# DIAGNijmegen/prostateMR_3D-CAD-csPCa

Measured on AMD Instinct MI355X. Metric: train-step volumes/sec (whole job), M1 (20,160,160,3), higher is better.
Workload: dtype bf16; 1 GPU; C3 M1 full hierarchical-probabilistic dense_skip+deep_supervision latents (3,2,1,0) (20,160,160,3); batch_per_gpu=2, global_batch=2, params=67254246, parallelism=dp1, hip_graph=True

## Files before the change

include/m1hip.h:

```cpp
#ifndef M1HIP_H
#define M1HIP_H

#include <stddef.h>
#include <stdint.h>

#ifdef __cplusplus
extern "C" {
#endif

enum m1_dtype { M1_F32 = 0, M1_BF16 = 1 };

enum m1_status {
    M1_OK = 0,
    M1_ERR_BAD_ARG = -1,
    M1_ERR_UNSUPPORTED = -2,
    M1_ERR_LAUNCH = -3,
    M1_ERR_WORKSPACE = -4
};

#define M1_MAX_SRC 6

typedef struct {
    const void* ptr;
    int C;
    int _pad;
} m1_src_t;

typedef struct {
    int N, D, H, W;
    int Cin, Cout;
    int kd, kh, kw;
    int sd, sh, sw;
    int dtype;
    int nsrc;
    m1_src_t src[M1_MAX_SRC];
} m1_conv_desc_t;

const char* m1_status_name(int status);
int m1_abi_version(void);

size_t m1_conv_ws_bytes(const m1_conv_desc_t* d, int transposed, int role);
int m1_conv_pack_jobs(const m1_conv_desc_t* d, int transposed, int role, void* ws, void** jobs_out);
int m1_pack_batch(const void* const* jobs_dev, const int* block_prefix_dev, int njobs, int total_blocks, void* stream);
int m1_conv3d_fwd(const m1_conv_desc_t* d, const float* w, const float* bias, void* y, float* stats, void* ws,
                  int ws_packed, void* stream);
int m1_conv3d_dgrad(const m1_conv_desc_t* d, const float* w, const void* dy, void* const* dx, const int* accumulate,
                    void* ws, int ws_packed, void* stream);
int m1_conv3d_pair_supported(const m1_conv_desc_t* d, int C1);
int m1_conv3d_dgrad_inbwd_rows(const m1_conv_desc_t* d);
int m1_conv3d_dgrad_inbwd(const m1_conv_desc_t* d, const float* w, const void* dy, void* da, const void* x, const float* stats,
                          const float* gamma, const float* beta, float slope, float* partial, int partial_rows, int* nparts,
                          void* ws, int ws_packed, void* stream);
int m1_conv3d_pair_fwd(const m1_conv_desc_t* d, const float* w1, const float* b1, const float* w4, const float* b4, int C1,
                       void* y1, void* y4, float* stats1, float* stats4, void* ws, int ws_packed, void* stream);
int m1_conv3d_pair_dgrad(const m1_conv_desc_t* d, const float* w1, const float* w4, int C1, const void* dy1, const void* dy4,
                         void* const* dx, const int* accumulate, void* ws, int ws_packed, void* stream);
int m1_conv3d_wgrad(const m1_conv_desc_t* d, const void* dy, float* dw, float* db, void* ws, int accumulate,
                    void* stream);
int m1_set_force_direct(int on);
int m1_config_set(const char* name, int value);
int m1_config_unset(const char* name);
int m1_config_get(const char* name, int* value);
int m1_debug_lds_canary(unsigned* bad, int blocks, int spins, void* stream);
int m1_debug_checksum(const void* p, long long nbytes, unsigned long long* slot, void* stream);
const char* m1_debug_kernels(int mode);
const char* m1_debug_plans(int mode);
int m1_debug_scribble(int blocks, int spins, void* stream);

int m1_convT3d_fwd(const m1_conv_desc_t* d, const float* w, const float* bias, void* y, void* ws, int ws_packed,
                   void* stream);
int m1_convT3d_dgrad(const m1_conv_desc_t* d, const float* w, const void* dy, void* const* dx, const int* accumulate,
                     void* ws, int ws_packed, void* stream);
int m1_convT3d_wgrad(const m1_conv_desc_t* d, const void* dy, float* dw, float* db, void* ws, int accumulate,
                     void* stream);

size_t m1_reduce_ws_floats(int N, long long V, int C, int nsums);
int m1_instnorm_stats(const void* x, int N, long long V, int C, int dtype, float eps, float* stats, float* ws,
                      void* stream);
int m1_instnorm_apply(const void* x, const float* stats, const float* gamma, const float* beta, float slope,
                      void* y, int N, long long V, int C, int dtype, void* stream);
int m1_instnorm_bwd(const void* x, const float* stats, const float* gamma, const float* beta, float slope,
                    const void* dy, void* dx, float* dgamma, float* dbeta, int N, long long V, int C, int dtype,
                    float* ws, int accumulate, void* stream);

int m1_instnorm_bwd_partials(const void* x, const float* stats, const float* gamma, const float* beta, float slope,
                             const void* dy, void* dx, float* dgamma, float* dbeta, int N, long long V, int C, int dtype,
                             const float* partial, int nparts, float* sums, int accumulate, void* stream);

int m1_se_gate_fwd(const float* beta3, const float* W6, const float* b6, const float* W7, const float* b7,
                   int F, int Fr, float* hidden, float* g, void* stream);
int m1_se_gate_bwd(const float* beta3, const float* W6, const float* W7, const float* hidden, const float* g,
                   const float* dg, int F, int Fr, float* dbeta3_add, float* dW6, float* db6, float* dW7,
                   float* db7, int accumulate, void* stream);
#define M1_SE_GATE_BATCH 16
typedef struct {
    const float* beta3; const float* W6; const float* b6; const float* W7; const float* b7;
    float* hidden; float* g;
    int F, Fr;
} m1_se_gate_fwd_job_t;
int m1_se_gate_fwd_batch(const m1_se_gate_fwd_job_t* jobs , int njobs, void* stream);
typedef struct {
    const float* beta3; const float* W6; const float* W7; const float* hidden; const float* g;
    float* dg;
    float* dbeta3_add; float* dW6; float* db6; float* dW7; float* db7;
    int F, Fr, accumulate, _pad;
} m1_se_gate_job_t;
int m1_se_gate_bwd_batch(const m1_se_gate_job_t* jobs , int njobs, void* stream);
int m1_se_combine_fwd(const void* y3, const void* y4, const float* stats3, const float* stats4,
                      const float* gamma3, const float* beta3, const float* gamma4, const float* beta4,
                      const float* g, void* out, int N, long long V, int F, int dtype, float drop_rate,
                      const uint64_t* rng, uint64_t layer_id, unsigned char* keep_mask, void* stream);
int m1_se_combine_bwd(const void* y3, const void* y4, const float* stats3, const float* stats4,
                      const float* gamma3, const float* beta3, const float* gamma4, const float* beta4,
                      const float* g, const void* dout, void* dy3, void* dy4, float* dgamma3, float* dbeta3,
                      float* dgamma4, float* dbeta4, float* dg, int N, long long V, int F, int dtype,
                      float drop_rate, const uint64_t* rng, uint64_t layer_id, const unsigned char* keep_mask,
                      float* ws, int accumulate, void* stream);

int m1_se_combine_dup_fwd(const void* y3, const void* y4, const float* stats3, const float* stats4,
                          const float* gamma3, const float* beta3, const float* gamma4, const float* beta4,
                          const float* g, void* out, int N, long long V, int F, int dtype, float drop_rate,
                          const uint64_t* rng, uint64_t layer_id, unsigned char* keep_mask, void* stream);
int m1_se_combine_dup_bwd(const void* y3, const void* y4, const float* stats3, const float* stats4,
                          const float* gamma3, const float* beta3, const float* gamma4, const float* beta4,
                          const float* g, const void* dout, void* dy3, void* dy4, float* dgamma3, float* dbeta3,
                          float* dgamma4, float* dbeta4, float* dg, int N, long long V, int F, int dtype,
                          float drop_rate, const uint64_t* rng, uint64_t layer_id, const unsigned char* keep_mask,
                          float* ws, int accumulate, void* stream);

int m1_gate_sigma_fwd(const void* theta, const void* phi, const float* wpsi, const float* bpsi, void* sigma,
                      int N, int Dt, int Ht, int Wt, int Dp, int Hp, int Wp, int C, int dtype, void* stream);
int m1_gate_sigma_bwd(const void* theta, const void* phi, const float* wpsi, const void* sigma,
                      const void* dsigma, void* dtheta, void* dphi, float* dwpsi, float* dbpsi, int N, int Dt,
                      int Ht, int Wt, int Dp, int Hp, int Wp, int C, int dtype, float* ws, int accumulate,
                      void* stream);
int m1_mul_sigma_fwd(const void* x, const void* sigma, void* y, int N, int D, int H, int W, int C, int s0,
                     int s1, int s2, int dtype, void* stream);
int m1_gate_sigma_mul_fwd(const void* theta, const void* phi, const float* wpsi, const float* bpsi, void* sigma, const void* x,
                          void* y, int N, int Dt, int Ht, int Wt, int Dp, int Hp, int Wp, int Ci, int D, int H, int W, int Cx,
                          int s0, int s1, int s2, int dtype, void* stream);
int m1_mul_sigma_bwd(const void* x, const void* sigma, const void* dy, void* dx, void* dsigma, int N, int D,
                     int H, int W, int C, int s0, int s1, int s2, int dtype, int accumulate_dx, void* stream);

int m1_latent_sample_fwd(const void* ml, const void* eps, void* z, int N, long long V, int L, int mode,
                         int dtype, void* stream);
int m1_latent_sample_bwd(const void* ml, const void* eps, const void* dz, void* dml, int N, long long V, int L,
                         int mode, int dtype, void* stream);
int m1_latent_sample_rng_fwd(const void* ml, const uint64_t* rng, uint64_t stream_id, void* z, int N, long long V, int L, int mode,
                             int dtype, void* stream);
int m1_latent_sample_rng_bwd(const void* ml, const uint64_t* rng, uint64_t stream_id, const void* dz, void* dml, int N, long long V,
                             int L, int mode, int dtype, void* stream);
int m1_kl_fwd(const void* ml_q, const void* ml_p, float* kl, int N, long long V, int L, int dtype, void* stream);
int m1_kl_bwd(const void* ml_q, const void* ml_p, const float* dkl, void* dml_q, void* dml_p, int N,
              long long V, int L, int dtype, void* stream);
int m1_kl_bwd_first(const void* ml_q, const void* ml_p, const float* dkl, void* dml_q, void* dml_p, int N, long long V,
                    int L, int Nall, int dtype, void* stream);

typedef struct {
    const void* logits;
    void* dlogits;
    int u0, u1, u2;
    int _pad;
} m1_head_t;
int m1_softmax_heads_fwd(const m1_head_t* heads, int nheads, float* probs, int N, int D, int H, int W, int nc,
                         int dtype, void* stream);
int m1_softmax_heads_bwd(const m1_head_t* heads, int nheads, const float* probs, const float* dprobs, int N,
                         int D, int H, int W, int nc, int dtype, void* stream);

int m1_mc_accum(const void* logits, int R, int B, long long V, int nc, int dtype, float* sum_p, int accumulate, float* samples_out,
                void* stream);
int m1_mc_finish(const float* sum_p, int n_draws, int B, long long V, int nc, float* mean, float* entropy, void* stream);

int m1_mc_accum_u(const void* logits, int R, int B, long long V, int nc, int dtype, float* sum_p, float* sum_h, float* sum_pp,
                  int accumulate, float* samples_out, void* stream);
int m1_mc_finish_u(const float* sum_p, const float* sum_h, const float* sum_pp, int n_draws, int B, long long V, int nc, float* mean,
                   float* entropy, float* expected_entropy, float* mutual_info, float* variance, void* stream);

int m1_mc_accum_v(const void* logits, int R, int B, int D, int H, int W, int nc, int dtype, unsigned long long flips, float* sum_p,
                  float* sum_h, float* sum_pp, int accumulate, float* samples_out, void* stream);
int m1_tta_views(const void* x, int B, int D, int H, int W, int C, int dtype, int R, unsigned long long flips, void* out, void* stream);

#define M1_TILE_MAX_AXIS 16
typedef struct { int vol[3]; int tile[3]; int n[3]; int origin[3][M1_TILE_MAX_AXIS]; } m1_tile_t;
int m1_tile_gather(const void* x, int B, int C, int dtype, const m1_tile_t* g, void* out, void* stream);
int m1_tile_blend(const float* tiles, int B, int C, const m1_tile_t* g, const float* profile, float* out, void* stream);

size_t m1_focal_ws_floats(int N, long long V, int nheads);
int m1_focal_fwd(const float* probs, const void* y_true, int y_dtype, const float* alpha, float gamma, int N, long long V,
                 int nheads, int nc, float* ws, float* loss, void* stream);
int m1_focal_bwd(const float* probs, const void* y_true, int y_dtype, const float* alpha, float gamma, int N, long long V,
                 int nheads, int nc, const float* dloss, float* dprobs, void* stream);

size_t m1_dist_map_ws_bytes(int N, int D, int H, int W, int nc);
int m1_dist_map(const void* y_true, int y_dtype, int N, int D, int H, int W, int nc, void* ws, float* out, void* stream);
size_t m1_dice_bd_ws_floats(long long NV, int nheads);
int m1_dice_bd_fwd(const float* probs, const void* y_true, int y_dtype, const float* phi, long long NV, int nheads, int nc,
                   float w0, float w1, float smooth, float* ws, float* loss, void* stream);
int m1_dice_bd_bwd(const float* probs, const void* y_true, int y_dtype, const float* phi, long long NV, int nheads, int nc,
                   float w0, float w1, float smooth, const float* ws, const float* dloss, float* dprobs, void* stream);

enum m1_aug_stage {
    M1_AUG_MASTER = 1, M1_AUG_ZOOM = 2, M1_AUG_FLIP = 4, M1_AUG_ROTATE = 8, M1_AUG_TRANSLATE = 16, M1_AUG_CSHIFT = 32,
    M1_AUG_GAMMA = 64, M1_AUG_POOR = 128, M1_AUG_NOISE = 256
};
typedef struct {
    uint32_t fired;
    uint32_t gamma_ch;
    uint32_t poor_ch;
    int32_t scale;
    int32_t rot_pad;
    float rot[6];
    int32_t tr[4];
    int32_t cs[4];
    int32_t cs_channel;
    float gamma;
    float noise_std;
    float angle_deg;
    int32_t _pad;
} m1_aug_params_t;
int m1_aug_draw(m1_aug_params_t* table, int N, const uint64_t* rng, uint64_t stream_id, double prob, double tx_prob,
                double translate_factor, double rotation_degree, int axial_hflip, double zoom_factor, double gauss_noise_stddev,
                double chan_shift_factor, int sim_poor_scan, double gamma_lo, double gamma_hi, int H, int W, int nimg, int lesion,
                void* stream);
size_t m1_aug_ws_bytes(int N, int D, int H, int W, int nimg);
int m1_aug_geom(const float* x, const float* y, const m1_aug_params_t* table, float* gx, float* gy, int N, int D, int H, int W,
                int C, int nimg, int nc, int stages, int dtype, void* ws, void* stream);
int m1_aug_gamma_stats(const float* gx, const m1_aug_params_t* table, int N, int D, int H, int W, int C, int nimg, int stages,
                       int dtype, void* ws, void* stream);
int m1_aug_intensity(const float* gx, const m1_aug_params_t* table, const uint64_t* rng, uint64_t stream_id, float* out, int N,
                     int D, int H, int W, int C, int nimg, int stages, int dtype, void* ws, void* stream);

int m1_contour_smooth_u8(const uint8_t* in, uint8_t* out, uint8_t* scratch, long long planes, int H, int W, const int* taps,
                         int iterations, void* stream);
enum m1_label_objective { M1_LABEL_LESION = 0, M1_LABEL_ZONAL = 1 };
enum m1_feed_mode { M1_FEED_TRAIN = 0, M1_FEED_VALID = 1, M1_FEED_TEST = 2 };
int m1_label_prepare(const uint8_t* ann, const float* image, float* x_out, float* detection, float* kl, int B, int D, int H, int W,
                     int C, int objective, int mode, int probabilistic, const int* taps, void* stream);

enum m1_raw_dtype { M1_RAW_F32 = 0, M1_RAW_I16 = 1, M1_RAW_I32 = 2 };
enum m1_pad_mode { M1_PAD_CONSTANT = 0, M1_PAD_EDGE = 1, M1_PAD_REFLECT = 2, M1_PAD_SYMMETRIC = 3 };
typedef struct { int src[3]; int dst[3]; int start[3]; int mode; float cval; } m1_crop_pad_t;
size_t m1_preprocess_ws_bytes(const m1_crop_pad_t* g, int B, int C, int nq);
int m1_crop_pad(const void* src, int src_dtype, const m1_crop_pad_t* g, int B, int C, void* out, int out_dtype, void* stream);
int m1_order_stats(const void* src, int src_dtype, const m1_crop_pad_t* g, int B, int C, const int* ranks, const double* weights,
                   int nq, float* pairs, float* values, void* ws, void* stream);
int m1_whiten(const void* src, int src_dtype, const m1_crop_pad_t* g, int B, int C, const float* bounds, void* out, int out_dtype,
              double* stats, void* ws, void* stream);

#define M1_RESAMPLE_MAX_LINE 1024
typedef struct { int src[3]; int dst[3]; int first[3]; int order; double step[3]; float defval; int _pad; } m1_resample_t;
size_t m1_resample_ws_bytes(const m1_resample_t* g, int B, int C);
int m1_resample(const void* src, int src_dtype, const m1_resample_t* g, int B, int C, void* out, int out_dtype, void* ws, void* stream);

#define M1_RESTORE_MAX_SEL 4
typedef struct { int src[3]; int dst[3]; int first[3]; int count[3]; int lo[3]; int order; double ratio[3]; float defval; int deflabel; } m1_restore_t;
int m1_restore(const void* src, int src_dtype, const m1_restore_t* g, int B, int C, int c0, int nsel, void* prob, void* label,
               void* stream);

#define M1_CC_TILE_Z 4
#define M1_CC_TILE_Y 8
#define M1_CC_TILE_X 32
enum m1_cc_dtype { M1_CC_F32 = 0, M1_CC_U8 = 1 };
enum m1_cc_state {
    M1_CC_ST_PEAK = 0, M1_CC_ST_ARGMAX = 1, M1_CC_ST_THRESHOLD = 2, M1_CC_ST_SEL = 3, M1_CC_ST_COUNT = 4, M1_CC_ST_DONE = 5,
    M1_CC_ST_NCAND = 6, M1_CC_ST_SPARE = 7
};
typedef struct {
    int32_t count;
    float vmax;
    int64_t argmax;
    int32_t lo[3];
    int32_t hi[3];
    int64_t sum[3];
} m1_cc_row_t;
size_t m1_cc_ws_bytes(int B, int D, int H, int W);
int m1_cc_label(const void* src, int src_dtype, float threshold, const float* threshold_dev, int connectivity, int B, int D, int H, int W,
                int* labels, int* counts, void* ws, void* stream);
int m1_cc_stats(const int* labels, const float* values, int B, int D, int H, int W, int max_components, m1_cc_row_t* rows, void* stream);
int m1_cc_overlap(const int* a, const int* b, int B, long long n, int max_a, int max_b, int* table, void* stream);
int m1_cc_peak(const float* w, int B, long long n, float factor, float min_confidence, int reset, int* state, void* ws, void* stream);
int m1_cc_select(const int* labels, int B, long long n, int* state, void* stream);
int m1_cc_take(const int* labels, int* state, const float* w_src, float* w, float* detection_map, int* candidates, float* confidences, int B, long long n,
               int max_candidates, int min_voxels, int reset, void* stream);
int m1_cc_relabel(const int* labels, const m1_cc_row_t* rows, int B, long long n, int max_components, int min_voxels, int* map,
                  float* detection_map, int* candidates, float* confidences, int* ncand, void* stream);

#define M1_SD_MAX_CLASSES 8
#define M1_SD_MAX_TOLERANCES 4
#define M1_SD_MAX_LINE 256
enum m1_sd_dtype { M1_SD_U8 = 0, M1_SD_I32 = 1 };
enum m1_sd_stage { M1_SD_STAGE_BORDER = 0, M1_SD_STAGE_DISTANCE = 1, M1_SD_STAGE_METRICS = 2 };
typedef struct {
    int64_t n[2];
    int64_t le[2][4];
    double sum[2];
    float hd, hd_ab, hd_ba;
    float assd, mean_ab, mean_ba;
    float hdq, hdq_ab, hdq_ba;
    float dice;
    float nsd[4];
    float _pad[2];
} m1_sd_row_t;
size_t m1_sd_ws_bytes(int stage, int B, int K, int D, int H, int W);
int m1_sd_border(const void* pred, const void* truth, int dtype, const int* labels, int K, int B, int D, int H, int W, uint8_t* borders,
                 long long* counts, void* ws, void* stream);
int m1_sd_distance(const uint8_t* mask, int N, int D, int H, int W, const double* spacing, float* dist, void* ws, void* stream);
int m1_sd_metrics(const uint8_t* borders, const float* dist, const long long* counts, int B, int K, int D, int H, int W, double percentile,
                  const float* tolerances, int T, m1_sd_row_t* rows, void* ws, void* stream);

int m1_dropout(const void* x, void* y, long long n, float rate, const uint64_t* rng, uint64_t layer_id, int dtype,
               void* stream);

int m1_cast(const void* x, int src_dtype, void* y, int dst_dtype, long long n, void* stream);

int m1_adam_amsgrad(float* p, const float* g, float* m, float* v, float* vhat, long long n, long long n_kernel,
                    long long n_bias, float l2_kernel, float l2_bias, float grad_scale, const float* lr_dev,
                    float beta1, float beta2, float eps, const int* step_dev, void* stream);
int m1_step_advance(int* step_dev, uint64_t* rng_dev, void* stream);

typedef struct {
    float norm;
    float coef;
    int32_t apply;
    int32_t skipped;
} m1_step_ctl_t;
size_t m1_grad_norm_ws(long long n);
int m1_grad_norm(const float* g, const float* p, long long n, long long n_kernel, long long n_bias, float l2_kernel,
                 float l2_bias, float grad_scale, float clipvalue, float global_clipnorm, int skip_nonfinite, void* ws,
                 size_t ws_bytes, m1_step_ctl_t* ctl, void* stream);
int m1_adam_amsgrad_ctl(float* p, const float* g, float* m, float* v, float* vhat, long long n, long long n_kernel,
                        long long n_bias, float l2_kernel, float l2_bias, float grad_scale, const float* lr_dev,
                        float beta1, float beta2, float eps, const int* step_dev, float clipvalue,
                        const m1_step_ctl_t* ctl, void* stream);
int m1_step_advance_ctl(int* step_dev, const m1_step_ctl_t* ctl, void* stream);

enum m1_val_dtype { M1_VAL_Y_F32 = 0, M1_VAL_Y_U8 = 1 };
typedef struct {
    double focal, entropy_sum, entropy_fg_sum, n_voxels, n_fg, _head[3];
    struct { double sum_p, sum_y, sum_py, n_pred, n_true, n_both, p_max, _pad; } cls[4];
} m1_val_record_t;
size_t m1_val_score_ws(int B, long long voxels, int K);
int m1_val_score(const float* p, const void* y, int y_dtype, const float* entropy, const float* alpha, float gamma, int B,
                 long long voxels, int K, m1_val_record_t* records, void* ws, size_t ws_bytes, void* stream);

size_t m1_cal_record_slots(int K, int bins);
int m1_cal_score(const void* p, int p_dtype, const unsigned char* label, const unsigned char* mask, const float* unc, float u_scale,
                 int B, long long voxels, int K, int bins, unsigned long long* records, void* stream);

#define M1_STREAM_BOOTSTRAP 0x424F4F54ull
#define M1_BOOTSTRAP_MAX_CASES 16384
#define M1_BOOTSTRAP_MAX_BOOT (1 << 20)
#define M1_BOOTSTRAP_MAX_RATES 8
#define M1_BOOTSTRAP_MAX_VALUES 16
#define M1_BOOTSTRAP_CHUNK 1024
typedef struct {
    const unsigned char* case_label; const unsigned char* case_group_end; const int* case_lesions;
    const int* ev_case; const unsigned char* ev_tp; const unsigned char* ev_group_end;
    const double* values; const int* draw_perm;
    int N, M, V, P;
} m1_bootstrap_table_t;
int m1_bootstrap_metrics(const m1_bootstrap_table_t* table, int n_boot, uint64_t seed, const int* weights, const double* fp_rates,
// ... 22 lines not shown
```

prostatemr_3d-cad-cspca_amd/csrc/dispatch.hip:

```cpp
#include "common.h"
#include "wgrad_fold.h"
#include "reduce.h"
#include <stdio.h>
#include <stdlib.h>

static inline bool desc_ok(const m1_conv_desc_t* d) {
    if (!(d && d->N > 0 && d->D > 0 && d->H > 0 && d->W > 0 && d->Cin > 0 && d->Cout > 0 && d->kd > 0 && d->kh > 0 &&
          d->kw > 0 && d->sd > 0 && d->sh > 0 && d->sw > 0 && d->nsrc >= 1 && d->nsrc <= M1_MAX_SRC)) return false;
    if (d->dtype != M1_F32 && d->dtype != M1_BF16) return false;
    int c = 0;
    for (int i = 0; i < d->nsrc; ++i) { if (!d->src[i].ptr || d->src[i].C <= 0) return false; c += d->src[i].C; }
    return c == d->Cin;
}
static inline double esz(int dt) { return dt == M1_BF16 ? 2.0 : 4.0; }
static inline void same_pad(int in, int k, int s, int* out, int* pb) {
    int o = (in + s - 1) / s;
    int tot = (o - 1) * s + k - in; if (tot < 0) tot = 0;
    *out = o; *pb = tot / 2;
}
static inline int convT_pb(int k, int s) { return (k - s > 0 ? k - s : 0) / 2; }

struct Geo { int OD, OH, OW, pd, ph, pw; };
static inline Geo conv_geo(const m1_conv_desc_t* d) {
    Geo g; same_pad(d->D, d->kd, d->sd, &g.OD, &g.pd); same_pad(d->H, d->kh, d->sh, &g.OH, &g.ph); same_pad(d->W, d->kw, d->sw, &g.OW, &g.pw);
// ... 240 lines not shown
    return align256(b);
}
struct WgradWs { size_t reduce_bytes, x8, r8, rx, total; long long rx_floats; };
static WgradWs wgrad_ws(const m1_conv_desc_t* d, bool T) {
    const Geo q = T ? convT_geo(d) : conv_geo(d);
    WgradWs w{};
    w.reduce_bytes = align256(m1_reduce_ws_floats(d->N, (long long)q.OD * q.OH * q.OW, d->Cout, 1) * sizeof(float)) + 256;
    w.x8 = w.r8 = w.rx = w.reduce_bytes;
    if (stem_wanted(d, T)) {
        w.r8 = w.x8 + align256((size_t)d->N * d->D * d->H * d->W * 16);
        w.rx = w.r8 + align256((size_t)d->kd * d->kh * d->kw * 8 * d->Cout * sizeof(float));
    }
    const size_t rx_bytes = wgrad_rx_bytes(d);
    w.rx_floats = (long long)(rx_bytes / sizeof(float));
    w.total = w.rx + rx_bytes * (size_t)d->nsrc;
    return w;
}

extern "C" size_t m1_conv_ws_bytes(const m1_conv_desc_t* d, int transposed, int role) {
    if (!desc_ok(d)) return 0;
    return role == 0 || role == 1 ? plan_gather(d, transposed != 0, role).total : wgrad_ws(d, transposed != 0).total;
}

extern "C" int m1_conv_pack_jobs(const m1_conv_desc_t* d, int transposed, int role, void* ws, void** jobs_out) {
    if (!desc_ok(d) || !ws || !jobs_out || (role != 0 && role != 1)) return 0;
    const GatherPlan p = plan_gather(d, transposed != 0, role);
    int n = 0;
    for (int k = 0; k < p.n; ++k) if (p.item[k].bytes) jobs_out[n++] = at(ws, p.item[k].off);
    return n;
}
extern "C" int m1_pack_batch(const void* const* jobs_dev, const int* block_prefix_dev, int njobs, int total_blocks, void* stream) {
    if (m1_debug_skip("pack")) return M1_OK;
    if (njobs < 0 || (njobs > 0 && !jobs_dev) || (block_prefix_dev && total_blocks < njobs)) return M1_ERR_BAD_ARG;
    M1ProfScope ps("pack_batch", 0.0, 0.0, (hipStream_t)stream);
    return m1_pack_batch_internal(jobs_dev, block_prefix_dev, njobs, total_blocks, (hipStream_t)stream);
}

static int fwd_common(const m1_conv_desc_t* d, bool T, const float* w, const float* bias, void* y, float* stats, void* ws, int ws_packed,
                      hipStream_t st) {
    if (stats && !ws) return M1_ERR_WORKSPACE;
    const GatherPlan p = plan_gather(d, T, 0);
    if (!ws && p.n > 1) return run_gather(fwd_spec(d, T, w, bias, y), nullptr, ws_packed, st);
    for (int k = 0; k < p.n; ++k) {
        GatherSpec g = fwd_item_spec(d, p, k, w, bias, y);
        const bool emit = stats && k == p.n - 1;
        if (emit) { g.stats_out = stats; g.stats_eps = 1e-3f; g.stats_ws = reinterpret_cast<float*>(at(ws, p.stats_off)); }
        int rc = run_gather(g, at(ws, p.item[k].off), ws_packed, st); if (rc) return rc;
        if (emit && p.n == 1 && !use_mfma(g))
            return m1_stats_internal(y, d->N, (long long)g.OD * g.OH * g.OW, d->Cout, d->dtype, 1e-3f, stats, g.stats_ws, st);
    }
    return M1_OK;
}
extern "C" int m1_conv3d_fwd(const m1_conv_desc_t* d, const float* w, const float* bias, void* y, float* stats, void* ws,
                             int ws_packed, void* stream) {
    if (m1_debug_skip("conv_fwd")) return M1_OK;
    if (!desc_ok(d) || !w || !y) return M1_ERR_BAD_ARG;
    M1ProfScope ps(prof_name("conv3d_fwd", d).s, 2.0 * conv_macs(d, false), conv_bytes(d, false), (hipStream_t)stream);
    return fwd_common(d, false, w, bias, y, stats, ws, ws_packed, (hipStream_t)stream);
}
static bool pair_ok(const m1_conv_desc_t* d, int C1) {
    if (!desc_ok(d) || g_force_direct) return false;
    const int seg = d->dtype == M1_BF16 ? 8 : 4;
    if (C1 <= 0 || C1 >= d->Cout || C1 % seg || (d->Cout - C1) % seg) return false;
    for (int i = 0; i < d->nsrc; ++i) if (d->src[i].C % seg) return false;
    return true;
}
static bool pair_fwd_spec(const m1_conv_desc_t* d, int C1, const float* w1, const float* b1, const float* w4, const float* b4, void* y1,
                          void* y4, float* stats1, float* stats4, void* ws, GatherSpec* out) {
    const GatherPlan p = plan_gather(d, false, 0);
    if (p.n != 1) return false;
    const int C4 = d->Cout - C1;
    GatherSpec g = fwd_item_spec(d, p, 0, w1, b1, nullptr);
    g.wST = (long long)d->Cin * C1; g.wSC = C1; g.wSO = 1;
    g.w2 = w4; g.w2ST = (long long)d->Cin * C4; g.w2SC = C4; g.w2SO = 1; g.oc_split = C1; g.bias2 = b4;
    g.nout = 2; g.outs[0] = y1; g.outC[0] = C1; g.outAcc[0] = 0; g.outs[1] = y4; g.outC[1] = C4; g.outAcc[1] = 0;
    if (stats1) { g.stats_out = stats1; g.stats_out2 = stats4; g.stats_eps = 1e-3f; g.stats_ws = reinterpret_cast<float*>(at(ws, p.stats_off)); }
    *out = g;
    return m1_mfma_supported(g) && gather_ws_bytes(g) == p.item[0].bytes;
}
static bool pair_dgrad_spec(const m1_conv_desc_t* d, int C1, const float* w1, const float* w4, const void* dy1, const void* dy4,
                            void* const* dx, const int* accumulate, GatherSpec* out) {
    const GatherPlan p = plan_gather(d, false, 1);
    if (p.n != 1) return false;
    const int C4 = d->Cout - C1;
    GatherSpec g = dgrad_item_spec(d, p, 0, w1, dy1, dx, accumulate);
    g.nsrc = 2; g.src[0] = dy1; g.srcC[0] = C1; g.src[1] = dy4; g.srcC[1] = C4;
    g.wST = (long long)d->Cin * C1; g.wSC = 1; g.wSO = C1;
    g.w2 = w4; g.w2ST = (long long)d->Cin * C4; g.w2SC = 1; g.w2SO = C4; g.c_split = C1;
    *out = g;
    return m1_mfma_supported(g) && gather_ws_bytes(g) <= p.item[0].bytes;
}
extern "C" int m1_conv3d_pair_fwd(const m1_conv_desc_t* d, const float* w1, const float* b1, const float* w4, const float* b4, int C1,
                                  void* y1, void* y4, float* stats1, float* stats4, void* ws, int ws_packed, void* stream) {
    if (m1_debug_skip("conv_fwd")) return M1_OK;
    if (!d || !w1 || !w4 || !y1 || !y4 || !ws || (stats1 == nullptr) != (stats4 == nullptr)) return M1_ERR_BAD_ARG;
    GatherSpec g;
    if (!pair_ok(d, C1) || !pair_fwd_spec(d, C1, w1, b1, w4, b4, y1, y4, stats1, stats4, ws, &g)) return M1_ERR_UNSUPPORTED;
    M1ProfScope ps(prof_name("conv3d_fwd", d).s, 2.0 * conv_macs(d, false), conv_bytes(d, false), (hipStream_t)stream);
    return m1_mfma_gather(g, ws, ws_packed, (hipStream_t)stream);
}
extern "C" int m1_conv3d_pair_dgrad(const m1_conv_desc_t* d, const float* w1, const float* w4, int C1, const void* dy1, const void* dy4,
                                    void* const* dx, const int* accumulate, void* ws, int ws_packed, void* stream) {
    if (m1_debug_skip("conv_dgrad")) return M1_OK;
    if (!d || !w1 || !w4 || !dy1 || !dy4 || !dx || !ws) return M1_ERR_BAD_ARG;
    if (!pair_ok(d, C1)) return M1_ERR_UNSUPPORTED;
    M1ProfScope ps(prof_name("conv3d_dgrad", d).s, 2.0 * conv_macs(d, false), conv_bytes(d, false), (hipStream_t)stream);
    if (d->nsrc == 1 && !dx[0]) return M1_OK;
    GatherSpec g;
    if (!pair_dgrad_spec(d, C1, w1, w4, dy1, dy4, dx, accumulate, &g)) return M1_ERR_UNSUPPORTED;
    bool any = false;
    for (int i = 0; i < d->nsrc; ++i) any |= dx[i] != nullptr;
    return any ? m1_mfma_gather(g, ws, ws_packed, (hipStream_t)stream) : M1_OK;
}

extern "C" int m1_conv3d_pair_supported(const m1_conv_desc_t* d, int C1) {
    GatherSpec g;
    return pair_ok(d, C1) && pair_fwd_spec(d, C1, nullptr, nullptr, nullptr, nullptr, nullptr, nullptr, nullptr, nullptr, nullptr, &g) &&
           pair_dgrad_spec(d, C1, nullptr, nullptr, nullptr, nullptr, nullptr, nullptr, &g);
}

extern "C" int m1_convT3d_fwd(const m1_conv_desc_t* d, const float* w, const float* bias, void* y, void* ws, int ws_packed,
                              void* stream) {
    if (m1_debug_skip("conv_fwd")) return M1_OK;
    if (!desc_ok(d) || !w || !y) return M1_ERR_BAD_ARG;
    M1ProfScope ps(prof_name("convT3d_fwd", d).s, 2.0 * conv_macs(d, true), conv_bytes(d, true), (hipStream_t)stream);
    return fwd_common(d, true, w, bias, y, nullptr, ws, ws_packed, (hipStream_t)stream);
}
static int dgrad_common(const m1_conv_desc_t* d, bool T, const float* w, const void* dy, void* const* dx, const int* accumulate,
                        void* ws, int ws_packed, hipStream_t st) {
    const GatherPlan p = plan_gather(d, T, 1);
    for (int k = 0; k < p.n; ++k) {
        const GatherItem& it = p.item[k];
        bool any = false;
        for (int i = it.first; i < it.first + it.count; ++i) any |= dx[i] != nullptr;
        if (!any) continue;
        int rc = run_gather(dgrad_item_spec(d, p, k, w, dy, dx, accumulate), at(ws, it.off), ws_packed, st); if (rc) return rc;
    }
    return M1_OK;
}
extern "C" int m1_conv3d_dgrad(const m1_conv_desc_t* d, const float* w, const void* dy, void* const* dx, const int* accumulate,
                               void* ws, int ws_packed, void* stream) {
    if (m1_debug_skip("conv_dgrad")) return M1_OK;
    if (!desc_ok(d) || !w || !dy || !dx) return M1_ERR_BAD_ARG;
    M1ProfScope ps(prof_name("conv3d_dgrad", d).s, 2.0 * conv_macs(d, false), conv_bytes(d, false), (hipStream_t)stream);
    return dgrad_common(d, false, w, dy, dx, accumulate, ws, ws_packed, (hipStream_t)stream);
}
extern "C" int m1_conv3d_dgrad_inbwd_rows(const m1_conv_desc_t* d) {
    if (!desc_ok(d)) return 0;
    const long long V = (long long)d->D * d->H * d->W;
    const long long tiles = m1_stats_rows_cap(V), chunks = m1_red_nchunks(V, d->Cin, d->N);
    const long long r = tiles > chunks ? tiles : chunks;
    return r > 0x3fffffff ? 0x3fffffff : (int)r;
}
extern "C" int m1_conv3d_dgrad_inbwd(const m1_conv_desc_t* d, const float* w, const void* dy, void* da, const void* x, const float* stats,
                                     const float* gamma, const float* beta, float slope, float* partial, int partial_rows, int* nparts,
                                     void* ws, int ws_packed, void* stream) {
    if (!desc_ok(d) || !w || !dy || !da || !x || !stats || !gamma || !beta || !partial || !nparts || d->nsrc != 1 || partial_rows < 0) return M1_ERR_BAD_ARG;
    M1ProfScope ps(prof_name("conv3d_dgrad", d).s, 2.0 * conv_macs(d, false), conv_bytes(d, false), (hipStream_t)stream);
    *nparts = 0;
    if (g_force_direct) { void* dxs[1] = {da}; int acc0[1] = {0}; return dgrad_common(d, false, w, dy, dxs, acc0, ws, ws_packed, (hipStream_t)stream); }
    GatherSpec g = dgrad_spec(d, false, w, dy, da, 0, 0);
    g.ib_x = x; g.ib_stats = stats; g.ib_gamma = gamma; g.ib_beta = beta; g.ib_slope = slope; g.ib_partial = partial; g.ib_nparts = nparts; g.ib_cap = partial_rows;
    return run_gather(g, ws, ws_packed, (hipStream_t)stream);
}
extern "C" int m1_convT3d_dgrad(const m1_conv_desc_t* d, const float* w, const void* dy, void* const* dx, const int* accumulate,
                                void* ws, int ws_packed, void* stream) {
    if (m1_debug_skip("conv_dgrad")) return M1_OK;
    if (!desc_ok(d) || !w || !dy || !dx) return M1_ERR_BAD_ARG;
    M1ProfScope ps(prof_name("convT3d_dgrad", d).s, 2.0 * conv_macs(d, true), conv_bytes(d, true), (hipStream_t)stream);
    return dgrad_common(d, true, w, dy, dx, accumulate, ws, ws_packed, (hipStream_t)stream);
}

static WgradSpec wgrad_spec(const m1_conv_desc_t* d, bool T, const Geo& q, int i, int off, const void* dy, float* dw, float* db, float* rx,
                            long long rx_floats) {
    WgradSpec g{};
    g.N = d->N; g.R = dw; g.kd = d->kd; g.kh = d->kh; g.kw = d->kw; g.sd = d->sd; g.sh = d->sh; g.sw = d->sw;
    g.pd = q.pd; g.ph = q.ph; g.pw = q.pw; g.dtype = d->dtype;
    g.rx = rx; g.rx_floats = rx_floats;
    if (!T) {
        g.A = d->src[i].ptr; g.CA = d->src[i].C; g.AD = d->D; g.AH = d->H; g.AW = d->W;
        g.B = dy; g.CB = d->Cout; g.BD = q.OD; g.BH = q.OH; g.BW = q.OW;
        g.RT = (long long)d->Cin * d->Cout; g.RSA = d->Cout; g.a_off = off; g.b_off = 0;
        if (db) { g.bsum = db; g.bsum_tap = (q.pd * d->kh + q.ph) * d->kw + q.pw; }
    } else {
        g.A = dy; g.CA = d->Cout; g.AD = q.OD; g.AH = q.OH; g.AW = q.OW;
        g.B = d->src[i].ptr; g.CB = d->src[i].C; g.BD = d->D; g.BH = d->H; g.BW = d->W;
        g.RT = (long long)d->Cout * d->Cin; g.RSA = d->Cin; g.a_off = 0; g.b_off = off;
    }
    return g;
}
static bool tf_wanted(const WgradSpec& g) {
    int maxc = M1_CFG("M1_TF_MAXC", 128);
    if (g.CA > 64 && g.CB > 32) return false;
    return g.CA <= maxc && g.CB <= maxc && m1_tf_wgrad_supported(g);
}
struct WgCall {
    bool T; int run; const void* Am[M1_MAX_SRC]; int aoffs[M1_MAX_SRC];
    long long nw; int nbias; long long rx_floats; hipStream_t st;
    const char** took;
};
static int equal_run(const m1_conv_desc_t* d, int i) {
    int n = 1;
    while (i + n < d->nsrc && d->src[i + n].C == d->src[i].C) ++n;
    return n;
}
struct WgRung {
    const char* name; bool whole_run, forced;
    bool (*gate)(const WgradSpec& g, const WgCall& c);
    int (*run)(const WgradSpec& g, const WgCall& c);
};
static const WgRung WG_LADDER[] = {
    {"t3", true, false, [](const WgradSpec& g, const WgCall&) { return g.rx && m1_t3_wgrad_supported(g); },
     [](const WgradSpec& g, const WgCall& c) { return m1_t3_wgrad(g, c.nw, c.nbias, c.st, c.run, c.Am, c.aoffs, c.rx_floats); }},
    {"pwf", false, false, [](const WgradSpec& g, const WgCall& c) { return g.rx && g.dtype == M1_F32 && !c.T && m1_pwf_wgrad_supported(g); },
     [](const WgradSpec& g, const WgCall& c) { return m1_pwf_wgrad(g, c.nw, c.nbias, c.st); }},
    {"t3s", false, false, [](const WgradSpec& g, const WgCall&) { return g.rx && g.dtype == M1_F32 && m1_t3s_wgrad_supported(g); },
     [](const WgradSpec& g, const WgCall& c) { return m1_t3s_wgrad(g, c.nw, c.nbias, c.st); }},
    {"tf-multi", true, false,
     [](const WgradSpec& g, const WgCall& c) { int multi = M1_CFG("M1_TF_MULTI", 1); return multi && !c.T && g.rx && tf_wanted(g) && c.run > 1; },
     [](const WgradSpec& g, const WgCall& c) { return m1_tf_wgrad_multi(g, c.nw, c.nbias, c.st, c.run, c.Am, c.aoffs, c.rx_floats); }},
    {"tf", false, false, [](const WgradSpec& g, const WgCall&) { return tf_wanted(g); },
     [](const WgradSpec& g, const WgCall& c) { return m1_tf_wgrad(g, c.nw, c.nbias, c.st); }},
    {"terminal", false, true, [](const WgradSpec&, const WgCall&) { return true; },
     [](const WgradSpec& g, const WgCall& c) {
         if (g_force_direct == 2 && m1_skinny_wgrad_supported(g)) { *c.took = "skinny"; return m1_skinny_wgrad(g, c.st); }
         if (!g_force_direct && m1_tap_wgrad_supported(g)) { *c.took = "tap"; return m1_tap_wgrad(g, c.nw, c.nbias, c.st); }
         if (!g_force_direct && m1_mfma_wgrad_supported(g)) { *c.took = "mfma"; return m1_mfma_wgrad_ex(g, c.nw, c.nbias, c.st); }
         *c.took = "direct"; return m1_direct_wgrad(g, c.st);
     }},
};
static int wgrad_common(const m1_conv_desc_t* d, bool T, const void* dy, float* dw, float* db, void* ws, hipStream_t st,
                        int accumulate) {
    Geo q = T ? convT_geo(d) : conv_geo(d);
    const size_t nw = (size_t)d->kd * d->kh * d->kw * d->Cin * d->Cout;
    if (!accumulate && m1_zero_async(dw, nw * sizeof(float), st) != M1_OK) return M1_ERR_LAUNCH;
    const bool fuse_db = db && !T && !g_force_direct;
    if (fuse_db && !accumulate && m1_zero_async(db, (size_t)d->Cout * sizeof(float), st) != M1_OK) return M1_ERR_LAUNCH;
    const int nbias = fuse_db ? d->Cout : 0;
    const WgradWs L = wgrad_ws(d, T);
    float* const rx = reinterpret_cast<float*>(at(ws, L.rx));
    const long long rx_floats = ws ? L.rx_floats : 0;
    if (stem_wanted(d, T) && ws) {
        const bool f32 = d->dtype == M1_F32;
        const int CP = f32 ? 4 : 8;
        uint4* x8 = reinterpret_cast<uint4*>(at(ws, L.x8));
        float* r8 = reinterpret_cast<float*>(at(ws, L.r8));
        m1_conv_desc_t dp = *d; dp.Cin = CP; dp.src[0].ptr = x8; dp.src[0].C = CP;
        const WgradSpec g = wgrad_spec(&dp, false, q, 0, 0, dy, r8, fuse_db ? db : nullptr, rx, rx_floats);
        if (f32 ? m1_t3s_wgrad_supported(g) : m1_tf_wgrad_supported(g)) {
            const int taps = d->kd * d->kh * d->kw, Cin = d->Cin;
            const long long nvox = (long long)d->N * d->D * d->H * d->W;
            const size_t nw8 = (size_t)taps * CP * d->Cout;
            if (m1_zero_async(r8, nw8 * sizeof(float), st) != M1_OK) return M1_ERR_LAUNCH;
            long long pb = (nvox + 255) / 256; if (pb > 8192) pb = 8192;
            if (f32) hipLaunchKernelGGL(stem_pad4f_kernel, dim3((unsigned)pb), dim3(256), 0, st, (const float*)d->src[0].ptr, reinterpret_cast<float4*>(x8), nvox, Cin);
            else hipLaunchKernelGGL(stem_pad8_kernel, dim3((unsigned)pb), dim3(256), 0, st, (const unsigned short*)d->src[0].ptr, x8, nvox, Cin);
            const int was = m1_fold_defer_set(0);
            int rc = f32 ? m1_t3s_wgrad(g, (long long)nw8, nbias, st) : m1_tf_wgrad(g, (long long)nw8, nbias, st);
            m1_fold_defer_set(was);
            if (rc == M1_OK) {
                m1_note_plan("stem:cp=%d", CP);
                hipLaunchKernelGGL(stem_fold_kernel, dim3((taps * Cin * d->Cout + 255) / 256), dim3(256), 0, st, r8, dw, taps, Cin, d->Cout, CP);
                return m1_check_launch();
            }
            if (rc != M1_ERR_UNSUPPORTED && rc != M1_ERR_WORKSPACE) return rc;
        }
    }
    const int wlog = M1_CFG("M1_WG_LOG", 0);
    for (int i = 0, off = 0; i < d->nsrc;) {
        WgCall c{};
        c.T = T; c.nw = (long long)nw; c.nbias = nbias; c.rx_floats = rx_floats; c.st = st;
        c.run = T ? 1 : equal_run(d, i);
        for (int m = 0, o = off; m < c.run; ++m) { c.Am[m] = d->src[i + m].ptr; c.aoffs[m] = o; o += d->src[i + m].C; }
        const WgradSpec g = wgrad_spec(d, T, q, i, off, dy, dw, fuse_db && i == 0 ? db : nullptr, rx ? rx + (long long)i * rx_floats : nullptr,
                                       rx_floats);
        int rc = M1_ERR_UNSUPPORTED, used = 1;
        for (const WgRung& r : WG_LADDER) {
            if ((g_force_direct && !r.forced) || !r.gate(g, c)) continue;
            const char* took = r.name; c.took = &took;
            rc = r.run(g, c); used = r.whole_run ? c.run : 1;
            if (wlog) fprintf(stderr, "wgrad %s N%d B %dx%dx%d CA %d x%d CB %d k%d%d%d s%d%d%d -> %s rc %d\n", T ? "convT" : "conv", g.N, g.BD,
                              g.BH, g.BW, g.CA, used, g.CB, g.kd, g.kh, g.kw, g.sd, g.sh, g.sw, took, rc);
            if (rc != M1_ERR_UNSUPPORTED && rc != M1_ERR_WORKSPACE) break;
            m1_note_plan("decline:%s rc=%d", r.name, rc);
        }
        if (rc) return rc;
        for (int m = 0; m < used; ++m) off += d->src[i++].C;
    }
    if (db && !fuse_db) {
        if (!ws) return M1_ERR_WORKSPACE;
        const long long Vd = (long long)q.OD * q.OH * q.OW;
        if (!g_force_direct && m1_colsum_defer(dy, d->N, Vd, d->Cout, d->dtype, db, (float*)ws, accumulate)) return M1_OK;
        return m1_colsum_internal(dy, d->N, Vd, d->Cout, d->dtype, db, (float*)ws, st, accumulate);
    }
    return M1_OK;
}
extern "C" int m1_conv3d_wgrad(const m1_conv_desc_t* d, const void* dy, float* dw, float* db, void* ws, int accumulate,
                               void* stream) {
    if (m1_debug_skip("conv_wgrad")) return M1_OK;
    if (!desc_ok(d) || !dy || !dw) return M1_ERR_BAD_ARG;
    M1ProfScope ps(prof_name("conv3d_wgrad", d).s, 2.0 * conv_macs(d, false), conv_bytes(d, false), (hipStream_t)stream);
    return wgrad_common(d, false, dy, dw, db, ws, (hipStream_t)stream, accumulate);
}
extern "C" int m1_convT3d_wgrad(const m1_conv_desc_t* d, const void* dy, float* dw, float* db, void* ws, int accumulate,
                                void* stream) {
    if (m1_debug_skip("conv_wgrad")) return M1_OK;
    if (!desc_ok(d) || !dy || !dw) return M1_ERR_BAD_ARG;
    M1ProfScope ps(prof_name("convT3d_wgrad", d).s, 2.0 * conv_macs(d, true), conv_bytes(d, true), (hipStream_t)stream);
    return wgrad_common(d, true, dy, dw, db, ws, (hipStream_t)stream, accumulate);
}
```

prostatemr_3d-cad-cspca_amd/csrc/gather.h:

```cpp
#pragma once
#include "common.h"

struct GatherSpec {
    const void* src[M1_MAX_SRC]; int srcC[M1_MAX_SRC]; int nsrc;
    int ID, IH, IW;
    void* out; int OC;
    int nout; void* outs[M1_MAX_SRC]; int outC[M1_MAX_SRC]; int outAcc[M1_MAX_SRC];
    int OD, OH, OW, N;
    const float* w; long long wST, wSC, wSO; int oc_off, cc_off;
    const float* bias;
    const float* w2; long long w2ST, w2SC, w2SO; int oc_split, c_split;
    const float* bias2; float* stats_out2;
    int kd, kh, kw, mode, sd, sh, sw, pd, ph, pw;
    int dtype, accumulate;
    float* stats_out;
    float* stats_ws;
    float stats_eps;
    const void* ib_x; const float* ib_stats; const float* ib_gamma; const float* ib_beta; float ib_slope;
    float* ib_partial; int* ib_nparts;
    int ib_cap;
};

int m1_stats_internal(const void* x, int N, long long V, int C, int dtype, float eps, float* stats, float* ws, hipStream_t st);
size_t m1_stats_ws_floats(int N, long long V, int C);

struct WgradSpec {
    const void* A; int CA; int AD, AH, AW;
    const void* B; int CB; int BD, BH, BW;
    int N;
    float* R; long long RT, RSA; int a_off, b_off;
    int kd, kh, kw, sd, sh, sw, pd, ph, pw;
    int dtype;
    float* rx; long long rx_floats;
    float* bsum;
    int bsum_tap;
};

int m1_direct_gather(const GatherSpec& g, hipStream_t st);
int m1_direct_wgrad(const WgradSpec& g, hipStream_t st);
bool m1_skinny_wgrad_supported(const WgradSpec& g);
int m1_skinny_wgrad(const WgradSpec& g, hipStream_t st);
bool m1_mfma_supported(const GatherSpec& g);
size_t m1_mfma_ws_bytes(const GatherSpec& g);
int m1_mfma_gather(const GatherSpec& g, void* ws, int ws_packed, hipStream_t st);
int m1_thin_conv_try(const GatherSpec& g, hipStream_t st, int* rc);
int m1_pack_batch_internal(const void* const* jobs_dev, const int* prefix_dev, int njobs, int total_blocks, hipStream_t st);
bool m1_mfma_wgrad_supported(const WgradSpec& g);
int m1_mfma_wgrad(const WgradSpec& g, hipStream_t st);
bool m1_tf_wgrad_supported(const WgradSpec& g);
int m1_tf_wgrad(const WgradSpec& g, long long nw, int nb, hipStream_t st);
int m1_tf_wgrad_multi(const WgradSpec& g, long long nw, int nb, hipStream_t st, int nmem, const void* const* Am, const int* a_offs, long long rx_mem);
int m1_mfma_wgrad_ex(const WgradSpec& g, long long nw, int nb, hipStream_t st);
bool m1_tap_wgrad_supported(const WgradSpec& g);
int m1_tap_wgrad(const WgradSpec& g, long long nw, int nb, hipStream_t st);
bool m1_t3_wgrad_supported(const WgradSpec& g);
int m1_t3_wgrad(const WgradSpec& g, long long nw, int nb, hipStream_t st, int nmem, const void* const* Am, const int* a_offs, long long rx_mem);
bool m1_t3s_wgrad_supported(const WgradSpec& g);
int m1_t3s_wgrad(const WgradSpec& g, long long nw, int nb, hipStream_t st);
bool m1_pwf_wgrad_supported(const WgradSpec& g);
int m1_pwf_wgrad(const WgradSpec& g, long long nw, int nb, hipStream_t st);
int m1_colsum_internal(const void* x, int N, long long V, int C, int dtype, float* out, float* ws, hipStream_t st, int accumulate);
long long m1_stats_rows_cap(long long V);
```

prostatemr_3d-cad-cspca_amd/csrc/wgrad_tf.hip:

```cpp
#include "common.h"
#include "wgrad_fold.h"
#include "cdna4.h"
#include <stdlib.h>

#define TF_MAX_NKS 4
#define TF_MAX_AIT 10

struct TfP {
    const bf16_t* A; const bf16_t* B; float* R; float* bsum;
    int CA, CB, AD, AH, AW, BD, BH, BW, N;
    long long RT, RSA; int a_off, b_off;
    int sd, sh, sw, pd, ph, pw;
    int KWs, TH;
    int AHt, AWt;
    int spra, sprb;
    int a_slots, b_slots;
    int a_bytes, b_bytes;
    int tiles_w, tiles_h; long long ntiles;
    int bTiles, nsplit;
    int stages;
    float* Rx; long long rx_stride;
    long long rx_bias;
    int nks;
    int nmem; const bf16_t* Am[M1_MAX_SRC]; long long rx_mem;
};

#define TF_MAX_STAGES 8

template <int KD, int KH, int KW, int KPARTS, int TF_NKS, bool M32 = false>
__global__ void __launch_bounds__(256, M32 ? 2 : 1) wgrad_tf_kernel(TfP p) {
#if defined(__HIP_DEVICE_COMPILE__)
    constexpr int NT = KD * KH * KW, NG = KD * KH;
    extern __shared__ __attribute__((aligned(16))) unsigned char smem[];
    const int tid = threadIdx.x, lane = tid & 63, wave = __builtin_amdgcn_readfirstlane(tid >> 6);
    constexpr int kparts = KPARTS, ntile = 4 / KPARTS;
    const int ntb = p.CB > 16 ? 2 : 1;
    const int tile_id = wave % ntile, part = wave / ntile;
    const int ta = tile_id / ntb, tb = tile_id % ntb;
    const int a0 = (blockIdx.x / p.bTiles) * 32, b0 = (blockIdx.x % p.bTiles) * 32;
    const int mem = p.nmem > 1 ? (int)blockIdx.z : 0;
    const bf16_t* Abase = p.A;
    if (p.nmem > 1) {
        Abase = p.Am[0];
#pragma unroll
        for (int m = 1; m < M1_MAX_SRC; ++m) if (mem == m) Abase = p.Am[m];
    }
    const int PA = p.spra * 16, PB = p.sprb * 16;
    const int stage_bytes = p.a_bytes + p.b_bytes;

    constexpr unsigned OOB = 0x80000000u;
    unsigned a_vo[TF_MAX_AIT]; int a_pk[TF_MAX_AIT];
    const int nait = p.a_slots >> 8;
#pragma unroll
    for (int it = 0; it < TF_MAX_AIT; ++it) {
        const int q = it * 256 + tid;
        const int row = q / p.spra, slp = q - row * p.spra;
        const int dd = row / (p.AHt * p.AWt); const int r2 = row - dd * (p.AHt * p.AWt);
        const int hh = r2 / p.AWt, ww = r2 - hh * p.AWt;
        const int sl = p.spra == 4 ? (slp ^ (((ww >> 3) & 1) << 1)) : slp;
        a_pk[it] = dd | (hh << 8) | (ww << 16);
        a_vo[it] = (row < KD * p.AHt * p.AWt) ? (unsigned)((((dd * p.AH + hh) * p.AW + ww) * p.CA + a0 + sl * 8) * 2) : OOB;
    }
    constexpr int NBIT = (TF_NKS * 32 * 4 + 255) / 256;
    const int nbit = (p.b_slots + 255) >> 8;
    unsigned b_vo[NBIT]; int b_th[NBIT];
#pragma unroll
    for (int it = 0; it < NBIT; ++it) {
        const int q = it * 256 + tid;
        const int row = q / p.sprb, slp = q - row * p.sprb;
        const int th = row / p.KWs, tw = row - th * p.KWs;
        const int sl = p.sprb == 4 ? (slp ^ (((tw >> 3) & 1) << 1)) : slp;
        b_th[it] = th;
        b_vo[it] = q < p.b_slots ? (unsigned)(((th * p.BW + tw) * p.CB + b0 + sl * 8) * 2) : OOB;
    }

    int q_kt = blockIdx.y, q_tw, q_th, q_bd, q_n;
    { int r = q_kt; q_tw = r % p.tiles_w; r /= p.tiles_w; q_th = r % p.tiles_h; r /= p.tiles_h; q_bd = r % p.BD; q_n = r / p.BD; }
    int s_tw, s_th, s_bd, s_n;
    { int r = p.nsplit; s_tw = r % p.tiles_w; r /= p.tiles_w; s_th = r % p.tiles_h; r /= p.tiles_h; s_bd = r % p.BD; s_n = r / p.BD; }
    auto issue = [&](int st) {
        const bool live = q_kt < (int)p.ntiles;
        const int twi = q_tw, thi = q_th, bd = q_bd, n = q_n;
        q_kt += p.nsplit;
        q_tw += s_tw; int c = q_tw >= p.tiles_w; q_tw -= c ? p.tiles_w : 0;
        q_th += s_th + c; c = q_th >= p.tiles_h; q_th -= c ? p.tiles_h : 0;
        q_bd += s_bd + c; c = q_bd >= p.BD; q_bd -= c ? p.BD : 0;
        q_n += s_n + c;
        const int ad0 = bd * p.sd - p.pd, ah0 = thi * p.TH * p.sh - p.ph, aw0 = twi * p.KWs * p.sw - p.pw;
        const long long lin0 = (((long long)n * p.AD + ad0) * p.AH + ah0) * p.AW + aw0;
        const int bh0 = thi * p.TH;
        const long long blin0 = (((long long)n * p.BD + bd) * p.BH + bh0) * p.BW + twi * p.KWs;
        unsigned char* As = smem + st * stage_bytes;
        unsigned char* Bs = As + p.a_bytes;
        const __amdgpu_buffer_rsrc_t ra = __builtin_amdgcn_make_buffer_rsrc((void*)(Abase + lin0 * p.CA), 0, live ? 0x7fffffff : 0, 0x00020000);
        const __amdgpu_buffer_rsrc_t rb = __builtin_amdgcn_make_buffer_rsrc((void*)(p.B + blin0 * p.CB), 0, live ? 0x7fffffff : 0, 0x00020000);
        const bool a_inner = ad0 >= 0 && ad0 + KD - 1 < p.AD && ah0 >= 0 && ah0 + p.AHt - 1 < p.AH && aw0 >= 0 && aw0 + p.AWt - 1 < p.AW;
        if (a_inner) {
#pragma unroll
            for (int it = 0; it < TF_MAX_AIT; ++it)
                if (it < nait) __builtin_amdgcn_raw_ptr_buffer_load_lds(ra, (lptr_t)(As + (it * 256 + wave * 64) * 16), 16, a_vo[it], 0, 0, 0);
        } else {
#pragma unroll
            for (int it = 0; it < TF_MAX_AIT; ++it) {
                if (it < nait) {
                    const int pk = a_pk[it];
                    const int dd = pk & 0xff, hh = (pk >> 8) & 0xff, ww = (pk >> 16) & 0xff;
                    const bool ok = (unsigned)(ad0 + dd) < (unsigned)p.AD && (unsigned)(ah0 + hh) < (unsigned)p.AH && (unsigned)(aw0 + ww) < (unsigned)p.AW;
                    __builtin_amdgcn_raw_ptr_buffer_load_lds(ra, (lptr_t)(As + (it * 256 + wave * 64) * 16), 16, ok ? a_vo[it] : OOB, 0, 0, 0);
                }
            }
        }
        const bool b_inner = bh0 + p.TH <= p.BH;
#pragma unroll
        for (int it = 0; it < NBIT; ++it)
            if (it < nbit)
                __builtin_amdgcn_raw_ptr_buffer_load_lds(rb, (lptr_t)(Bs + (it * 256 + wave * 64) * 16), 16,
                                                         (b_inner || bh0 + b_th[it] < p.BH) ? b_vo[it] : OOB, 0, 0, 0);
    };

    if constexpr (M32) {
    const unsigned lds0 = (unsigned)(unsigned long long)(lptr_t)smem;
    const int S = p.stages;
    const int npiece = nait + nbit;
    const long long kt0 = blockIdx.y, step = p.nsplit;
    static_assert(KPARTS == 1 && KW == 3, "the tap split assumes 32 x 32 tiles and t % KW == (w + j) % KW");
    constexpr int NK = 2 * TF_NKS, NTW = (NT + 3) / 4;
    const int g2 = lane >> 4, i = lane & 15, kg = g2 >> 1, ch = g2 & 1;
    unsigned a_ad[2][KW], b_ad[2];
#pragma unroll
    for (int h = 0; h < 2; ++h) {
        const int kk = 8 * kg + 4 * h + (i >> 2);
        const int th = kk / p.KWs, tw = kk - th * p.KWs;
#pragma unroll
        for (int r = 0; r < KW; ++r) {
            const int ww = tw * p.sw + (wave + r) % KW;
            a_ad[h][r] = lds0 + ((th * p.sh) * p.AWt + ww) * PA + (ch ^ ((ww >> 3) & 1)) * 32 + (i & 3) * 8;
        }
        b_ad[h] = lds0 + p.a_bytes + kk * PB + (ch ^ ((tw >> 3) & 1)) * 32 + (i & 3) * 8;
    }
    const unsigned ko1 = (unsigned)(((16 / p.KWs) * p.sh * p.AWt + (16 % p.KWs) * p.sw) * PA);
    const unsigned ko2 = (unsigned)(((32 / p.KWs) * p.sh * p.AWt + (32 % p.KWs) * p.sw) * PA);
    unsigned ro[NTW];
#pragma unroll
    for (int j = 0; j < NTW; ++j) {
        const int tg = (wave + 4 * j) / KW;
        ro[j] = (unsigned)(((tg / KH) * p.AHt + tg % KH) * p.AWt * PA);
    }
    const bool last_ok = wave + 4 * (NTW - 1) < NT;

    f32x16_t acc[NTW];
#pragma unroll
    for (int j = 0; j < NTW; ++j)
#pragma unroll
        for (int e = 0; e < 16; ++e) acc[j][e] = 0.f;
    const bool do_bsum = p.bsum != nullptr && a0 == 0 && wave == 3 && mem == 0;
    f32x16_t accb;
#pragma unroll
    for (int e = 0; e < 16; ++e) accb[e] = 0.f;
    const bf16x8_t ones = __builtin_bit_cast(bf16x8_t, make_uint4(0x3F803F80u, 0x3F803F80u, 0x3F803F80u, 0x3F803F80u));

    auto tile = [&](unsigned sb, auto n_c) {
        constexpr int N = decltype(n_c)::value, NI = NK * (N + 1);
        constexpr int D = N + 1 < 6 ? N + 1 : 6, RS = D + 1;
        u32x2_t bl[2], bh[2], al[RS], ah[RS];
        auto rd = [&](auto m_c) {
            constexpr int m = decltype(m_c)::value, u = m / (N + 1), j = m % (N + 1) - 1;
            if constexpr (j < 0) {
                const unsigned so = sb + (unsigned)(u * 16) * PB;
                bl[u & 1] = m1_tr_read_asm(b_ad[0] + so); bh[u & 1] = m1_tr_read_asm(b_ad[1] + so);
            } else {
                constexpr int sl = (u * N + j) % RS;
                const unsigned so = sb + ro[j] + (u >> 1) * ko2 + (u & 1) * ko1;
                al[sl] = m1_tr_read_asm(a_ad[0][j % KW] + so); ah[sl] = m1_tr_read_asm(a_ad[1][j % KW] + so);
            }
        };
        m1_static_for<0, D>(rd);
        bf16x8_t bfr;
        m1_static_for<0, NI>([&](auto m_c) {
            constexpr int m = decltype(m_c)::value, u = m / (N + 1), j = m % (N + 1) - 1;
            if constexpr (m + D < NI) rd(std::integral_constant<int, m + D>{});
            constexpr int after = NI - 1 - m < D ? NI - 1 - m : D;
            if constexpr (j < 0) {
                m1_lds_wait_n<2 * after>(bl[u & 1], bh[u & 1]);
                bfr = m1_frag8(bl[u & 1], bh[u & 1]);
                if (do_bsum) accb = __builtin_amdgcn_mfma_f32_32x32x16_bf16(ones, bfr, accb, 0, 0, 0);
            } else {
                constexpr int sl = (u * N + j) % RS;
                m1_lds_wait_n<2 * after>(al[sl], ah[sl]);
                acc[j] = __builtin_amdgcn_mfma_f32_32x32x16_bf16(m1_frag8(al[sl], ah[sl]), bfr, acc[j], 0, 0, 0);
            }
            __builtin_amdgcn_sched_barrier(0);
        });
    };

    auto run_tiles = [&](auto&& tile_fn) {
        for (int s = 0; s < S - 1; ++s) issue(s);
        int st = 0;
        for (long long kt = kt0; kt < p.ntiles; kt += step) {
            m1_wait_vm<48>(npiece * (S - 2));
            __builtin_amdgcn_s_barrier();
            int stn = st + S - 1; if (stn >= S) stn -= S;
            issue(stn);
            tile_fn((unsigned)(st * stage_bytes));
            if (++st == S) st = 0;
        }
        asm volatile("s_waitcnt vmcnt(0)" ::: "memory");
    };
    if (last_ok) run_tiles([&](unsigned sb) { tile(sb, std::integral_constant<int, NTW>{}); });
    else run_tiles([&](unsigned sb) { tile(sb, std::integral_constant<int, NTW - 1>{}); });

    float* Rx = p.Rx + (long long)mem * p.rx_mem + (long long)blockIdx.y * p.rx_stride;
    const int b = b0 + (lane & 31);
    if (do_bsum && lane < 32 && b < p.CB) Rx[p.rx_bias + b] = accb[0];
#pragma unroll
    for (int j = 0; j < NTW; ++j) {
        const int t = wave + 4 * j;
#pragma unroll
        for (int e = 0; e < 16; ++e) {
            const int a = a0 + (e & 3) + 8 * (e >> 2) + 4 * (lane >> 5);
            if (t < NT && a < p.CA && b < p.CB) Rx[((long long)t * p.CA + a) * p.CB + b] = acc[j][e];
        }
    }
    } else {
    const int g = lane >> 4, i = lane & 15;
    const unsigned lds0 = (unsigned)(unsigned long long)(lptr_t)smem;
    unsigned a_ad[TF_NKS][2][KW], b_ad[TF_NKS][2];
#pragma unroll
    for (int ks = 0; ks < TF_NKS; ++ks)
#pragma unroll
        for (int h = 0; h < 2; ++h) {
            const int kk = ks * 32 + 8 * g + 4 * h + (i >> 2);
            const int th = kk / p.KWs, tw = kk - th * p.KWs;
#pragma unroll
            for (int kw = 0; kw < KW; ++kw) {
                const int ww = tw * p.sw + kw;
                const int half = p.spra == 4 ? (ta ^ ((ww >> 3) & 1)) : ta;
                a_ad[ks][h][kw] = lds0 + ((th * p.sh) * p.AWt + ww) * PA + half * 32 + (i & 3) * 8;
            }
            const int halfb = p.sprb == 4 ? (tb ^ ((tw >> 3) & 1)) : tb;
            b_ad[ks][h] = lds0 + p.a_bytes + kk * PB + halfb * 32 + (i & 3) * 8;
        }
    const int grp_pitch = p.AWt * PA;

    f32x4_t acc[NT];
#pragma unroll
    for (int t = 0; t < NT; ++t) acc[t] = (f32x4_t){0.f, 0.f, 0.f, 0.f};
    const bool do_bsum = p.bsum != nullptr && a0 == 0 && ta == 0 && part == 0 && mem == 0;
    f32x4_t accb = (f32x4_t){0.f, 0.f, 0.f, 0.f};
    const bf16x8_t ones = __builtin_bit_cast(bf16x8_t, make_uint4(0x3F803F80u, 0x3F803F80u, 0x3F803F80u, 0x3F803F80u));

    const int S = p.stages;
    const int npiece = nait + nbit;
    const long long kt0 = blockIdx.y, step = p.nsplit;
    for (int s = 0; s < S - 1; ++s) issue(s);
    int st = 0;
    for (long long kt = kt0; kt < p.ntiles; kt += step) {
        m1_wait_vm<48>(npiece * (S - 2));
        __builtin_amdgcn_s_barrier();
        int stn = st + S - 1; if (stn >= S) stn -= S;
        issue(stn);
        const unsigned sb = (unsigned)(st * stage_bytes);
        constexpr int NU = TF_NKS * KD, CH = KH * KW;
        u32x2_t bl[2], bh[2], al[2][CH], ah[2][CH];
        auto rd_unit = [&](int u, int set) {
            const int ks = u / KD, kd = u % KD;
            if (kd == 0) { bl[ks & 1] = m1_tr_read_asm(b_ad[ks][0] + sb); bh[ks & 1] = m1_tr_read_asm(b_ad[ks][1] + sb); }
#pragma unroll
            for (int kh = 0; kh < KH; ++kh) {
                const unsigned ro = sb + (unsigned)((kd * p.AHt + kh) * grp_pitch);
#pragma unroll
                for (int kw = 0; kw < KW; ++kw) {
                    if (((kd * CH + kh * KW + kw) % kparts) == part) {
                        al[set][kh * KW + kw] = m1_tr_read_asm(a_ad[ks][0][kw] + ro);
                        ah[set][kh * KW + kw] = m1_tr_read_asm(a_ad[ks][1][kw] + ro);
                    }
                }
            }
        };
        rd_unit(0, 0);
#pragma unroll
        for (int u = 0; u < NU; ++u) {
            const int ks = u / KD, kd = u % KD, set = u & 1;
            if (kd == 0) m1_lds_wait(bl[ks & 1], bh[ks & 1]);
#pragma unroll
            for (int c = 0; c < CH; ++c) m1_lds_wait(al[set][c], ah[set][c]);
            if (u + 1 < NU) rd_unit(u + 1, set ^ 1);
            __builtin_amdgcn_sched_barrier(0);
            const bf16x8_t bfr = m1_frag8(bl[ks & 1], bh[ks & 1]);
            if (do_bsum && kd == 0) accb = __builtin_amdgcn_mfma_f32_16x16x32_bf16(ones, bfr, accb, 0, 0, 0);
#pragma unroll
            for (int c = 0; c < CH; ++c)
                if (((kd * CH + c) % kparts) == part)
                    acc[kd * CH + c] = __builtin_amdgcn_mfma_f32_16x16x32_bf16(m1_frag8(al[set][c], ah[set][c]), bfr, acc[kd * CH + c], 0, 0, 0);
            __builtin_amdgcn_sched_barrier(0);
        }
        if (++st == S) st = 0;
    }
    asm volatile("s_waitcnt vmcnt(0)" ::: "memory");

    float* Rx = p.Rx + (long long)mem * p.rx_mem + (long long)blockIdx.y * p.rx_stride;
    const int b = b0 + tb * 16 + i;
    if (do_bsum && g == 0 && b < p.CB) Rx[p.rx_bias + b] = accb[0];
#pragma unroll
    for (int t = 0; t < NT; ++t)
#pragma unroll
        for (int r = 0; r < 4; ++r) {
            const int a = a0 + ta * 16 + g * 4 + r;
            if ((t % kparts) == part && a < p.CA && b < p.CB) Rx[((long long)t * p.CA + a) * p.CB + b] = acc[t][r];
        }
    }
#endif
}


static inline bool tf_chan_ok(int c) { return c == 8 || c == 16 || (c >= 32 && c % 32 == 0); }

static bool tf_plan(const WgradSpec& g, TfP& p) {
    if (g.dtype != M1_BF16) return false;
    const bool k133 = g.kd == 1 && g.kh == 3 && g.kw == 3, k333 = g.kd == 3 && g.kh == 3 && g.kw == 3;
    if (!k133 && !k333) return false;
    if (!tf_chan_ok(g.CA) || !tf_chan_ok(g.CB)) return false;
    if (g.BW % 8) return false;
    if (!m1_wg_vox32(g)) return false;
    p = TfP{};
    p.A = (const bf16_t*)g.A; p.B = (const bf16_t*)g.B; p.R = g.R; p.bsum = g.bsum;
    p.CA = g.CA; p.CB = g.CB; p.AD = g.AD; p.AH = g.AH; p.AW = g.AW; p.BD = g.BD; p.BH = g.BH; p.BW = g.BW; p.N = g.N;
    p.RT = g.RT; p.RSA = g.RSA; p.a_off = g.a_off; p.b_off = g.b_off;
    p.sd = g.sd; p.sh = g.sh; p.sw = g.sw; p.pd = g.pd; p.ph = g.ph; p.pw = g.pw;
    int n4 = M1_CFG("M1_TF_NKS4", 2);
    const int nks = ((n4 && g.CA <= 16 && g.CB <= 16) || (n4 == 2 && g.kd == 1)) ? 4 : 2;
    p.nks = nks;
    if (!m1_wg_ktiles(g, nks * 32, m1_wg_kws(g.BW, 8), 0, p)) return false;
    p.AHt = (p.TH - 1) * g.sh + g.kh; p.AWt = (p.KWs - 1) * g.sw + g.kw;
    p.spra = (g.CA < 32 ? g.CA : 32) / 8; p.sprb = (g.CB < 32 ? g.CB : 32) / 8;
    const int a_rows = g.kd * p.AHt * p.AWt;
    p.a_slots = (a_rows * p.spra + 255) / 256 * 256; p.b_slots = nks * 32 * p.sprb;
    if (p.a_slots > TF_MAX_AIT * 256 || p.AHt > 255 || p.AWt > 255) return false;
    p.a_bytes = p.a_slots * 16; p.b_bytes = (p.b_slots + 255) / 256 * 256 * 16 + 64;
    const int sb = p.a_bytes + p.b_bytes, npiece = p.a_slots / 256 + (p.b_slots + 255) / 256;
    int S = (76 * 1024) / sb;
    if (S < 3) S = 3;
    if (S > TF_MAX_STAGES) S = TF_MAX_STAGES;
    while (S > 3 && npiece * (S - 2) > 48) --S;
    { int fs = M1_CFG("M1_TF_STAGES", 0); if (fs >= 3) S = fs; }
    p.stages = S;
    return npiece * (S - 2) <= 48 && (size_t)S * sb <= 160 * 1024;
}
bool m1_tf_wgrad_supported(const WgradSpec& g) { TfP p; return tf_plan(g, p); }

static const WgCopyRule TF_COPIES = {1, 0, 96ll << 20, WG_SHORT_ERROR};
static int tf_wgrad_launch(const WgradSpec& g, long long nw, int nb, hipStream_t st, int nmem, const void* const* Am, const int* a_offs, long long rx_mem);
int m1_tf_wgrad_multi(const WgradSpec& g, long long nw, int nb, hipStream_t st, int nmem, const void* const* Am, const int* a_offs, long long rx_mem) {
    return tf_wgrad_launch(g, nw, nb, st, nmem, Am, a_offs, rx_mem);
}
int m1_tf_wgrad(const WgradSpec& g, long long nw, int nb, hipStream_t st) { return tf_wgrad_launch(g, nw, nb, st, 1, nullptr, nullptr, 0); }
static int tf_wgrad_launch(const WgradSpec& g, long long nw, int nb, hipStream_t st, int nmem, const void* const* Am, const int* a_offs, long long rx_mem) {
    TfP p;
    if (!tf_plan(g, p)) return M1_ERR_UNSUPPORTED;
    const int TS = 32;
    const int aTiles = (g.CA + TS - 1) / TS; p.bTiles = (g.CB + TS - 1) / TS;
    const int ctiles = aTiles * p.bTiles;
    int tgt_env = M1_CFG("M1_TF_SPLIT", 0);
    const int tgt = tgt_env > 0 ? tgt_env : (p.ntiles >= 24576 ? 512 : 256);
    const long long want = (tgt + ctiles - 1) / ctiles;
    const WgCopies c = m1_wg_copies(g, g.kd * g.kh * g.kw, want, p.ntiles, TF_COPIES);
    if (c.rc) return c.rc;
    const long long nsplit = c.nsplit;
    p.nsplit = (int)nsplit;
    p.Rx = c.Rx; p.rx_stride = c.stride; p.rx_bias = c.rx_bias;
    const size_t smem = (size_t)p.stages * (p.a_bytes + p.b_bytes);
    dim3 grid(ctiles, (unsigned)nsplit, 1);
    p.nmem = 1; p.rx_mem = 0;
    if (nmem > 1) {
        if (nmem > M1_MAX_SRC) return M1_ERR_UNSUPPORTED;
        p.nmem = nmem; p.rx_mem = rx_mem; grid.z = (unsigned)nmem;
        for (int m = 0; m < nmem; ++m) p.Am[m] = (const bf16_t*)Am[m];
    }
    const int kparts = 4 / ((g.CA > 16 ? 2 : 1) * (g.CB > 16 ? 2 : 1));
    void (*kern)(TfP) = nullptr;
#define TF_PICK(KD_, KP_) if ((g.kd == KD_) && kparts == KP_ && p.nks == 2) kern = wgrad_tf_kernel<KD_, 3, 3, KP_, 2>;
    TF_PICK(1, 1) TF_PICK(1, 2) TF_PICK(1, 4) TF_PICK(3, 1) TF_PICK(3, 2) TF_PICK(3, 4)
#undef TF_PICK
    if (p.nks == 4 && kparts == 4) kern = g.kd == 1 ? wgrad_tf_kernel<1, 3, 3, 4, 4> : (g.kd == 3 ? wgrad_tf_kernel<3, 3, 3, 4, 4> : nullptr);
    if (p.nks == 4 && g.kd == 1 && kparts == 1) kern = wgrad_tf_kernel<1, 3, 3, 1, 4>;
    if (p.nks == 4 && g.kd == 1 && kparts == 2) kern = wgrad_tf_kernel<1, 3, 3, 2, 4>;
    if (kparts == 1 && kern && M1_CFG("M1_TF_MFMA32", 1)) {
        if (g.kd == 3) kern = wgrad_tf_kernel<3, 3, 3, 1, 2, true>;
        else kern = p.nks == 4 ? wgrad_tf_kernel<1, 3, 3, 1, 4, true> : wgrad_tf_kernel<1, 3, 3, 1, 2, true>;
    }
    if (!kern) return M1_ERR_UNSUPPORTED;
    if (m1_allow_dynamic_lds((const void*)kern, 160 * 1024) != M1_OK) return M1_ERR_LAUNCH;
    m1_note_kernel("wgrad_tf");
    m1_wg_note_plan("wgrad_tf", p.ntiles, want, nsplit, c, true, p.stages, grid.x, grid.y, grid.z);
    hipLaunchKernelGGL(kern, grid, dim3(256), smem, st, p);
    int rc = m1_check_launch(); if (rc) return rc;
    return m1_wg_fold_members(p.Rx, rx_mem, c.stride, (int)nsplit, g, c.rx_bias, nmem < 1 ? 1 : nmem, a_offs, st);
}
```

prostatemr_3d-cad-cspca_amd/hip/lib.py:

```python
from __future__ import annotations

import ctypes as C
import os
import subprocess
import threading

_HERE = os.path.dirname(os.path.abspath(__file__))
PKG_DIR = os.path.dirname(_HERE)
CSRC_DIR = os.path.join(PKG_DIR, "csrc")
SO_PATH = os.path.join(PKG_DIR, "libm1hip.so")
if os.environ.get("M1HIP_SO"):
    SO_PATH = os.path.join(PKG_DIR, os.path.basename(os.environ["M1HIP_SO"]))
HEADER = os.path.join(os.path.dirname(PKG_DIR), "include", "m1hip.h")

M1_F32, M1_BF16 = 0, 1
M1_MAX_SRC = 6


class m1_src_t(C.Structure):
    _fields_ = [("ptr", C.c_void_p), ("C", C.c_int), ("_pad", C.c_int)]


class m1_conv_desc_t(C.Structure):
    _fields_ = [("N", C.c_int), ("D", C.c_int), ("H", C.c_int), ("W", C.c_int),
                ("Cin", C.c_int), ("Cout", C.c_int),
                ("kd", C.c_int), ("kh", C.c_int), ("kw", C.c_int),
                ("sd", C.c_int), ("sh", C.c_int), ("sw", C.c_int),
                ("dtype", C.c_int), ("nsrc", C.c_int),
                ("src", m1_src_t * M1_MAX_SRC)]


class m1_head_t(C.Structure):
    _fields_ = [("logits", C.c_void_p), ("dlogits", C.c_void_p),
                ("u0", C.c_int), ("u1", C.c_int), ("u2", C.c_int), ("_pad", C.c_int)]


class SeGateFwdJob(C.Structure):
    _fields_ = [(n, C.c_void_p) for n in ("beta3", "W6", "b6", "W7", "b7", "hidden", "g")] + [("F", C.c_int), ("Fr", C.c_int)]


class SeGateJob(C.Structure):
    _fields_ = [(n, C.c_void_p) for n in ("beta3", "W6", "W7", "hidden", "g", "dg", "dbeta3_add", "dW6", "db6", "dW7", "db7")] \
        + [("F", C.c_int), ("Fr", C.c_int), ("accumulate", C.c_int), ("_pad", C.c_int)]


class m1_aug_params_t(C.Structure):
    _fields_ = [("fired", C.c_uint32), ("gamma_ch", C.c_uint32), ("poor_ch", C.c_uint32), ("scale", C.c_int32),
                ("rot_pad", C.c_int32), ("rot", C.c_float * 6), ("tr", C.c_int32 * 4), ("cs", C.c_int32 * 4),
                ("cs_channel", C.c_int32), ("gamma", C.c_float), ("noise_std", C.c_float), ("angle_deg", C.c_float),
                ("_pad", C.c_int32)]


M1_AUG_MASTER, M1_AUG_ZOOM, M1_AUG_FLIP, M1_AUG_ROTATE, M1_AUG_TRANSLATE = 1, 2, 4, 8, 16
M1_AUG_CSHIFT, M1_AUG_GAMMA, M1_AUG_POOR, M1_AUG_NOISE = 32, 64, 128, 256


class m1_crop_pad_t(C.Structure):
    _fields_ = [("src", C.c_int * 3), ("dst", C.c_int * 3), ("start", C.c_int * 3), ("mode", C.c_int), ("cval", C.c_float)]


M1_RAW_F32, M1_RAW_I16, M1_RAW_I32 = 0, 1, 2
M1_PAD_CONSTANT, M1_PAD_EDGE, M1_PAD_REFLECT, M1_PAD_SYMMETRIC = 0, 1, 2, 3


class m1_resample_t(C.Structure):
    _fields_ = [("src", C.c_int * 3), ("dst", C.c_int * 3), ("first", C.c_int * 3), ("order", C.c_int), ("step", C.c_double * 3),
                ("defval", C.c_float), ("_pad", C.c_int)]


M1_RESAMPLE_MAX_LINE = 1024


class m1_restore_t(C.Structure):
    _fields_ = [("src", C.c_int * 3), ("dst", C.c_int * 3), ("first", C.c_int * 3), ("count", C.c_int * 3), ("lo", C.c_int * 3),
                ("order", C.c_int), ("ratio", C.c_double * 3), ("defval", C.c_float), ("deflabel", C.c_int)]


M1_RESTORE_MAX_SEL = 4

M1_TILE_MAX_AXIS = 16


class m1_tile_t(C.Structure):
    _fields_ = [("vol", C.c_int * 3), ("tile", C.c_int * 3), ("n", C.c_int * 3), ("origin", (C.c_int * M1_TILE_MAX_AXIS) * 3)]


class m1_cc_row_t(C.Structure):
    _fields_ = [("count", C.c_int32), ("vmax", C.c_float), ("argmax", C.c_int64), ("lo", C.c_int32 * 3), ("hi", C.c_int32 * 3),
                ("sum", C.c_int64 * 3)]


M1_CC_F32, M1_CC_U8 = 0, 1
(M1_CC_ST_PEAK, M1_CC_ST_ARGMAX, M1_CC_ST_THRESHOLD, M1_CC_ST_SEL, M1_CC_ST_COUNT, M1_CC_ST_DONE, M1_CC_ST_NCAND,
 M1_CC_ST_SPARE) = range(8)
M1_CC_TILE = (4, 8, 32)

class m1_sd_row_t(C.Structure):
    _fields_ = [("n", C.c_int64 * 2), ("le", (C.c_int64 * 4) * 2), ("sum", C.c_double * 2), ("hd", C.c_float), ("hd_ab", C.c_float),
                ("hd_ba", C.c_float), ("assd", C.c_float), ("mean_ab", C.c_float), ("mean_ba", C.c_float), ("hdq", C.c_float),
                ("hdq_ab", C.c_float), ("hdq_ba", C.c_float), ("dice", C.c_float), ("nsd", C.c_float * 4), ("_pad", C.c_float * 2)]


M1_SD_U8, M1_SD_I32 = 0, 1
M1_SD_STAGE_BORDER, M1_SD_STAGE_DISTANCE, M1_SD_STAGE_METRICS = 0, 1, 2
M1_SD_MAX_CLASSES, M1_SD_MAX_TOLERANCES, M1_SD_MAX_LINE = 8, 4, 256

M1_VAL_Y_F32, M1_VAL_Y_U8 = 0, 1
M1_VAL_SLOTS, M1_VAL_MAX_K = 40, 4
VAL_HEAD_KEYS = ("focal", "entropy_sum", "entropy_fg_sum", "n_voxels", "n_fg")
VAL_CLASS_KEYS = ("sum_p", "sum_y", "sum_py", "n_pred", "n_true", "n_both", "p_max")

M1_CAL_HEAD, M1_CAL_MIN_K, M1_CAL_MAX_K, M1_CAL_MAX_BINS, M1_CAL_MAX_VOXELS = 8, 2, 4, 64, 1 << 27
CAL_HEAD_KEYS = ("n_valid", "n_invalid", "n_ignored", "nll")
CAL_HIST_KEYS = {"top": ("count", "conf_sum", "correct"), "cls": ("count", "p_sum", "pos"), "unc": ("count", "u_sum", "errors")}

M1_STREAM_BOOTSTRAP = 0x424F4F54
M1_BOOTSTRAP_MAX_CASES, M1_BOOTSTRAP_MAX_BOOT, M1_BOOTSTRAP_MAX_RATES, M1_BOOTSTRAP_MAX_VALUES = 16384, 1 << 20, 8, 16
M1_BOOTSTRAP_CHUNK = 1024


class m1_bootstrap_table_t(C.Structure):
    _fields_ = [(n, C.c_void_p) for n in ("case_label", "case_group_end", "case_lesions", "ev_case", "ev_tp", "ev_group_end",
                                          "values", "draw_perm")] + [(n, C.c_int) for n in ("N", "M", "V", "P")]


M1_LABEL_LESION, M1_LABEL_ZONAL = 0, 1
M1_FEED_TRAIN, M1_FEED_VALID, M1_FEED_TEST = 0, 1, 2


class m1_prof_rec_t(C.Structure):
    _fields_ = [("name", C.c_char * 48), ("total_ms", C.c_double), ("flops", C.c_double),
                ("bytes", C.c_double), ("launches", C.c_longlong)]


_vp, _i, _ll, _f, _u64, _sz, _d = C.c_void_p, C.c_int, C.c_longlong, C.c_float, C.c_uint64, C.c_size_t, C.c_double
_desc_p = C.POINTER(m1_conv_desc_t)

SIGNATURES = {
    "m1_status_name": (C.c_char_p, [_i]),
    "m1_abi_version": (_i, []),
    "m1_conv_ws_bytes": (_sz, [_desc_p, _i, _i]),
    "m1_conv_pack_jobs": (_i, [_desc_p, _i, _i, _vp, C.POINTER(_vp)]),
    "m1_pack_batch": (_i, [_vp, _vp, _i, _i, _vp]),
    "m1_set_force_direct": (_i, [_i]),
    "m1_conv3d_fwd": (_i, [_desc_p, _vp, _vp, _vp, _vp, _vp, _i, _vp]),
    "m1_conv3d_dgrad": (_i, [_desc_p, _vp, _vp, C.POINTER(_vp), C.POINTER(_i), _vp, _i, _vp]),
    "m1_conv3d_dgrad_inbwd_rows": (_i, [_desc_p]),
    "m1_conv3d_dgrad_inbwd": (_i, [_desc_p, _vp, _vp, _vp, _vp, _vp, _vp, _vp, _f, _vp, _i, C.POINTER(_i), _vp, _i, _vp]),
    "m1_config_set": (_i, [C.c_char_p, _i]),
    "m1_config_unset": (_i, [C.c_char_p]),
    "m1_config_get": (_i, [C.c_char_p, C.POINTER(_i)]),
    "m1_debug_lds_canary": (_i, [_vp, _i, _i, _vp]),
    "m1_debug_checksum": (_i, [_vp, _ll, _vp, _vp]),
    "m1_debug_scribble": (_i, [_i, _i, _vp]),
    "m1_debug_kernels": (C.c_char_p, [_i]),
    "m1_debug_plans": (C.c_char_p, [_i]),
    "m1_conv3d_wgrad": (_i, [_desc_p, _vp, _vp, _vp, _vp, _i, _vp]),
    "m1_conv3d_pair_supported": (_i, [_desc_p, _i]),
    "m1_conv3d_pair_fwd": (_i, [_desc_p, _vp, _vp, _vp, _vp, _i, _vp, _vp, _vp, _vp, _vp, _i, _vp]),
    "m1_conv3d_pair_dgrad": (_i, [_desc_p, _vp, _vp, _i, _vp, _vp, C.POINTER(_vp), C.POINTER(_i), _vp, _i, _vp]),
    "m1_convT3d_fwd": (_i, [_desc_p, _vp, _vp, _vp, _vp, _i, _vp]),
    "m1_convT3d_dgrad": (_i, [_desc_p, _vp, _vp, C.POINTER(_vp), C.POINTER(_i), _vp, _i, _vp]),
    "m1_convT3d_wgrad": (_i, [_desc_p, _vp, _vp, _vp, _vp, _i, _vp]),
    "m1_reduce_ws_floats": (_sz, [_i, _ll, _i, _i]),
    "m1_instnorm_stats": (_i, [_vp, _i, _ll, _i, _i, _f, _vp, _vp, _vp]),
    "m1_instnorm_apply": (_i, [_vp, _vp, _vp, _vp, _f, _vp, _i, _ll, _i, _i, _vp]),
    "m1_instnorm_bwd": (_i, [_vp, _vp, _vp, _vp, _f, _vp, _vp, _vp, _vp, _i, _ll, _i, _i, _vp, _i, _vp]),
    "m1_instnorm_bwd_partials": (_i, [_vp, _vp, _vp, _vp, _f, _vp, _vp, _vp, _vp, _i, _ll, _i, _i, _vp, _i, _vp, _i, _vp]),
    "m1_se_gate_fwd": (_i, [_vp, _vp, _vp, _vp, _vp, _i, _i, _vp, _vp, _vp]),
    "m1_se_gate_fwd_batch": (_i, [C.POINTER(SeGateFwdJob), _i, _vp]),
    "m1_se_gate_bwd_batch": (_i, [C.POINTER(SeGateJob), _i, _vp]),
    "m1_se_gate_bwd": (_i, [_vp, _vp, _vp, _vp, _vp, _vp, _i, _i, _vp, _vp, _vp, _vp, _vp, _i, _vp]),
    "m1_se_combine_fwd": (_i, [_vp] * 10 + [_i, _ll, _i, _i, _f, _vp, _u64, _vp, _vp]),
    "m1_se_combine_bwd": (_i, [_vp] * 17 + [_i, _ll, _i, _i, _f, _vp, _u64, _vp, _vp, _i, _vp]),
    "m1_se_combine_dup_fwd": (_i, [_vp] * 10 + [_i, _ll, _i, _i, _f, _vp, _u64, _vp, _vp]),
    "m1_se_combine_dup_bwd": (_i, [_vp] * 17 + [_i, _ll, _i, _i, _f, _vp, _u64, _vp, _vp, _i, _vp]),
    "m1_gate_sigma_fwd": (_i, [_vp] * 5 + [_i] * 9 + [_vp]),
    "m1_gate_sigma_bwd": (_i, [_vp] * 9 + [_i] * 9 + [_vp, _i, _vp]),
    "m1_mul_sigma_fwd": (_i, [_vp] * 3 + [_i] * 9 + [_vp]),
    "m1_gate_sigma_mul_fwd": (_i, [_vp] * 7 + [_i] * 16 + [_vp]),
    "m1_mul_sigma_bwd": (_i, [_vp] * 5 + [_i] * 10 + [_vp]),
    "m1_latent_sample_fwd": (_i, [_vp, _vp, _vp, _i, _ll, _i, _i, _i, _vp]),
    "m1_latent_sample_bwd": (_i, [_vp, _vp, _vp, _vp, _i, _ll, _i, _i, _i, _vp]),
    "m1_latent_sample_rng_fwd": (_i, [_vp, _vp, _u64, _vp, _i, _ll, _i, _i, _i, _vp]),
    "m1_latent_sample_rng_bwd": (_i, [_vp, _vp, _u64, _vp, _vp, _i, _ll, _i, _i, _i, _vp]),
    "m1_kl_fwd": (_i, [_vp, _vp, _vp, _i, _ll, _i, _i, _vp]),
    "m1_kl_bwd": (_i, [_vp, _vp, _vp, _vp, _vp, _i, _ll, _i, _i, _vp]),
    "m1_kl_bwd_first": (_i, [_vp, _vp, _vp, _vp, _vp, _i, _ll, _i, _i, _i, _vp]),
    "m1_softmax_heads_fwd": (_i, [C.POINTER(m1_head_t), _i, _vp, _i, _i, _i, _i, _i, _i, _vp]),
    "m1_softmax_heads_bwd": (_i, [C.POINTER(m1_head_t), _i, _vp, _vp, _i, _i, _i, _i, _i, _i, _vp]),
    "m1_mc_accum": (_i, [_vp, _i, _i, _ll, _i, _i, _vp, _i, _vp, _vp]),
    "m1_mc_finish": (_i, [_vp, _i, _i, _ll, _i, _vp, _vp, _vp]),
    "m1_mc_accum_u": (_i, [_vp, _i, _i, _ll, _i, _i, _vp, _vp, _vp, _i, _vp, _vp]),
    "m1_mc_finish_u": (_i, [_vp, _vp, _vp, _i, _i, _ll, _i, _vp, _vp, _vp, _vp, _vp, _vp]),
    "m1_mc_accum_v": (_i, [_vp, _i, _i, _i, _i, _i, _i, _i, _u64, _vp, _vp, _vp, _i, _vp, _vp]),
    "m1_tta_views": (_i, [_vp, _i, _i, _i, _i, _i, _i, _i, _u64, _vp, _vp]),
    "m1_tile_gather": (_i, [_vp, _i, _i, _i, C.POINTER(m1_tile_t), _vp, _vp]),
    "m1_tile_blend": (_i, [_vp, _i, _i, C.POINTER(m1_tile_t), _vp, _vp, _vp]),
    "m1_focal_ws_floats": (_sz, [_i, _ll, _i]),
    "m1_focal_fwd": (_i, [_vp, _vp, _i, C.POINTER(_f), _f, _i, _ll, _i, _i, _vp, _vp, _vp]),
    "m1_focal_bwd": (_i, [_vp, _vp, _i, C.POINTER(_f), _f, _i, _ll, _i, _i, _vp, _vp, _vp]),
    "m1_dist_map_ws_bytes": (_sz, [_i, _i, _i, _i, _i]),
    "m1_dist_map": (_i, [_vp, _i, _i, _i, _i, _i, _i, _vp, _vp, _vp]),
    "m1_dice_bd_ws_floats": (_sz, [_ll, _i]),
    "m1_dice_bd_fwd": (_i, [_vp, _vp, _i, _vp, _ll, _i, _i, _f, _f, _f, _vp, _vp, _vp]),
    "m1_dice_bd_bwd": (_i, [_vp, _vp, _i, _vp, _ll, _i, _i, _f, _f, _f, _vp, _vp, _vp, _vp]),
    "m1_aug_draw": (_i, [_vp, _i, _vp, _u64, _d, _d, _d, _d, _i, _d, _d, _d, _i, _d, _d, _i, _i, _i, _i, _vp]),
    "m1_aug_ws_bytes": (_sz, [_i, _i, _i, _i, _i]),
    "m1_aug_geom": (_i, [_vp] * 5 + [_i] * 9 + [_vp, _vp]),
    "m1_aug_gamma_stats": (_i, [_vp, _vp] + [_i] * 8 + [_vp, _vp]),
    "m1_aug_intensity": (_i, [_vp, _vp, _vp, _u64, _vp] + [_i] * 8 + [_vp, _vp]),
    "m1_contour_smooth_u8": (_i, [_vp, _vp, _vp, _ll, _i, _i, C.POINTER(_i), _i, _vp]),
    "m1_label_prepare": (_i, [_vp] * 5 + [_i] * 8 + [C.POINTER(_i), _vp]),
    "m1_preprocess_ws_bytes": (_sz, [C.POINTER(m1_crop_pad_t), _i, _i, _i]),
    "m1_crop_pad": (_i, [_vp, _i, C.POINTER(m1_crop_pad_t), _i, _i, _vp, _i, _vp]),
    "m1_order_stats": (_i, [_vp, _i, C.POINTER(m1_crop_pad_t), _i, _i, C.POINTER(_i), C.POINTER(_d), _i, _vp, _vp, _vp, _vp]),
    "m1_whiten": (_i, [_vp, _i, C.POINTER(m1_crop_pad_t), _i, _i, _vp, _vp, _i, _vp, _vp, _vp]),
    "m1_resample_ws_bytes": (_sz, [C.POINTER(m1_resample_t), _i, _i]),
    "m1_resample": (_i, [_vp, _i, C.POINTER(m1_resample_t), _i, _i, _vp, _i, _vp, _vp]),
    "m1_restore": (_i, [_vp, _i, C.POINTER(m1_restore_t), _i, _i, _i, _i, _vp, _vp, _vp]),
    "m1_cc_ws_bytes": (_sz, [_i, _i, _i, _i]),
    "m1_cc_label": (_i, [_vp, _i, _f, _vp, _i, _i, _i, _i, _i, _vp, _vp, _vp, _vp]),
    "m1_cc_stats": (_i, [_vp, _vp, _i, _i, _i, _i, _i, _vp, _vp]),
    "m1_cc_overlap": (_i, [_vp, _vp, _i, _ll, _i, _i, _vp, _vp]),
    "m1_cc_peak": (_i, [_vp, _i, _ll, _f, _f, _i, _vp, _vp, _vp]),
    "m1_cc_select": (_i, [_vp, _i, _ll, _vp, _vp]),
    "m1_cc_take": (_i, [_vp, _vp, _vp, _vp, _vp, _vp, _vp, _i, _ll, _i, _i, _i, _vp]),
    "m1_cc_relabel": (_i, [_vp, _vp, _i, _ll, _i, _i, _vp, _vp, _vp, _vp, _vp, _vp]),
    "m1_sd_ws_bytes": (_sz, [_i, _i, _i, _i, _i, _i]),
    "m1_sd_border": (_i, [_vp, _vp, _i, C.POINTER(_i), _i, _i, _i, _i, _i, _vp, _vp, _vp, _vp]),
    "m1_sd_distance": (_i, [_vp, _i, _i, _i, _i, C.POINTER(_d), _vp, _vp, _vp]),
    "m1_sd_metrics": (_i, [_vp, _vp, _vp, _i, _i, _i, _i, _i, _d, C.POINTER(_f), _i, _vp, _vp, _vp]),
    "m1_dropout": (_i, [_vp, _vp, _ll, _f, _vp, _u64, _i, _vp]),
    "m1_cast": (_i, [_vp, _i, _vp, _i, _ll, _vp]),
    "m1_adam_amsgrad": (_i, [_vp] * 5 + [_ll, _ll, _ll, _f, _f, _f, _vp, _f, _f, _f, _vp, _vp]),
    "m1_step_advance": (_i, [_vp, _vp, _vp]),
    "m1_grad_norm_ws": (_sz, [_ll]),
    "m1_grad_norm": (_i, [_vp, _vp, _ll, _ll, _ll, _f, _f, _f, _f, _f, _i, _vp, _sz, _vp, _vp]),
    "m1_adam_amsgrad_ctl": (_i, [_vp] * 5 + [_ll, _ll, _ll, _f, _f, _f, _vp, _f, _f, _f, _vp, _f, _vp, _vp]),
    "m1_step_advance_ctl": (_i, [_vp, _vp, _vp]),
    "m1_val_score_ws": (_sz, [_i, _ll, _i]),
    "m1_val_score": (_i, [_vp, _vp, _i, _vp, C.POINTER(_f), _f, _i, _ll, _i, _vp, _vp, _sz, _vp]),
    "m1_cal_record_slots": (_sz, [_i, _i]),
    "m1_cal_score": (_i, [_vp, _i, _vp, _vp, _vp, _f, _i, _ll, _i, _i, _vp, _vp]),
    "m1_bootstrap_metrics": (_i, [C.POINTER(m1_bootstrap_table_t), _i, _u64, _vp, C.POINTER(_d), _i, _vp, _vp]),
    "m1_wgrad_defer": (_i, [_i]),
    "m1_wgrad_fold_pending": (_i, [_vp]),
    "m1_wgrad_fold_drop": (_i, []),
    "m1_prof_enable": (_i, [_i]),
    "m1_prof_reset": (_i, []),
    "m1_prof_read": (_i, [C.POINTER(m1_prof_rec_t), _i]),
}

_lib = None
_lock = threading.Lock()


def build(verbose: bool = False) -> str:
    cmd = ["make", "-C", CSRC_DIR, "-j8"]
    res = subprocess.run(cmd, capture_output=True, text=True)
    if verbose or res.returncode != 0:
        print(res.stdout[-4000:])
        print(res.stderr[-4000:])
    if res.returncode != 0:
        raise RuntimeError("hipcc build of libm1hip.so failed (see output above)")
    return SO_PATH


def load() -> C.CDLL:
    global _lib
    with _lock:
        if _lib is not None:
            return _lib
        if not os.path.exists(SO_PATH):
            raise RuntimeError(
                f"libm1hip.so not found at {SO_PATH}: the HIP extension is the only compute path of this "
                "package (no CPU/eager fallback). Run `python -c 'import __graft_entry__ as g; g.build()'`.")
        import torch
        lib = C.CDLL(SO_PATH, mode=C.RTLD_GLOBAL)
        for name, (res, args) in SIGNATURES.items():
            fn = getattr(lib, name)
            fn.restype = res
            fn.argtypes = args
        _lib = lib
        return _lib


def status_name(rc: int) -> str:
    return load().m1_status_name(rc).decode()


def check(rc: int, what: str) -> None:
    if rc != 0:
        raise RuntimeError(f"{what} failed: {status_name(rc)} ({rc})")
```

prostatemr_3d-cad-cspca_amd/hip/ops.py:

```python
from __future__ import annotations

import ctypes as C
import os as _os
from typing import Optional, Sequence, Tuple

import torch

from .debug import trace_reset, trace_snapshot
from . import lib as L
from .streams import (_BRANCH, _FOLD, _WGP, _p, _req, _run_deferred_wgrads, _stream, branch, exchange_streams,
                      finish_queued_for_exchange, fold_async_default, fold_drop, fold_pending, join_side_streams,
                      on_origin_stream, submit_wgrad)
from .gradslot import _GradSlot, _slot_of, _slot_target, _slot_written, batch_tail, fanout
from .panels import _PANEL_EPOCH, _conv_ws, _pair_panel_ws, _panel_ws, invalidate_panels, repack_all

IN_EPS = 1e-3


def _dt(t: torch.Tensor) -> int:
    if t.dtype == torch.float32:
        return L.M1_F32
    if t.dtype == torch.bfloat16:
        return L.M1_BF16
    raise RuntimeError(f"unsupported activation dtype {t.dtype} (float32 / bfloat16 only)")


def _ws(N: int, V: int, Cn: int, nsums: int, device) -> torch.Tensor:
    n = L.load().m1_reduce_ws_floats(int(N), int(V), int(Cn), int(nsums))
    return torch.empty(int(n), dtype=torch.float32, device=device)


def _desc(srcs: Sequence[torch.Tensor], cout: int, k, s) -> L.m1_conv_desc_t:
    d = L.m1_conv_desc_t()
    x0 = srcs[0]
    d.N, d.D, d.H, d.W = int(x0.shape[0]), int(x0.shape[1]), int(x0.shape[2]), int(x0.shape[3])
    d.Cin = int(sum(int(t.shape[4]) for t in srcs))
    d.Cout = int(cout)
    d.kd, d.kh, d.kw = (int(v) for v in k)
    d.sd, d.sh, d.sw = (int(v) for v in s)
    d.dtype = _dt(x0)
    d.nsrc = len(srcs)
    if len(srcs) > L.M1_MAX_SRC:
        raise RuntimeError("too many concat members")
    for i, t in enumerate(srcs):
        if t.shape[:4] != x0.shape[:4] or t.dtype != x0.dtype:
            raise RuntimeError("concat members must agree in N,D,H,W and dtype")
        d.src[i].ptr = t.data_ptr()
        d.src[i].C = int(t.shape[4])
    return d


def _nvc(x: torch.Tensor, k: int = 1) -> Tuple[int, int, int]:
    N, Cn = int(x.shape[0]), int(x.shape[-1]) // k
    return N, x.numel() // (N * k * Cn), Cn


def _sink(param: torch.Tensor):
    g = getattr(param, "_m1_gsink", None)
    if g is not None:
        param._m1_live = True
        return g, 1, None
    t = torch.empty_like(param, dtype=torch.float32)
    return t, 0, t


def _sinks(*params):
    bound = {getattr(p, "_m1_gsink", None) is not None for p in params if p is not None}
    if len(bound) == 1:
        out = [(None, 0, None) if p is None else _sink(p) for p in params]
        return [o[0] for o in out], int(True in bound), [o[2] for o in out]
    tmp = [None if p is None else torch.empty(p.shape if p.dim() > 1 else (p.numel(),), dtype=torch.float32, device=p.device)
           for p in params]
    return tmp, 0, list(tmp)


def same_out(size: int, s: int) -> int:
    return -(-size // s)


_INBWD = {"on": _os.environ.get("M1_INBWD_FUSE", "1") != "0", "fused": 0, "plain": 0}


def _dgrad_targets(ctx, srcs, first: int):
    dsrc = []
    ptrs = (C.c_void_p * len(srcs))()
    accs = (C.c_int * len(srcs))()
    for i, t in enumerate(srcs):
        g = None
        if ctx.needs_input_grad[first + i]:
            g, accs[i] = _slot_target(ctx.gslots[i], t)
        dsrc.append(g)
        ptrs[i] = _p(g)
    return dsrc, ptrs, accs


def _dgrad_written(ctx, dsrc) -> None:
    for slot, g in zip(ctx.gslots, dsrc):
        if g is not None:
            _slot_written(slot)


class _Conv3d(torch.autograd.Function):
    @staticmethod
    def forward(ctx, w, b, k, s, transposed, want_stats, *srcs):
        _req(w, b, *srcs)
        lib = L.load()
        x0 = srcs[0]
        cout = int(w.shape[3] if transposed else w.shape[4])
        cin = int(w.shape[4] if transposed else w.shape[3])
        d = _desc(srcs, cout, k, s)
        if d.Cin != cin or tuple(w.shape[:3]) != tuple(k):
            raise RuntimeError(f"kernel {tuple(w.shape)} does not match inputs (Cin={d.Cin}, k={k})")
        if transposed:
            osz = (d.N, d.D * d.sd, d.H * d.sh, d.W * d.sw, cout)
        else:
            osz = (d.N, same_out(d.D, d.sd), same_out(d.H, d.sh), same_out(d.W, d.sw), cout)
        y = torch.empty(osz, dtype=x0.dtype, device=x0.device)
        ws, packed = _panel_ws(w, d, transposed, 0)
        stats = None
        if transposed:
            L.check(lib.m1_convT3d_fwd(C.byref(d), _p(w), _p(b), _p(y), _p(ws), packed, _stream()), "m1_convT3d_fwd")
        else:
            if want_stats:
                stats = torch.empty((d.N, cout, 2), dtype=torch.float32, device=x0.device)
            L.check(lib.m1_conv3d_fwd(C.byref(d), _p(w), _p(b), _p(y), _p(stats), _p(ws), packed, _stream()), "m1_conv3d_fwd")
        ctx.save_for_backward(w, *srcs)
        ctx.w_param, ctx.b_param = w, b
        ctx.gslots = [_slot_of(t) for t in srcs]
        ctx.k, ctx.s, ctx.transposed, ctx.has_bias, ctx.cout = tuple(k), tuple(s), transposed, b is not None, cout
        ctx.in_src = None
        for t in srcs:
            tk = getattr(t, "_m1_in_src", None)
            if tk is not None:
                tk.readers += 1
        tok = getattr(srcs[0], "_m1_in_src", None)
        if _INBWD["on"] and len(srcs) == 1 and not transposed and ctx.gslots[0] is None and tok is not None and tok.src is not None:
            ctx.in_src = tok
        if want_stats:
            ctx.mark_non_differentiable(stats)
            ctx.set_materialize_grads(False)
            return y, stats
        return y

    @staticmethod
    def backward(ctx, dy, *_unused):
        lib = L.load()
        w, *srcs = ctx.saved_tensors
        if dy is None:
            return (None,) * (6 + len(srcs))
        dy = dy.contiguous()
        _req(dy)
        d = _desc(srcs, ctx.cout, ctx.k, ctx.s)
        st = _stream()
        name = "convT3d" if ctx.transposed else "conv3d"
        dw = db = None
        if ctx.needs_input_grad[0] or (ctx.has_bias and ctx.needs_input_grad[1]):
            dw, db = _wgrad_into_sinks(lib, d, dy, ctx.w_param, ctx.b_param if ctx.has_bias else None, ctx.transposed, st, srcs)
        dsrc, ptrs, accs = _dgrad_targets(ctx, srcs, 6)
        any_d = any(g is not None for g in dsrc)
        if any_d and ctx.in_src is not None and accs[0] == 0:
            tok = ctx.in_src
            xs, stats, gamma, beta, slope = tok.src
            da = dsrc[0]
            N, _, Cn = _nvc(xs)
            nmax = int(lib.m1_conv3d_dgrad_inbwd_rows(C.byref(d)))
            part = torch.empty(N * nmax * Cn * 2 + N * Cn * 2 + 64, dtype=torch.float32, device=da.device)
            nparts = C.c_int(0)
            ws, packed = _panel_ws(ctx.w_param, d, False, 1, (True,))
            L.check(lib.m1_conv3d_dgrad_inbwd(C.byref(d), _p(w), _p(dy), _p(da), _p(xs), _p(stats), _p(gamma), _p(beta), float(slope),
                                              _p(part), nmax, C.byref(nparts), _p(ws), packed, st), "m1_conv3d_dgrad_inbwd")
            if nparts.value > 0:
                tok.partials = (part, int(nparts.value), da.data_ptr(), da._version, tuple(da.shape))
                _INBWD["fused"] += 1
            else:
                _INBWD["plain"] += 1
        elif any_d:
            fn = lib.m1_convT3d_dgrad if ctx.transposed else lib.m1_conv3d_dgrad
            ws, packed = _panel_ws(ctx.w_param, d, ctx.transposed, 1, tuple(bool(g is not None) for g in dsrc))
            L.check(fn(C.byref(d), _p(w), _p(dy), ptrs, accs, _p(ws), packed, st), f"m1_{name}_dgrad")
            _dgrad_written(ctx, dsrc)
        return (dw, db, None, None, None, None, *dsrc)


def _wgrad_into_sinks(lib, d, dy, w_param, b_param, transposed: bool, st, srcs=()):
    (wbuf, bbuf), acc_w, (dw, db) = _sinks(w_param, b_param)
    fn = lib.m1_convT3d_wgrad if transposed else lib.m1_conv3d_wgrad
    ws = _conv_ws(d, transposed, 2, w_param.device)
    submit_wgrad(fn, d, dy, wbuf, bbuf, ws, acc_w, transposed, srcs, st, flat=dw is None and db is None)
    return dw, db


class _ConvPair(torch.autograd.Function):

    @staticmethod
    def forward(ctx, w1, b1, w4, b4, k, s, *srcs):
        _req(w1, b1, w4, b4, *srcs)
        lib = L.load()
        x0 = srcs[0]
        c1, c4 = int(w1.shape[4]), int(w4.shape[4])
        d = _desc(srcs, c1 + c4, k, s)
        osz = (d.N, same_out(d.D, d.sd), same_out(d.H, d.sh), same_out(d.W, d.sw))
        y1 = torch.empty((*osz, c1), dtype=x0.dtype, device=x0.device)
        y4 = torch.empty((*osz, c4), dtype=x0.dtype, device=x0.device)
        s1 = torch.empty((d.N, c1, 2), dtype=torch.float32, device=x0.device)
        s4 = torch.empty((d.N, c4, 2), dtype=torch.float32, device=x0.device)
        ws, packed = _pair_panel_ws(w1, w4, d, 0)
        L.check(lib.m1_conv3d_pair_fwd(C.byref(d), _p(w1), _p(b1), _p(w4), _p(b4), c1, _p(y1), _p(y4), _p(s1), _p(s4), _p(ws), packed,
                                       _stream()), "m1_conv3d_pair_fwd")
        ctx.save_for_backward(w1, w4, *srcs)
        ctx.w1_param, ctx.b1_param, ctx.w4_param = w1, b1, w4
        ctx.gslots = [_slot_of(t) for t in srcs]
        ctx.k, ctx.s, ctx.c1, ctx.c4 = tuple(k), tuple(s), c1, c4
        ctx.mark_non_differentiable(s1, s4)
        ctx.set_materialize_grads(False)
        return y1, s1, y4, s4

    @staticmethod
    def backward(ctx, dy1, _s1, dy4, _s4):
        lib = L.load()
        w1, w4, *srcs = ctx.saved_tensors
        n_in = 6 + len(srcs)
        if dy1 is None and dy4 is None:
            return (None,) * n_in
        osz = (srcs[0].shape[0], *[same_out(int(v), st_) for v, st_ in zip(srcs[0].shape[1:4], ctx.s)])
        if dy1 is None:
            dy1 = torch.zeros((*osz, ctx.c1), dtype=srcs[0].dtype, device=srcs[0].device)
        if dy4 is None:
            dy4 = torch.zeros((*osz, ctx.c4), dtype=srcs[0].dtype, device=srcs[0].device)
        dy1, dy4 = dy1.contiguous(), dy4.contiguous()
        st = _stream()
        dw1 = db1 = None
        iw, isrc = getattr(ctx, "idx_w1", 0), getattr(ctx, "idx_src", 6)
        if ctx.needs_input_grad[iw] or ctx.needs_input_grad[iw + 1]:
            dw1, db1 = _wgrad_into_sinks(lib, _desc(srcs, ctx.c1, ctx.k, ctx.s), dy1, ctx.w1_param, ctx.b1_param, False, st, srcs)
        d = _desc(srcs, ctx.c1 + ctx.c4, ctx.k, ctx.s)
        dsrc, ptrs, accs = _dgrad_targets(ctx, srcs, isrc)
        if any(g is not None for g in dsrc):
            ws, packed = _pair_panel_ws(ctx.w1_param, ctx.w4_param, d, 1, tuple(bool(g is not None) for g in dsrc))
            L.check(lib.m1_conv3d_pair_dgrad(C.byref(d), _p(w1), _p(w4), ctx.c1, _p(dy1), _p(dy4), ptrs, accs, _p(ws), packed, st),
                    "m1_conv3d_pair_dgrad")
            _dgrad_written(ctx, dsrc)
        return (dw1, db1, None, None, None, None, *dsrc)


class _WgradTap(torch.autograd.Function):

    @staticmethod
    def forward(ctx, y, w, b, k, s, *srcs):
        ctx.save_for_backward(*srcs)
        ctx.w_param, ctx.b_param, ctx.k, ctx.s = w, b, tuple(k), tuple(s)
        return y.view_as(y)

    @staticmethod
    def backward(ctx, dy):
        srcs = ctx.saved_tensors
        if dy is None:
            return (None,) * (5 + len(srcs))
        dyc = dy.contiguous()
        dw, db = _wgrad_into_sinks(L.load(), _desc(srcs, int(ctx.w_param.shape[4]), ctx.k, ctx.s), dyc, ctx.w_param, ctx.b_param, False,
                                   _stream(), srcs)
        return (dy, dw, db, None, None, *([None] * len(srcs)))


class _PairGraft(torch.autograd.Function):

    @staticmethod
    def forward(ctx, y1, y4, w1, b1, w4, k, s, *srcs):
        ctx.save_for_backward(w1, w4, *srcs)
        ctx.w1_param, ctx.b1_param, ctx.w4_param = w1, b1, w4
        ctx.gslots = [_slot_of(t) for t in srcs]
        ctx.k, ctx.s, ctx.c1, ctx.c4 = tuple(k), tuple(s), int(w1.shape[4]), int(w4.shape[4])
        ctx.idx_w1, ctx.idx_src = 2, 7
        ctx.set_materialize_grads(False)
        return y1.view_as(y1), y4.view_as(y4)

    @staticmethod
    def backward(ctx, dy1, dy4):
        g = _ConvPair.backward(ctx, dy1, None, dy4, None)
        return (None, None, g[0], g[1], None, None, None, *g[6:])


_FORCE_DIRECT = [False]


def conv_pair_supported(srcs, w1, w4, s) -> bool:
    if _os.environ.get("M1_CONV_PAIR", "1") == "0" or _FORCE_DIRECT[0] or not srcs[0].is_cuda:
        return False
    seg = 8 if srcs[0].dtype == torch.bfloat16 else 4
    c1, c4 = int(w1.shape[4]), int(w4.shape[4])
    if not (c4 >= 128 and c1 % seg == 0 and all(int(t.shape[4]) % seg == 0 for t in srcs)):
        return False
    d = _desc(srcs, c1 + c4, tuple(int(v) for v in w1.shape[:3]), s)
    return bool(L.load().m1_conv3d_pair_supported(C.byref(d), c1))


def conv_pair_same(srcs, w1, b1, w4, b4, k, s):
    dev = srcs[0].device
    if _os.environ.get("M1_CONV_PAIR_FWD", "1") == "1":
        y1, s1, y4raw, s4 = _ConvPair.apply(w1, b1, w4, b4, tuple(k), tuple(s), *srcs)
    else:
        with torch.no_grad():
            det = [t.detach() for t in srcs]
            with branch(dev, 0) as br0:
                y4n, s4 = _Conv3d.apply(w4, b4, tuple(k), tuple(s), False, True, *det)
            y1n, s1 = _Conv3d.apply(w1, b1, tuple(k), tuple(s), False, True, *det)
            br0.join()
        y1, y4raw = _PairGraft.apply(y1n, y4n, w1, b1, w4, tuple(k), tuple(s), *srcs)
    with branch(dev, 0) as br:
        y4 = _WgradTap.apply(y4raw, w4, b4, tuple(k), tuple(s), *[t.detach() for t in srcs])
    return y1, s1, y4, s4, br


def conv3d_same(srcs, w, b, k, s, stats: bool = False):
    if isinstance(srcs, torch.Tensor):
        srcs = [srcs]
    return _Conv3d.apply(w, b, tuple(k), tuple(s), False, bool(stats), *srcs)


def conv3d_transpose_same(srcs, w, b, k, s):
    if isinstance(srcs, torch.Tensor):
        srcs = [srcs]
    return _Conv3d.apply(w, b, tuple(k), tuple(s), True, False, *srcs)


def instnorm_stats(x: torch.Tensor) -> torch.Tensor:
    _req(x)
    N, V, Cn = _nvc(x)
    stats = torch.empty((N, Cn, 2), dtype=torch.float32, device=x.device)
    ws = _ws(N, V, Cn, 2, x.device)
    L.check(L.load().m1_instnorm_stats(_p(x), N, V, Cn, _dt(x), IN_EPS, _p(stats), _p(ws), _stream()), "m1_instnorm_stats")
    return stats


class _InTok:
    __slots__ = ("src", "partials", "readers")

    def __init__(self):
        self.src, self.partials, self.readers = None, None, 0


class _InstNormAct(torch.autograd.Function):
    @staticmethod
    def forward(ctx, x, gamma, beta, slope, stats, tok=None):
        _req(x, gamma, beta)
        N, V, Cn = _nvc(x)
        if stats is None:
            stats = instnorm_stats(x)
        y = torch.empty_like(x)
        L.check(L.load().m1_instnorm_apply(_p(x), _p(stats), _p(gamma), _p(beta), float(slope), _p(y), N, V, Cn, _dt(x),
                                           _stream()), "m1_instnorm_apply")
        ctx.save_for_backward(x, stats, gamma, beta)
        ctx.g_param, ctx.b_param = gamma, beta
        ctx.slope = float(slope)
        ctx.tok = tok
        return y

    @staticmethod
    def backward(ctx, dy):
        x, stats, gamma, beta = ctx.saved_tensors
        dy = dy.contiguous()
        N, V, Cn = _nvc(x)
        dx = torch.empty_like(x)
        (gbuf, bbuf), acc, (dg, db) = _sinks(ctx.g_param, ctx.b_param)
        tok = ctx.tok
        pp = tok.partials if tok is not None else None
        if tok is not None:
            tok.partials = None
        if (pp is not None and tok.readers == 1 and pp[2] == dy.data_ptr() and pp[3] == dy._version and pp[4] == tuple(dy.shape)):
            part, nparts = pp[0], pp[1]
            sums = part[part.numel() - N * Cn * 2 - 64:]
            L.check(L.load().m1_instnorm_bwd_partials(_p(x), _p(stats), _p(gamma), _p(beta), ctx.slope, _p(dy), _p(dx), _p(gbuf), _p(bbuf),
                                                      N, V, Cn, _dt(x), _p(part), nparts, _p(sums), acc, _stream()),
                    "m1_instnorm_bwd_partials")
            return dx, dg, db, None, None, None
        ws = _ws(N, V, Cn, 2, x.device)
        L.check(L.load().m1_instnorm_bwd(_p(x), _p(stats), _p(gamma), _p(beta), ctx.slope, _p(dy), _p(dx), _p(gbuf), _p(bbuf),
                                         N, V, Cn, _dt(x), _p(ws), acc, _stream()), "m1_instnorm_bwd")
        return dx, dg, db, None, None, None


def instnorm_act(x, gamma, beta, slope: float = 1.0, stats=None):
    if _INBWD["on"] and stats is not None and torch.is_grad_enabled():
        tok = _InTok()
        y = _InstNormAct.apply(x, gamma, beta, slope, stats, tok)
        tok.src = (x, stats, gamma, beta, float(slope))
        y._m1_in_src = tok
        return y
    return _InstNormAct.apply(x, gamma, beta, slope, stats)


_SE_DEFER: list = []


def flush_deferred() -> None:
    join_side_streams()
    if not _SE_DEFER:
        return
    jobs = (L.SeGateJob * len(_SE_DEFER))(*[j for j, _ in _SE_DEFER])
    try:
        L.check(L.load().m1_se_gate_bwd_batch(jobs, len(_SE_DEFER), _stream()), "m1_se_gate_bwd_batch")
    finally:
        _SE_DEFER.clear()


def drop_deferred() -> None:
    fold_drop()
    join_side_streams()
    _SE_DEFER.clear()


class _SECombine(torch.autograd.Function):
    @staticmethod
    def forward(ctx, y3, y4, g3, b3, g4, b4, W6, b6, W7, b7, drop_rate, rng, layer_id, s3, s4, gate, dup=False):
        _req(y3, y4, g3, b3, g4, b4, W6, b6, W7, b7)
        lib = L.load()
        N, V, Fn = _nvc(y3)
        Fr = int(W6.shape[-1])
        st = _stream()
        ident = g4 is None and b4 is None
        if (g4 is None) != (b4 is None) or tuple(y4.shape) != tuple(y3.shape):
            raise RuntimeError("se_combine: gamma4 / beta4 both or neither; y4 must have y3's shape")
        s3 = instnorm_stats(y3) if s3 is None else s3
        s4 = None if ident else (instnorm_stats(y4) if s4 is None else s4)
        if gate is not None:
            hidden, g = gate
            if hidden.numel() != Fr or g.numel() != Fn:
                raise RuntimeError("se_combine: precomputed gate does not match this block")
        else:
            hidden = torch.empty(Fr, dtype=torch.float32, device=y3.device)
            g = torch.empty(Fn, dtype=torch.float32, device=y3.device)
            L.check(lib.m1_se_gate_fwd(_p(b3), _p(W6), _p(b6), _p(W7), _p(b7), Fn, Fr, _p(hidden), _p(g), st), "m1_se_gate_fwd")
        dup = bool(dup)
        if dup and (ident or Fn % (8 if y3.dtype == torch.bfloat16 else 4)):
            raise RuntimeError("se_combine: the duplicating form needs a norm4 residual and whole 16-byte channel vectors")
        out = torch.empty((2 * N, *y3.shape[1:]), dtype=y3.dtype, device=y3.device) if dup else torch.empty_like(y3)
        mask = None
        if drop_rate > 0.0 and y3.dtype == torch.bfloat16 and Fn % 8 == 0 and any(ctx.needs_input_grad):
            mask = torch.empty(out.numel() // 8, dtype=torch.uint8, device=y3.device)
        fwd = lib.m1_se_combine_dup_fwd if dup else lib.m1_se_combine_fwd
        L.check(fwd(_p(y3), _p(y4), _p(s3), _p(s4), _p(g3), _p(b3), _p(g4), _p(b4), _p(g), _p(out), N, V, Fn,
                    _dt(y3), float(drop_rate), _p(rng), int(layer_id), _p(mask), st), "m1_se_combine_fwd")
        ctx.ident, ctx.dup = ident, dup
        if ident:
            ctx.save_for_backward(y3, y4, s3, g3, b3, W6, W7, hidden, g)
        else:
            ctx.save_for_backward(y3, y4, s3, s4, g3, b3, g4, b4, W6, W7, hidden, g)
        ctx.params = (g3, b3, g4, b4, W6, b6, W7, b7)
        ctx.mask = mask
        ctx.rng, ctx.drop_rate, ctx.layer_id = rng, float(drop_rate), int(layer_id)
        return out

    @staticmethod
    def backward(ctx, dout):
        lib = L.load()
        if ctx.ident:
            y3, y4, s3, g3, b3, W6, W7, hidden, g = ctx.saved_tensors
            s4 = g4 = b4 = None
        else:
            y3, y4, s3, s4, g3, b3, g4, b4, W6, W7, hidden, g = ctx.saved_tensors
        dout = dout.contiguous()
        N, V, Fn = _nvc(y3)
        Fr = int(W6.shape[-1])
        st = _stream()
        dev = y3.device
        dy3, dy4 = torch.empty_like(y3), torch.empty_like(y4)
        (bg3, bb3, bg4, bb4, bW6, bb6, bW7, bb7), acc, rets = _sinks(*ctx.params)
        dg = torch.empty(Fn + Fr, dtype=torch.float32, device=dev)
        ws = _ws(N, V, Fn, 5, dev)
        bwd = lib.m1_se_combine_dup_bwd if ctx.dup else lib.m1_se_combine_bwd
        L.check(bwd(_p(y3), _p(y4), _p(s3), _p(s4), _p(g3), _p(b3), _p(g4), _p(b4), _p(g), _p(dout),
                    _p(dy3), _p(dy4), _p(bg3), _p(bb3), _p(bg4), _p(bb4), _p(dg), N, V, Fn, _dt(y3),
                    ctx.drop_rate, _p(ctx.rng), ctx.layer_id, _p(ctx.mask), _p(ws), acc, st), "m1_se_combine_bwd")
        if acc == 1:
            job = L.SeGateJob(_p(b3), _p(W6), _p(W7), _p(hidden), _p(g), _p(dg), _p(bb3), _p(bW6), _p(bb6), _p(bW7), _p(bb7),
                              Fn, Fr, 1, 0)
            _SE_DEFER.append((job, (b3, W6, W7, hidden, g, dg)))
        else:
            L.check(lib.m1_se_gate_bwd(_p(b3), _p(W6), _p(W7), _p(hidden), _p(g), _p(dg), Fn, Fr, _p(bb3), _p(bW6), _p(bb6),
                                       _p(bW7), _p(bb7), acc, st), "m1_se_gate_bwd")
        return (dy3, dy4, *rets, None, None, None, None, None, None, None)


def se_combine(y3, y4, g3, b3, g4, b4, W6, b6, W7, b7, drop_rate=0.0, rng=None, layer_id=0, stats3=None, stats4=None,
               gate=None, dup=False):
    return _SECombine.apply(y3, y4, g3, b3, g4, b4, W6, b6, W7, b7, drop_rate, rng, layer_id, stats3, stats4, gate, bool(dup))


def se_gate_batch(params):
    if not params:
        return []
    _req(*[t for ps in params for t in ps])
    dev = params[0][0].device
    sizes = [(int(W6.shape[-1]), int(W6.shape[-2])) for _, W6, _, _, _ in params]
    buf = torch.empty(sum(a + b for a, b in sizes), dtype=torch.float32, device=dev)
    jobs = (L.SeGateFwdJob * len(params))()
    out, off = [], 0
    for j, ((b3, W6, b6, W7, b7), (Fr, Fn)) in enumerate(zip(params, sizes)):
        hidden, g = buf[off:off + Fr], buf[off + Fr:off + Fr + Fn]
        off += Fr + Fn
        jobs[j] = L.SeGateFwdJob(_p(b3), _p(W6), _p(b6), _p(W7), _p(b7), hidden.data_ptr(), g.data_ptr(), Fn, Fr)
        out.append((hidden, g))
    L.check(L.load().m1_se_gate_fwd_batch(jobs, len(params), _stream()), "m1_se_gate_fwd_batch")
    return out


def _gate_sigma_bwd(ctx, theta, phi, wpsi, sigma, dsigma):
    N, Dt, Ht, Wt, Cn = (int(v) for v in theta.shape)
    Dp, Hp, Wp = (int(v) for v in phi.shape[1:4])
    dtheta, dphi = torch.empty_like(theta), torch.empty_like(phi)
    (wbuf, bbuf), acc, (dw, db) = _sinks(ctx.w_param, ctx.b_param)
    ws = _ws(N, Dt * Ht * Wt, Cn, 2, theta.device)
    L.check(L.load().m1_gate_sigma_bwd(_p(theta), _p(phi), _p(wpsi), _p(sigma), _p(dsigma), _p(dtheta), _p(dphi), _p(wbuf),
                                       _p(bbuf), N, Dt, Ht, Wt, Dp, Hp, Wp, Cn, _dt(theta), _p(ws), acc, _stream()),
            "m1_gate_sigma_bwd")
    return dtheta, dphi, dw, db


def _mul_sigma_bwd(ctx, x, sigma, dy):
    N, D, H, W, Cn = (int(v) for v in x.shape)
    dsig = torch.empty_like(sigma)
    dx, acc = _slot_target(ctx.gslot, x)
    L.check(L.load().m1_mul_sigma_bwd(_p(x), _p(sigma), _p(dy), _p(dx), _p(dsig), N, D, H, W, Cn, *ctx.ss, _dt(x), acc,
                                      _stream()), "m1_mul_sigma_bwd")
    _slot_written(ctx.gslot)
    return dx, dsig


class _GateSigma(torch.autograd.Function):
    @staticmethod
    def forward(ctx, theta, phi, wpsi, bpsi):
        _req(theta, phi, wpsi, bpsi)
        N, Dt, Ht, Wt, Cn = (int(v) for v in theta.shape)
        Dp, Hp, Wp = (int(v) for v in phi.shape[1:4])
        sigma = torch.empty((N, Dt, Ht, Wt), dtype=theta.dtype, device=theta.device)
        L.check(L.load().m1_gate_sigma_fwd(_p(theta), _p(phi), _p(wpsi), _p(bpsi), _p(sigma), N, Dt, Ht, Wt, Dp, Hp, Wp, Cn,
                                           _dt(theta), _stream()), "m1_gate_sigma_fwd")
        ctx.save_for_backward(theta, phi, wpsi, sigma)
        ctx.w_param, ctx.b_param = wpsi, bpsi
        return sigma

    @staticmethod
    def backward(ctx, dsigma):
        return _gate_sigma_bwd(ctx, *ctx.saved_tensors, dsigma.contiguous())


def gate_sigma(theta, phi, wpsi, bpsi):
    return _GateSigma.apply(theta, phi, wpsi, bpsi)


class _MulSigma(torch.autograd.Function):
    @staticmethod
    def forward(ctx, x, sigma, ss):
        _req(x, sigma)
        N, D, H, W, Cn = (int(v) for v in x.shape)
        y = torch.empty_like(x)
        L.check(L.load().m1_mul_sigma_fwd(_p(x), _p(sigma), _p(y), N, D, H, W, Cn, int(ss[0]), int(ss[1]), int(ss[2]), _dt(x),
                                          _stream()), "m1_mul_sigma_fwd")
        ctx.save_for_backward(x, sigma)
        ctx.ss = tuple(int(v) for v in ss)
        ctx.gslot = _slot_of(x)
        return y

    @staticmethod
    def backward(ctx, dy):
        return (*_mul_sigma_bwd(ctx, *ctx.saved_tensors, dy.contiguous()), None)


def mul_sigma(x, sigma, ss=(1, 1, 1)):
    return _MulSigma.apply(x, sigma, tuple(ss))


class _GateSigmaMul(torch.autograd.Function):

    @staticmethod
    def forward(ctx, theta, phi, wpsi, bpsi, x, ss):
        _req(theta, phi, x)
        N, Dt, Ht, Wt, Ci = (int(v) for v in theta.shape)
        Dp, Hp, Wp = (int(v) for v in phi.shape[1:4])
        _, D, H, W, Cx = (int(v) for v in x.shape)
        sigma = torch.empty((N, Dt, Ht, Wt), dtype=theta.dtype, device=theta.device)
        y = torch.empty_like(x)
        L.check(L.load().m1_gate_sigma_mul_fwd(_p(theta), _p(phi), _p(wpsi), _p(bpsi), _p(sigma), _p(x), _p(y), N, Dt, Ht, Wt, Dp, Hp, Wp,
                                               Ci, D, H, W, Cx, int(ss[0]), int(ss[1]), int(ss[2]), _dt(x), _stream()),
                "m1_gate_sigma_mul_fwd")
        ctx.save_for_backward(theta, phi, wpsi, sigma, x)
        ctx.w_param, ctx.b_param = wpsi, bpsi
        ctx.ss = tuple(int(v) for v in ss)
        ctx.gslot = _slot_of(x)
        ctx.set_materialize_grads(False)
        return y, sigma

    @staticmethod
    def backward(ctx, dy, dsigma_out):
        theta, phi, wpsi, sigma, x = ctx.saved_tensors
        if dy is None:
            dy = torch.zeros_like(x)
        dx, dsig = _mul_sigma_bwd(ctx, x, sigma, dy.contiguous())
        if dsigma_out is not None:
            dsig = dsig + dsigma_out.to(dsig.dtype)
        return (*_gate_sigma_bwd(ctx, theta, phi, wpsi, sigma, dsig), dx, None)


_GATE_FUSED = {"on": _os.environ.get("M1_GATE_FWD_FUSED", "1") != "0"}


def gate_sigma_mul(theta, phi, wpsi, bpsi, x, ss=(1, 1, 1)):
    vec = 8 if theta.dtype == torch.bfloat16 else 4
    ok = (_GATE_FUSED["on"] and theta.shape[-1] % vec == 0 and x.shape[-1] % vec == 0 and
          all(int(x.shape[1 + i]) == int(theta.shape[1 + i]) * int(ss[i]) for i in range(3)))
    if ok:
        return _GateSigmaMul.apply(theta, phi, wpsi, bpsi, x, tuple(ss))
    sigma = gate_sigma(theta, phi, wpsi, bpsi)
    return mul_sigma(x, sigma, ss), sigma
# ... 1164 lines not shown
```

prostatemr_3d-cad-cspca_amd/hip/streams.py:

```python
import ctypes as C
import os as _os
from typing import Optional

import torch

from . import lib as L
from .debug import _POISON

_BRANCH = {"on": _os.environ.get("M1_STREAMS", "1") != "0", "streams": {}, "used": set(), "depth": 0}


def _p(t: Optional[torch.Tensor]):
    return None if t is None else t.data_ptr()


def _stream():
    s = torch.cuda.current_stream().cuda_stream
    if _POISON >= 2:
        L.load().m1_debug_scribble(0, 8, s)
    return s


def _side_stream():
    if not _BRANCH["on"]:
        return False
    origin = _BRANCH.get("origin")
    if origin is None:
        return False
    cur = torch.cuda.current_stream()
    return cur if cur != origin else False


def _req(*ts):
    side = None
    for t in ts:
        if t is None:
            continue
        if not t.is_cuda:
            raise RuntimeError("M1 HIP ops need tensors on a GPU (cuda/HIP) device: the HIP extension is the only "
                               "compute path of this package; there is no CPU fallback")
        if not t.is_contiguous():
            raise RuntimeError("M1 HIP ops need contiguous NDHWC tensors")
        if side is None:
            side = _side_stream()
        if side:
            t.record_stream(side)


class branch:

    def __init__(self, device, k: int = 0):
        self.on = _BRANCH["on"] and device.type == "cuda" and _BRANCH["depth"] == 0
        if self.on:
            _BRANCH["origin"] = torch.cuda.current_stream(device)
            key = (device, k)
            if key not in _BRANCH["streams"]:
                _BRANCH["streams"][key] = torch.cuda.Stream(device=device)
            self.side = _BRANCH["streams"][key]
            self.cur = torch.cuda.current_stream(device)
            self.ctx = torch.cuda.stream(self.side)

    def __enter__(self):
        if self.on:
            self.side.wait_stream(self.cur)
            _BRANCH["used"].add(self.side)
            self.ctx.__enter__()
            _BRANCH["depth"] += 1
        return self

    def __exit__(self, *exc):
        if self.on:
            _BRANCH["depth"] -= 1
            self.ctx.__exit__(*exc)
        return False

    def join(self, *tensors):
        if self.on:
            self.cur.wait_stream(self.side)
            for t in tensors:
                if t is not None:
                    t.record_stream(self.cur)


_FOLD = {"on": _os.environ.get("M1_WG_FOLD_BATCH", "1") != "0", "keep": [],
         "async": int(_os.environ.get("M1_FOLD_ASYNC", "-1")), "stream": None,
         "async_mb": int(_os.environ.get("M1_FOLD_ASYNC_MB", "0")), "bytes": 0}


_WGP = {"maxvox": int(_os.environ.get("M1_WG_DEFER_VOX", str(1 << 40)) or 0), "jobs": [], "extra": []}


def submit_wgrad(fn, d, dy, wbuf, bbuf, ws, acc_w, transposed: bool, srcs, st, flat: bool) -> None:
    if not (flat and _FOLD["on"]):
        L.check(fn(C.byref(d), _p(dy), _p(wbuf), _p(bbuf), _p(ws), acc_w, st), "m1_conv3d_wgrad")
        return
    lib = L.load()
    cur_ = torch.cuda.current_stream(ws.device)
    if (_WGP["maxvox"] > 0 and _BRANCH["on"] and _BRANCH.get("origin") is not None and
            int(d.N) * int(d.D) * int(d.H) * int(d.W) <= _WGP["maxvox"]):
        _WGP["jobs"].append((fn, d, dy, wbuf, bbuf, ws, acc_w, tuple(srcs)))
        _WGP["extra"].extend((t, cur_) for t in (dy, *srcs))
    else:
        lib.m1_wgrad_defer(1)
        try:
            L.check(fn(C.byref(d), _p(dy), _p(wbuf), _p(bbuf), _p(ws), acc_w, st), "m1_conv3d_wgrad")
        finally:
            lib.m1_wgrad_defer(0)
    _FOLD["keep"].append((ws, cur_))
    if transposed and bbuf is not None:
        _FOLD["keep"].append((dy, cur_))
    _FOLD["bytes"] += ws.numel() * ws.element_size()
    if _BRANCH["on"] and ((_FOLD["async"] > 0 and len(_FOLD["keep"]) >= _FOLD["async"]) or
                          (_FOLD["async_mb"] > 0 and _FOLD["bytes"] >= _FOLD["async_mb"] << 20)):
        _fold_async()


def _run_deferred_wgrads(stream_handle, stream) -> None:
    jobs, _WGP["jobs"] = _WGP["jobs"], []
    if not jobs:
        return
    lib = L.load()
    lib.m1_wgrad_defer(1)
    try:
        for fn, d, dy, wbuf, bbuf, ws, acc_w, _srcs in jobs:
            L.check(fn(C.byref(d), _p(dy), _p(wbuf), _p(bbuf), _p(ws), acc_w, stream_handle), "m1_conv3d_wgrad (deferred)")
    finally:
        lib.m1_wgrad_defer(0)
    for t, made_on in _WGP["extra"]:
        if made_on != stream:
            t.record_stream(stream)
    _WGP["extra"] = []


def fold_async_default(n: int) -> None:
    if "M1_FOLD_ASYNC" not in _os.environ:
        _FOLD["async"] = int(n)


def _fold_here() -> None:
    cur = torch.cuda.current_stream()
    try:
        _run_deferred_wgrads(_stream(), cur)
        L.check(L.load().m1_wgrad_fold_pending(_stream()), "m1_wgrad_fold_pending")
        for ws, made_on in _FOLD["keep"]:
            if made_on != cur:
                ws.record_stream(cur)
    finally:
        _FOLD["keep"].clear(); _FOLD["bytes"] = 0


def _fold_async() -> None:
    origin = _BRANCH.get("origin")
    cur = torch.cuda.current_stream()
    if origin is None or cur != origin or not _FOLD["keep"]:
        return
    fs = _FOLD["stream"]
    if fs is None:
        fs = _FOLD["stream"] = torch.cuda.Stream(device=cur.device)
    fs.wait_stream(cur)
    for s in _BRANCH["used"]:
        if s != cur and s != fs:
            fs.wait_stream(s)
    _BRANCH["used"].add(fs)
    with torch.cuda.stream(fs):
        _fold_here()


def fold_pending() -> None:
    if _FOLD["keep"]:
        _fold_here()


def fold_drop() -> None:
    _WGP["jobs"], _WGP["extra"] = [], []
    if _FOLD["keep"]:
        L.load().m1_wgrad_fold_drop()
        _FOLD["keep"].clear(); _FOLD["bytes"] = 0


def join_side_streams() -> None:
    if _BRANCH["used"]:
        cur = torch.cuda.current_stream()
        for s in _BRANCH["used"]:
            if s != cur:
                cur.wait_stream(s)
        _BRANCH["used"].clear()
    fold_pending()


def finish_queued_for_exchange() -> None:
    if _FOLD["keep"]:
        cur = torch.cuda.current_stream()
        origin = _BRANCH.get("origin")
        if origin is not None and origin != cur:
            cur.wait_stream(origin)
        for s in _BRANCH["used"]:
            if s != cur:
                cur.wait_stream(s)
        fold_pending()


def on_origin_stream() -> bool:
    origin = _BRANCH.get("origin")
    return origin is None or not torch.cuda.is_available() or torch.cuda.current_stream() == origin


def exchange_streams():
    origin = _BRANCH.get("origin")
    out = [origin] if origin is not None else []
    return out + [s for s in _BRANCH["used"] if s is not origin]
```

prostatemr_3d-cad-cspca_amd/unets/network_blocks.py:

```python
from __future__ import annotations

from typing import Dict, List, Optional, Sequence, Union

import torch
import torch.nn as nn

from .. import initializers as init
from ..hip import ops

Tensors = Union[torch.Tensor, Sequence[torch.Tensor]]
_GEN = torch.Generator().manual_seed(0)


def set_init_seed(seed: int) -> None:
    _GEN.manual_seed(int(seed))


def _as_list(x: Tensors) -> List[torch.Tensor]:
    return [x] if isinstance(x, torch.Tensor) else list(x)


class Conv3D(nn.Module):
    transposed = False

    def __init__(self, in_channels: int, filters: int, kernel_size, strides=(1, 1, 1), padding: str = "same",
                 kernel_initializer=None, bias_initializer=None, kernel_regularizer=None, bias_regularizer=None):
        super().__init__()
        assert padding == "same" or tuple(kernel_size) == (1, 1, 1), "only padding='same' occurs on the M1 path"
        self.in_channels, self.filters = int(in_channels), int(filters)
        self.kernel_size, self.strides = tuple(int(k) for k in kernel_size), tuple(int(s) for s in strides)
        self.kernel_regularizer, self.bias_regularizer = kernel_regularizer, bias_regularizer
        kinit = kernel_initializer if kernel_initializer is not None else init.GlorotUniform()
        binit = bias_initializer if bias_initializer is not None else init.Zeros()
        self.kernel = nn.Parameter(kinit(self._kernel_shape(), _GEN).contiguous())
        self.bias = nn.Parameter(binit((self.filters,), _GEN).contiguous())

    def _kernel_shape(self):
        return (*self.kernel_size, self.in_channels, self.filters)

    def forward(self, x: Tensors, stats: bool = False):
        return ops.conv3d_same(_as_list(x), self.kernel, self.bias, self.kernel_size, self.strides, stats=stats)


class Conv3DTranspose(Conv3D):
    transposed = True

    def _kernel_shape(self):
        return (*self.kernel_size, self.filters, self.in_channels)

    def forward(self, x: Tensors) -> torch.Tensor:
        return ops.conv3d_transpose_same(_as_list(x), self.kernel, self.bias, self.kernel_size, self.strides)


class InstanceNormalization(nn.Module):

    def __init__(self, channels: int):
        super().__init__()
        self.gamma = nn.Parameter(torch.ones(channels))
        self.beta = nn.Parameter(torch.zeros(channels))

    def forward(self, x: torch.Tensor, slope: float = 1.0, stats=None) -> torch.Tensor:
        return ops.instnorm_act(x, self.gamma, self.beta, slope, stats)


class _DropoutBase(nn.Module):
    _next_id = [1]

    def __init__(self, rate: float):
        super().__init__()
        self.rate = float(rate)
        self.layer_id = _DropoutBase._next_id[0]
        _DropoutBase._next_id[0] += 1
        self.rng: Optional[torch.Tensor] = None

    def active(self) -> bool:
        raise NotImplementedError

    def effective_rate(self) -> float:
        return self.rate if (self.rate > 0.0 and self.active()) else 0.0

    def forward(self, x: torch.Tensor) -> torch.Tensor:
        r = self.effective_rate()
        if r == 0.0:
            return x
        if self.rng is None:
            raise RuntimeError("dropout layer has no RNG state attached (construct it through M1/M1Core)")
        return ops.dropout(x, r, self.rng, self.layer_id)


class MonteCarloDropout(_DropoutBase):

    def active(self) -> bool:
        return True


class Dropout(_DropoutBase):

    def active(self) -> bool:
        return self.training


class SEResNetBottleNeck(nn.Module):

    def __init__(self, filters, kernel_size, strides, conv_params, reduction, in_channels=None):
        super().__init__()
        if in_channels is None:
            raise TypeError("SEResNetBottleNeck needs in_channels (torch builds weights eagerly)")
        self.filters, self.kernel_size, self.strides = int(filters), tuple(kernel_size), tuple(strides)
        self.identity_residual = int(in_channels) == int(filters)
        if self.identity_residual and self.strides != (1, 1, 1):
            raise ValueError("Incompatible shapes: SEResNetBottleNeck with C_in == filters (%d) multiplies its output with its own input "
                             "(network_blocks.py:63,77), which needs strides (1,1,1), got %r" % (self.filters, self.strides))
        self.conv_params, self.reduction = conv_params, int(reduction)
        cp = {k: v for k, v in conv_params.items() if k != "padding"}
        q = self.filters // 4
        self.conv1 = Conv3D(in_channels, q, self.kernel_size, self.strides, **cp)
        self.norm1 = InstanceNormalization(q)
        self.conv2 = Conv3D(q, q, (3, 3, 3), (1, 1, 1), **cp)
        self.norm2 = InstanceNormalization(q)
        self.conv3 = Conv3D(q, self.filters, (1, 1, 1), (1, 1, 1), **cp)
        self.norm3 = InstanceNormalization(self.filters)
        if not self.identity_residual:
            self.conv4 = Conv3D(in_channels, self.filters, self.kernel_size, self.strides, **cp)
            self.norm4 = InstanceNormalization(self.filters)
        self.conv6 = Conv3D(self.filters, self.filters // self.reduction, (1, 1, 1), (1, 1, 1), padding="valid")
        self.conv7 = Conv3D(self.filters // self.reduction, self.filters, (1, 1, 1), (1, 1, 1), padding="valid")
        self._gate = None

    def gate_params(self):
        return (self.norm3.beta, self.conv6.kernel, self.conv6.bias, self.conv7.kernel, self.conv7.bias)

    @staticmethod
    def precompute_gates(blocks):
        for blk, pair in zip(blocks, ops.se_gate_batch([b.gate_params() for b in blocks])):
            blk._gate = pair

    def forward(self, input_tensor: Tensors, dropout: Optional[_DropoutBase] = None, dup: bool = False) -> torch.Tensor:
        members = _as_list(input_tensor)
        if self.identity_residual:
            if dup:
                members = [torch.cat([t, t], dim=0) for t in members]
            return self._forward_identity(members, dropout)
        if ops.conv_pair_supported(members, self.conv1.kernel, self.conv4.kernel, self.strides):
            y1, s1, y4, s4, br = ops.conv_pair_same(members, self.conv1.kernel, self.conv1.bias, self.conv4.kernel, self.conv4.bias,
                                                    self.kernel_size, self.strides)
        else:
            pairs = [ops.fanout(t, 2) for t in members]
            srcs, srcs4 = [a for a, _ in pairs], [b for _, b in pairs]
            with ops.branch(srcs[0].device, 0) as br:
                y4, s4 = self.conv4(srcs4, stats=True)
            y1, s1 = self.conv1(srcs, stats=True)
        a = self.norm1(y1, 0.1, s1)
        y2, s2 = self.conv2(a, stats=True)
        a = self.norm2(y2, 0.1, s2)
        y3, s3 = self.conv3(a, stats=True)
        br.join(y4, s4)
        rate = dropout.effective_rate() if dropout is not None else 0.0
        gate, self._gate = self._gate, None
        return ops.se_combine(y3, y4, self.norm3.gamma, self.norm3.beta, self.norm4.gamma, self.norm4.beta,
                              self.conv6.kernel, self.conv6.bias, self.conv7.kernel, self.conv7.bias, rate,
                              dropout.rng if (dropout is not None and rate > 0.0) else None,
                              dropout.layer_id if dropout is not None else 0, s3, s4, gate, dup=dup)


    def _forward_identity(self, members, dropout):
        x = members[0] if len(members) == 1 else torch.cat(members, dim=-1).contiguous()
        x1, xr = ops.fanout(x, 2)
        y1, s1 = self.conv1([x1], stats=True)
        a = self.norm1(y1, 0.1, s1)
        y2, s2 = self.conv2(a, stats=True)
        a = self.norm2(y2, 0.1, s2)
        y3, s3 = self.conv3(a, stats=True)
        rate = dropout.effective_rate() if dropout is not None else 0.0
        gate, self._gate = self._gate, None
        return ops.se_combine(y3, xr, self.norm3.gamma, self.norm3.beta, None, None,
                              self.conv6.kernel, self.conv6.bias, self.conv7.kernel, self.conv7.bias, rate,
                              dropout.rng if (dropout is not None and rate > 0.0) else None,
                              dropout.layer_id if dropout is not None else 0, s3, None, gate)


class GridAttentionBlock3D(nn.Module):

    def __init__(self, inter_channels, sub_samp, conv_params, in_channels=None, gating_channels=None):
        super().__init__()
        if in_channels is None or gating_channels is None:
            raise TypeError("GridAttentionBlock3D needs in_channels and gating_channels")
        self.inter_channels, self.sub_samp, self.conv_params = int(inter_channels), tuple(sub_samp), conv_params
        cp = {k: v for k, v in conv_params.items() if k != "padding"}
        ic = self.inter_channels
        self.theta = Conv3D(in_channels, ic, self.sub_samp, self.sub_samp, **cp)
        self.phi = Conv3D(gating_channels, ic, (1, 1, 1), (1, 1, 1), **cp)
        self.psi = Conv3D(ic, 1, (1, 1, 1), (1, 1, 1), **cp)
        self.W = Conv3D(in_channels, ic, (1, 1, 1), (1, 1, 1), **cp)
        self.normW = InstanceNormalization(ic)

    def forward(self, conv_tensor: torch.Tensor, gating_tensor: torch.Tensor):
        g = gating_tensor
        x_t, x = ops.fanout(conv_tensor, 2)
        theta_x = self.theta(x_t)
        phi_g = self.phi(g)
        y, sigma = ops.gate_sigma_mul(theta_x, phi_g, self.psi.kernel, self.psi.bias, x, self.sub_samp)
        Wy_raw, sW = self.W(y, stats=True)
        W_y = self.normW(Wy_raw, 1.0, sW)
        return W_y, sigma


class StitchingProbDecoder(nn.Module):

    def __init__(self, num_classes=2, filters=(32, 64, 128, 256, 512), strides=None, kernel_sizes=None,
                 kernel_initializer=None, bias_initializer=None, kernel_regularizer=None, bias_regularizer=None):
        super().__init__()
        self.num_classes, self.filters = int(num_classes), tuple(filters)
        self.logits = Conv3D(self.filters[0], self.num_classes, (1, 1, 1), (1, 1, 1),
                             kernel_initializer=kernel_initializer, bias_initializer=bias_initializer,
                             kernel_regularizer=kernel_regularizer, bias_regularizer=bias_regularizer)

    def forward(self, decoder_features: torch.Tensor) -> torch.Tensor:
        return self.logits(decoder_features)
```

Before: 91.07 volumes/s.

## Fuse twin conv1/conv4 weight-gradient jobs into one paired wgrad kernel

Adds a paired weight-gradient kernel that reads the shared input activation once and accumulates gradients for two convolutions (conv1 and the small conv4 branch) that consume the same sources, writing both dW/dB outputs. On the Python side, deferred wgrad jobs are tagged as twins, matched at fold time and launched as one paired call, and unmatched jobs are carried over to a later fold. The goal is to avoid loading the input tile twice and to save a kernel launch per residual block. The cost is a more complex deferral and matching path, a per-launch workspace allocation, and a new kernel variant that only applies to bf16 1x3x3 shapes where the second conv has at most 32 output channels.

```diff
diff --git a/include/m1hip.h b/include/m1hip.h
--- a/include/m1hip.h
+++ b/include/m1hip.h
@@ -57,6 +57,9 @@
                          void* const* dx, const int* accumulate, void* ws, int ws_packed, void* stream);
 int m1_conv3d_wgrad(const m1_conv_desc_t* d, const void* dy, float* dw, float* db, void* ws, int accumulate,
                     void* stream);
+int m1_conv3d_pair_wgrad_supported(const m1_conv_desc_t* d, int C1);
+int m1_conv3d_pair_wgrad(const m1_conv_desc_t* d, int C1, const void* dy1, const void* dy4, float* dw1, float* db1, float* dw4,
+                         float* db4, void* ws, int accumulate, void* stream);
 int m1_set_force_direct(int on);
 int m1_config_set(const char* name, int value);
 int m1_config_unset(const char* name);
diff --git a/prostatemr_3d-cad-cspca_amd/csrc/dispatch.hip b/prostatemr_3d-cad-cspca_amd/csrc/dispatch.hip
--- a/prostatemr_3d-cad-cspca_amd/csrc/dispatch.hip
+++ b/prostatemr_3d-cad-cspca_amd/csrc/dispatch.hip
@@ -566,6 +566,47 @@
     M1ProfScope ps(prof_name("conv3d_wgrad", d).s, 2.0 * conv_macs(d, false), conv_bytes(d, false), (hipStream_t)stream);
     return wgrad_common(d, false, dy, dw, db, ws, (hipStream_t)stream, accumulate);
 }
+static int pair_wgrad_runs(const m1_conv_desc_t* d, int C1, const void* dy1, const void* dy4, float* dw1, float* db1, float* dw4, float* db4,
+                           void* ws, hipStream_t st, bool dry) {
+    if (!desc_ok(d) || g_force_direct || !M1_CFG("M1_WG_PAIR", 1)) return M1_ERR_UNSUPPORTED;
+    if (d->dtype != M1_BF16 || C1 <= 0 || C1 >= d->Cout) return M1_ERR_UNSUPPORTED;
+    const Geo q = conv_geo(d);
+    const WgradWs L = wgrad_ws(d, false);
+    float* const rx = ws ? reinterpret_cast<float*>(at(ws, L.rx)) : reinterpret_cast<float*>(256);
+    m1_conv_desc_t d1 = *d, d4 = *d;
+    d1.Cout = C1; d4.Cout = d->Cout - C1;
+    for (int i = 0, off = 0; i < d->nsrc;) {
+        const int run = equal_run(d, i);
+        const void* Am[M1_MAX_SRC]; int aoffs[M1_MAX_SRC];
+        for (int m = 0, o = off; m < run; ++m) { Am[m] = d->src[i + m].ptr; aoffs[m] = o; o += d->src[i + m].C; }
+        float* const rxi = rx + (long long)i * L.rx_floats;
+        const WgradSpec g4 = wgrad_spec(&d4, false, q, i, off, dy4, dw4, i == 0 ? db4 : nullptr, rxi, L.rx_floats);
+        const WgradSpec g1 = wgrad_spec(&d1, false, q, i, off, dy1, dw1, i == 0 ? db1 : nullptr, rxi, L.rx_floats);
+        if (!tf_wanted(g4) || !tf_wanted(g1)) return M1_ERR_UNSUPPORTED;
+        const int rc = m1_tf_pair_wgrad(g4, g1, st, run, Am, aoffs, L.rx_floats, dry);
+        if (rc) return dry ? M1_ERR_UNSUPPORTED : rc;
+        for (int m = 0; m < run; ++m) off += d->src[i++].C;
+    }
+    return M1_OK;
+}
+extern "C" int m1_conv3d_pair_wgrad_supported(const m1_conv_desc_t* d, int C1) {
+    return pair_wgrad_runs(d, C1, nullptr, nullptr, nullptr, nullptr, nullptr, nullptr, nullptr, nullptr, true) == M1_OK;
+}
+extern "C" int m1_conv3d_pair_wgrad(const m1_conv_desc_t* d, int C1, const void* dy1, const void* dy4, float* dw1, float* db1, float* dw4,
+                                    float* db4, void* ws, int accumulate, void* stream) {
+    if (m1_debug_skip("conv_wgrad")) return M1_OK;
+    if (!desc_ok(d) || !dy1 || !dy4 || !dw1 || !dw4 || !ws) return M1_ERR_BAD_ARG;
+    hipStream_t st = (hipStream_t)stream;
+    int rc = pair_wgrad_runs(d, C1, dy1, dy4, dw1, db1, dw4, db4, ws, st, true); if (rc) return rc;
+    M1ProfScope ps(prof_name("conv3d_wgrad", d).s, 2.0 * conv_macs(d, false), conv_bytes(d, false), st);
+    if (!accumulate) {
+        const size_t taps = (size_t)d->kd * d->kh * d->kw, C4 = (size_t)(d->Cout - C1);
+        if (m1_zero_async(dw1, taps * d->Cin * C1 * sizeof(float), st) != M1_OK || m1_zero_async(dw4, taps * d->Cin * C4 * sizeof(float), st) != M1_OK ||
+            (db1 && m1_zero_async(db1, (size_t)C1 * sizeof(float), st) != M1_OK) || (db4 && m1_zero_async(db4, C4 * sizeof(float), st) != M1_OK))
+            return M1_ERR_LAUNCH;
+    }
+    return pair_wgrad_runs(d, C1, dy1, dy4, dw1, db1, dw4, db4, ws, st, false);
+}
 extern "C" int m1_convT3d_wgrad(const m1_conv_desc_t* d, const void* dy, float* dw, float* db, void* ws, int accumulate,
                                 void* stream) {
     if (m1_debug_skip("conv_wgrad")) return M1_OK;
diff --git a/prostatemr_3d-cad-cspca_amd/csrc/gather.h b/prostatemr_3d-cad-cspca_amd/csrc/gather.h
--- a/prostatemr_3d-cad-cspca_amd/csrc/gather.h
+++ b/prostatemr_3d-cad-cspca_amd/csrc/gather.h
@@ -50,6 +50,9 @@
 bool m1_tf_wgrad_supported(const WgradSpec& g);
 int m1_tf_wgrad(const WgradSpec& g, long long nw, int nb, hipStream_t st);
 int m1_tf_wgrad_multi(const WgradSpec& g, long long nw, int nb, hipStream_t st, int nmem, const void* const* Am, const int* a_offs, long long rx_mem);
+bool m1_tf_pair_wgrad_supported(const WgradSpec& g4, int C1);
+int m1_tf_pair_wgrad(const WgradSpec& g4, const WgradSpec& g1, hipStream_t st, int nmem, const void* const* Am, const int* a_offs,
+                     long long rx_mem, bool dry);
 int m1_mfma_wgrad_ex(const WgradSpec& g, long long nw, int nb, hipStream_t st);
 bool m1_tap_wgrad_supported(const WgradSpec& g);
 int m1_tap_wgrad(const WgradSpec& g, long long nw, int nb, hipStream_t st);
diff --git a/prostatemr_3d-cad-cspca_amd/csrc/wgrad_tf.hip b/prostatemr_3d-cad-cspca_amd/csrc/wgrad_tf.hip
--- a/prostatemr_3d-cad-cspca_amd/csrc/wgrad_tf.hip
+++ b/prostatemr_3d-cad-cspca_amd/csrc/wgrad_tf.hip
@@ -312,9 +312,247 @@
 #endif
 }
 
+struct TfPairP {
+    TfP t;
+    const bf16_t* B1; int C1;
+    long long off1;
+    int bias4, bias1;
+    int remap;
+};
+
+template <int TF_NKS, int NB>
+__global__ void __launch_bounds__(256, NB == 2 ? 2 : 1) wgrad_tf_pair_kernel(TfPairP pp) {
+#if defined(__HIP_DEVICE_COMPILE__)
+    const TfP& p = pp.t;
+    constexpr int KD = 1, KH = 3, KW = 3, NT = KD * KH * KW;
+    extern __shared__ __attribute__((aligned(16))) unsigned char smem[];
+    const int tid = threadIdx.x, lane = tid & 63, wave = __builtin_amdgcn_readfirstlane(tid >> 6);
+    int bx = blockIdx.x, by = blockIdx.y, bz = blockIdx.z;
+    if (pp.remap) {
+        const int gx = gridDim.x, units = gx * gridDim.z;
+        const int lin = bx + gx * (by + (int)gridDim.y * bz), j = lin >> 3, u = j % units;
+        by = (j / units) * 8 + (lin & 7); bx = u % gx; bz = u / gx;
+    }
+    const int a0 = bx * 32;
+    const int mem = p.nmem > 1 ? bz : 0;
+    const bf16_t* Abase = p.A;
+    if (p.nmem > 1) {
+        Abase = p.Am[0];
+#pragma unroll
+        for (int m = 1; m < M1_MAX_SRC; ++m) if (mem == m) Abase = p.Am[m];
+    }
+    constexpr int PA = 64, PB = 64;
+    constexpr int BT = TF_NKS * 32 * 4 / 256;
+    constexpr int BTILE = BT * 256 * 16;
+    constexpr int NBIT = NB * BT;
+    const int stage_bytes = p.a_bytes + p.b_bytes;
+
+    constexpr unsigned OOB = 0x80000000u;
+    unsigned a_vo[TF_MAX_AIT]; int a_pk[TF_MAX_AIT];
+    const int nait = p.a_slots >> 8;
+#pragma unroll
+    for (int it = 0; it < TF_MAX_AIT; ++it) {
+        const int q = it * 256 + tid;
+        const int row = q >> 2, slp = q & 3;
+        const int hh = row / p.AWt, ww = row - hh * p.AWt;
+        const int sl = slp ^ (((ww >> 3) & 1) << 1);
+        a_pk[it] = (hh << 8) | (ww << 16);
+        a_vo[it] = (row < p.AHt * p.AWt) ? (unsigned)(((hh * p.AW + ww) * p.CA + a0 + sl * 8) * 2) : OOB;
+    }
+    unsigned b_vo[NBIT]; int b_th[BT];
+#pragma unroll
+    for (int it = 0; it < NBIT; ++it) {
+        const int j = it / BT, q = (it % BT) * 256 + tid;
+        const int row = q >> 2, slp = q & 3;
+        const int th = row / p.KWs, tw = row - th * p.KWs;
+        const int sl = slp ^ (((tw >> 3) & 1) << 1);
+        b_th[it % BT] = th;
+        if (j < NB - 1) b_vo[it] = (unsigned)(((th * p.BW + tw) * p.CB + j * 32 + sl * 8) * 2);
+        else b_vo[it] = sl * 8 < pp.C1 ? (unsigned)(((th * p.BW + tw) * pp.C1 + sl * 8) * 2) : OOB;
+    }
+
+    int q_kt = by, q_tw, q_th, q_bd, q_n;
+    { int r = q_kt; q_tw = r % p.tiles_w; r /= p.tiles_w; q_th = r % p.tiles_h; r /= p.tiles_h; q_bd = r % p.BD; q_n = r / p.BD; }
+    int s_tw, s_th, s_bd, s_n;
+    { int r = p.nsplit; s_tw = r % p.tiles_w; r /= p.tiles_w; s_th = r % p.tiles_h; r /= p.tiles_h; s_bd = r % p.BD; s_n = r / p.BD; }
+    auto issue = [&](int st) {
+        const bool live = q_kt < (int)p.ntiles;
+        const int twi = q_tw, thi = q_th, bd = q_bd, n = q_n;
+        q_kt += p.nsplit;
+        q_tw += s_tw; int c = q_tw >= p.tiles_w; q_tw -= c ? p.tiles_w : 0;
+        q_th += s_th + c; c = q_th >= p.tiles_h; q_th -= c ? p.tiles_h : 0;
+        q_bd += s_bd + c; c = q_bd >= p.BD; q_bd -= c ? p.BD : 0;
+        q_n += s_n + c;
+        const int ad0 = bd * p.sd - p.pd, ah0 = thi * p.TH * p.sh - p.ph, aw0 = twi * p.KWs * p.sw - p.pw;
+        const long long lin0 = (((long long)n * p.AD + ad0) * p.AH + ah0) * p.AW + aw0;
+        const int bh0 = thi * p.TH;
+        const long long blin0 = (((long long)n * p.BD + bd) * p.BH + bh0) * p.BW + twi * p.KWs;
+        unsigned char* As = smem + st * stage_bytes;
+        unsigned char* Bs = As + p.a_bytes;
+        const int nrec = live ? 0x7fffffff : 0;
+        const __amdgpu_buffer_rsrc_t ra = __builtin_amdgcn_make_buffer_rsrc((void*)(Abase + lin0 * p.CA), 0, nrec, 0x00020000);
+        const __amdgpu_buffer_rsrc_t rb4 = __builtin_amdgcn_make_buffer_rsrc((void*)(p.B + blin0 * p.CB), 0, nrec, 0x00020000);
+        const __amdgpu_buffer_rsrc_t rb1 = __builtin_amdgcn_make_buffer_rsrc((void*)(pp.B1 + blin0 * pp.C1), 0, nrec, 0x00020000);
+        const bool a_inner = (unsigned)ad0 < (unsigned)p.AD && ah0 >= 0 && ah0 + p.AHt - 1 < p.AH && aw0 >= 0 && aw0 + p.AWt - 1 < p.AW;
+        if (a_inner) {
+#pragma unroll
+            for (int it = 0; it < TF_MAX_AIT; ++it)
+                if (it < nait) __builtin_amdgcn_raw_ptr_buffer_load_lds(ra, (lptr_t)(As + (it * 256 + wave * 64) * 16), 16, a_vo[it], 0, 0, 0);
+        } else {
+#pragma unroll
+            for (int it = 0; it < TF_MAX_AIT; ++it) {
+                if (it < nait) {
+                    const int pk = a_pk[it];
+                    const int hh = (pk >> 8) & 0xff, ww = (pk >> 16) & 0xff;
+                    const bool ok = (unsigned)ad0 < (unsigned)p.AD && (unsigned)(ah0 + hh) < (unsigned)p.AH && (unsigned)(aw0 + ww) < (unsigned)p.AW;
+                    __builtin_amdgcn_raw_ptr_buffer_load_lds(ra, (lptr_t)(As + (it * 256 + wave * 64) * 16), 16, ok ? a_vo[it] : OOB, 0, 0, 0);
+                }
+            }
+        }
+        const bool b_inner = bh0 + p.TH <= p.BH;
+#pragma unroll
+        for (int it = 0; it < NBIT; ++it)
+            __builtin_amdgcn_raw_ptr_buffer_load_lds(it / BT < NB - 1 ? rb4 : rb1, (lptr_t)(Bs + (it * 256 + wave * 64) * 16), 16,
+                                                     (b_inner || bh0 + b_th[it % BT] < p.BH) ? b_vo[it] : OOB, 0, 0, 0);
+    };
+
+    const unsigned lds0 = (unsigned)(unsigned long long)(lptr_t)smem;
+    const int S = p.stages;
+    const int npiece = nait + NBIT;
+    const long long kt0 = by, step = p.nsplit;
+    constexpr int NK = 2 * TF_NKS, NTW = (NT + 3) / 4;
+    const int g2 = lane >> 4, i = lane & 15, kg = g2 >> 1, ch = g2 & 1;
+    unsigned a_ad[2][KW], b_ad[2];
+#pragma unroll
+    for (int h = 0; h < 2; ++h) {
+        const int kk = 8 * kg + 4 * h + (i >> 2);
+        const int th = kk / p.KWs, tw = kk - th * p.KWs;
+#pragma unroll
+        for (int r = 0; r < KW; ++r) {
+            const int ww = tw * p.sw + (wave + r) % KW;
+            a_ad[h][r] = lds0 + ((th * p.sh) * p.AWt + ww) * PA + (ch ^ ((ww >> 3) & 1)) * 32 + (i & 3) * 8;
+        }
+        b_ad[h] = lds0 + p.a_bytes + kk * PB + (ch ^ ((tw >> 3) & 1)) * 32 + (i & 3) * 8;
+    }
+    const unsigned ko1 = (unsigned)(((16 / p.KWs) * p.sh * p.AWt + (16 % p.KWs) * p.sw) * PA);
+    const unsigned ko2 = (unsigned)(((32 / p.KWs) * p.sh * p.AWt + (32 % p.KWs) * p.sw) * PA);
+    unsigned ro[NTW];
+#pragma unroll
+    for (int j = 0; j < NTW; ++j) ro[j] = (unsigned)((((wave + 4 * j) / KW) % KH) * p.AWt * PA);
+    const bool last_ok = wave + 4 * (NTW - 1) < NT;
+    const bool do_bsum = (pp.bias4 || pp.bias1) && a0 == 0 && wave == 3 && mem == 0;
+    const bf16x8_t ones = __builtin_bit_cast(bf16x8_t, make_uint4(0x3F803F80u, 0x3F803F80u, 0x3F803F80u, 0x3F803F80u));
+
+    auto tile = [&](unsigned sb, auto n_c, auto wb_c, f32x16_t (&acc)[NTW][NB], f32x16_t (&accb)[NB]) {
+        constexpr int N = decltype(n_c)::value, P = N + NB, NI = NK * P;
+        constexpr bool WB = decltype(wb_c)::value;
+        constexpr int D = 4, RS = D + 1;
+        static_assert(D <= P, "a dY fragment set must outlive its k-step");
+        u32x2_t bl[2][NB], bh[2][NB], al[RS], ah[RS];
+        auto rd = [&](auto m_c) {
+            constexpr int m = decltype(m_c)::value, u = m / P, j = m % P - NB;
+            if constexpr (j < 0) {
+                const unsigned so = sb + (unsigned)(u * 16) * PB + (unsigned)((j + NB) * BTILE);
+                bl[u & 1][j + NB] = m1_tr_read_asm(b_ad[0] + so); bh[u & 1][j + NB] = m1_tr_read_asm(b_ad[1] + so);
+            } else {
+                constexpr int sl = (u * N + j) % RS;
+                const unsigned so = sb + ro[j] + (u >> 1) * ko2 + (u & 1) * ko1;
+                al[sl] = m1_tr_read_asm(a_ad[0][j % KW] + so); ah[sl] = m1_tr_read_asm(a_ad[1][j % KW] + so);
+            }
+        };
+        m1_static_for<0, D>(rd);
+        bf16x8_t bfr[NB];
+        m1_static_for<0, NI>([&](auto m_c) {
+            constexpr int m = decltype(m_c)::value, u = m / P, j = m % P - NB;
+            if constexpr (m + D < NI) rd(std::integral_constant<int, m + D>{});
+            constexpr int after = NI - 1 - m < D ? NI - 1 - m : D;
+            if constexpr (j < 0) {
+                constexpr int nb = j + NB;
+                m1_lds_wait_n<2 * after>(bl[u & 1][nb], bh[u & 1][nb]);
+                bfr[nb] = m1_frag8(bl[u & 1][nb], bh[u & 1][nb]);
+                if constexpr (WB) { if (do_bsum) accb[nb] = __builtin_amdgcn_mfma_f32_32x32x16_bf16(ones, bfr[nb], accb[nb], 0, 0, 0); }
+            } else {
+                constexpr int sl = (u * N + j) % RS;
+                m1_lds_wait_n<2 * after>(al[sl], ah[sl]);
+                const bf16x8_t afr = m1_frag8(al[sl], ah[sl]);
+#pragma unroll
+                for (int nb = 0; nb < NB; ++nb) acc[j][nb] = __builtin_amdgcn_mfma_f32_32x32x16_bf16(afr, bfr[nb], acc[j][nb], 0, 0, 0);
+            }
+            __builtin_amdgcn_sched_barrier(0);
+        });
+    };
+    auto run_tiles = [&](auto&& tile_fn) {
+        for (int s = 0; s < S - 1; ++s) issue(s);
+        int st = 0;
+        for (long long kt = kt0; kt < p.ntiles; kt += step) {
+            m1_wait_vm<48>(npiece * (S - 2));
+            __builtin_amdgcn_s_barrier();
+            int stn = st + S - 1; if (stn >= S) stn -= S;
+            issue(stn);
+            tile_fn((unsigned)(st * stage_bytes));
+            if (++st == S) st = 0;
+        }
+        asm volatile("s_waitcnt vmcnt(0)" ::: "memory");
+    };
+    float* Rx = p.Rx + (long long)mem * p.rx_mem + (long long)by * p.rx_stride;
+    const int b = lane & 31;
+    auto store = [&](auto n_c, f32x16_t (&acc)[NTW][NB]) {
+#pragma unroll
+        for (int j = 0; j < decltype(n_c)::value; ++j) {
+            const int t = wave + 4 * j;
+#pragma unroll
+            for (int nb = 0; nb < NB; ++nb)
+#pragma unroll
+                for (int e = 0; e < 16; ++e) {
+                    const int a = a0 + (e & 3) + 8 * (e >> 2) + 4 * (lane >> 5);
+                    if (nb < NB - 1) Rx[((long long)t * p.CA + a) * p.CB + nb * 32 + b] = acc[j][nb][e];
+                    else if (b < pp.C1) Rx[pp.off1 + ((long long)t * p.CA + a) * pp.C1 + b] = acc[j][nb][e];
+                }
+        }
+    };
+    f32x16_t acc[NTW][NB];
+#pragma unroll
+    for (int j = 0; j < NTW; ++j)
+#pragma unroll
+        for (int nb = 0; nb < NB; ++nb)
+#pragma unroll
+            for (int e = 0; e < 16; ++e) acc[j][nb][e] = 0.f;
+    f32x16_t accb[NB];
+    if (last_ok) {
+        run_tiles([&](unsigned sb) { tile(sb, std::integral_constant<int, NTW>{}, std::false_type{}, acc, accb); });
+        store(std::integral_constant<int, NTW>{}, acc);
+    } else {
+#pragma unroll
+        for (int nb = 0; nb < NB; ++nb)
+#pragma unroll
+            for (int e = 0; e < 16; ++e) accb[nb][e] = 0.f;
+        run_tiles([&](unsigned sb) { tile(sb, std::integral_constant<int, NTW - 1>{}, std::true_type{}, acc, accb); });
+        store(std::integral_constant<int, NTW - 1>{}, acc);
+        if (do_bsum && lane < 32) {
+#pragma unroll
+            for (int nb = 0; nb < NB; ++nb) {
+                if (nb < NB - 1) { if (pp.bias4) Rx[p.rx_bias + nb * 32 + b] = accb[nb][0]; }
+                else if (pp.bias1 && b < pp.C1) Rx[pp.off1 + (long long)NT * p.CA * pp.C1 + b] = accb[nb][0];
+            }
+        }
+    }
+#endif
+}
+
 
 static inline bool tf_chan_ok(int c) { return c == 8 || c == 16 || (c >= 32 && c % 32 == 0); }
 
+static bool tf_tiles(const WgradSpec& g, int nks, TfP& p) {
+    p.nks = nks;
+    if (!m1_wg_ktiles(g, nks * 32, m1_wg_kws(g.BW, 8), 0, p)) return false;
+    p.AHt = (p.TH - 1) * g.sh + g.kh; p.AWt = (p.KWs - 1) * g.sw + g.kw;
+    p.spra = (g.CA < 32 ? g.CA : 32) / 8; p.sprb = (g.CB < 32 ? g.CB : 32) / 8;
+    const int a_rows = g.kd * p.AHt * p.AWt;
+    p.a_slots = (a_rows * p.spra + 255) / 256 * 256; p.b_slots = nks * 32 * p.sprb;
+    if (p.a_slots > TF_MAX_AIT * 256 || p.AHt > 255 || p.AWt > 255) return false;
+    p.a_bytes = p.a_slots * 16; p.b_bytes = (p.b_slots + 255) / 256 * 256 * 16 + 64;
+    return true;
+}
 static bool tf_plan(const WgradSpec& g, TfP& p) {
     if (g.dtype != M1_BF16) return false;
     const bool k133 = g.kd == 1 && g.kh == 3 && g.kw == 3, k333 = g.kd == 3 && g.kh == 3 && g.kw == 3;
@@ -329,14 +567,7 @@
     p.sd = g.sd; p.sh = g.sh; p.sw = g.sw; p.pd = g.pd; p.ph = g.ph; p.pw = g.pw;
     int n4 = M1_CFG("M1_TF_NKS4", 2);
     const int nks = ((n4 && g.CA <= 16 && g.CB <= 16) || (n4 == 2 && g.kd == 1)) ? 4 : 2;
-    p.nks = nks;
-    if (!m1_wg_ktiles(g, nks * 32, m1_wg_kws(g.BW, 8), 0, p)) return false;
-    p.AHt = (p.TH - 1) * g.sh + g.kh; p.AWt = (p.KWs - 1) * g.sw + g.kw;
-    p.spra = (g.CA < 32 ? g.CA : 32) / 8; p.sprb = (g.CB < 32 ? g.CB : 32) / 8;
-    const int a_rows = g.kd * p.AHt * p.AWt;
-    p.a_slots = (a_rows * p.spra + 255) / 256 * 256; p.b_slots = nks * 32 * p.sprb;
-    if (p.a_slots > TF_MAX_AIT * 256 || p.AHt > 255 || p.AWt > 255) return false;
-    p.a_bytes = p.a_slots * 16; p.b_bytes = (p.b_slots + 255) / 256 * 256 * 16 + 64;
+    if (!tf_tiles(g, nks, p)) return false;
     const int sb = p.a_bytes + p.b_bytes, npiece = p.a_slots / 256 + (p.b_slots + 255) / 256;
     int S = (76 * 1024) / sb;
     if (S < 3) S = 3;
@@ -396,3 +627,64 @@
     int rc = m1_check_launch(); if (rc) return rc;
     return m1_wg_fold_members(p.Rx, rx_mem, c.stride, (int)nsplit, g, c.rx_bias, nmem < 1 ? 1 : nmem, a_offs, st);
 }
+
+static bool tf_pair_plan(const WgradSpec& g4, int C1, TfPairP& pp) {
+    TfP& p = pp.t;
+    if (g4.kd != 1 || g4.CA % 32 || (g4.CB != 32 && g4.CB != 64) || (C1 != 8 && C1 != 16 && C1 != 32)) return false;
+    if (g4.sd != 1 || g4.sh != g4.sw || (g4.sh != 1 && g4.sh != 2)) return false;
+    if (!tf_plan(g4, p)) return false;
+    const int NB = g4.CB / 32 + 1, fenv = M1_CFG("M1_WG_PAIR_NKS", 0), force = (fenv == 2 || fenv == 4) ? fenv : 0;
+    const int first = force ? force : 4;
+    for (int k = 0; k < 2; ++k) {
+        const int nks = k == 0 ? first : 6 - first;
+        if (!tf_tiles(g4, nks, p)) { if (force) return false; continue; }
+        p.b_slots = NB * nks * 128; p.b_bytes = p.b_slots * 16 + 64;
+        const int sb = p.a_bytes + p.b_bytes, npiece = (p.a_slots + p.b_slots) / 256;
+        int S = (76 * 1024) / sb;
+        if (S < 3) S = (160 * 1024) / sb;
+        if (S > TF_MAX_STAGES) S = TF_MAX_STAGES;
+        while (S > 3 && npiece * (S - 2) > 48) --S;
+        if (S >= 3 && npiece * (S - 2) <= 48) { p.stages = S; return true; }
+        if (force) return false;
+    }
+    return false;
+}
+bool m1_tf_pair_wgrad_supported(const WgradSpec& g4, int C1) { TfPairP pp; return tf_pair_plan(g4, C1, pp); }
+
+int m1_tf_pair_wgrad(const WgradSpec& g4, const WgradSpec& g1, hipStream_t st, int nmem, const void* const* Am, const int* a_offs,
+                     long long rx_mem, bool dry) {
+    TfPairP pp;
+    if (nmem < 1 || nmem > M1_MAX_SRC || !tf_pair_plan(g4, g1.CB, pp)) return M1_ERR_UNSUPPORTED;
+    TfP& p = pp.t;
+    const int NB = g4.CB / 32 + 1, taps = g4.kd * g4.kh * g4.kw, aTiles = g4.CA / 32;
+    int tgt_env = M1_CFG("M1_TF_SPLIT", 0);
+    const int tgt = tgt_env > 0 ? tgt_env : (p.ntiles >= 24576 ? 512 : 256);
+    const int ctiles = aTiles * (NB - 1);
+    const long long want = (tgt + ctiles - 1) / ctiles;
+    WgradSpec gc = g4; gc.CB = g4.CB + g1.CB;
+    const WgCopies c = m1_wg_copies(gc, taps, want, p.ntiles, TF_COPIES);
+    if (c.rc) return c.rc;
+    if (dry) return M1_OK;
+    p.bTiles = 1; p.nsplit = (int)c.nsplit;
+    p.Rx = c.Rx; p.rx_stride = c.stride; p.rx_bias = (long long)taps * g4.CA * g4.CB;
+    p.nmem = nmem; p.rx_mem = nmem > 1 ? rx_mem : 0;
+    for (int m = 0; m < nmem && nmem > 1; ++m) p.Am[m] = (const bf16_t*)Am[m];
+    pp.B1 = (const bf16_t*)g1.B; pp.C1 = g1.CB;
+    pp.off1 = m1_wg_copy_floats(taps, g4.CA, g4.CB, g4.CB);
+    pp.bias4 = g4.bsum != nullptr; pp.bias1 = g1.bsum != nullptr;
+    pp.remap = c.nsplit % 8 == 0 && M1_CFG("M1_WG_PAIR_XCD", 1);
+    void (*kern)(TfPairP) = nullptr;
+    if (NB == 2) kern = p.nks == 4 ? wgrad_tf_pair_kernel<4, 2> : wgrad_tf_pair_kernel<2, 2>;
+    if (NB == 3) kern = p.nks == 4 ? wgrad_tf_pair_kernel<4, 3> : wgrad_tf_pair_kernel<2, 3>;
+    if (!kern) return M1_ERR_UNSUPPORTED;
+    if (m1_allow_dynamic_lds((const void*)kern, 160 * 1024) != M1_OK) return M1_ERR_LAUNCH;
+    const size_t smem = (size_t)p.stages * (p.a_bytes + p.b_bytes);
+    dim3 grid(aTiles, (unsigned)c.nsplit, (unsigned)nmem);
+    m1_note_kernel("wgrad_tf_pair");
+    m1_wg_note_plan("wgrad_tf_pair", p.ntiles, want, c.nsplit, c, true, p.stages, grid.x, grid.y, grid.z);
+    m1_note_plan("wgpair:nks=%d nb=%d c1=%d lds=%d xcd=%d", p.nks, NB, g1.CB, (int)smem, pp.remap);
+    hipLaunchKernelGGL(kern, grid, dim3(256), smem, st, pp);
+    int rc = m1_check_launch(); if (rc) return rc;
+    rc = m1_wg_fold_members(p.Rx, p.rx_mem, c.stride, (int)c.nsplit, g4, p.rx_bias, nmem, a_offs, st); if (rc) return rc;
+    return m1_wg_fold_members(p.Rx + pp.off1, p.rx_mem, c.stride, (int)c.nsplit, g1, (long long)taps * g1.CA * g1.CB, nmem, a_offs, st);
+}
diff --git a/prostatemr_3d-cad-cspca_amd/hip/lib.py b/prostatemr_3d-cad-cspca_amd/hip/lib.py
--- a/prostatemr_3d-cad-cspca_amd/hip/lib.py
+++ b/prostatemr_3d-cad-cspca_amd/hip/lib.py
@@ -159,6 +159,8 @@
     "m1_conv3d_pair_supported": (_i, [_desc_p, _i]),
     "m1_conv3d_pair_fwd": (_i, [_desc_p, _vp, _vp, _vp, _vp, _i, _vp, _vp, _vp, _vp, _vp, _i, _vp]),
     "m1_conv3d_pair_dgrad": (_i, [_desc_p, _vp, _vp, _i, _vp, _vp, C.POINTER(_vp), C.POINTER(_i), _vp, _i, _vp]),
+    "m1_conv3d_pair_wgrad_supported": (_i, [_desc_p, _i]),
+    "m1_conv3d_pair_wgrad": (_i, [_desc_p, _i, _vp, _vp, _vp, _vp, _vp, _vp, _vp, _i, _vp]),
     "m1_convT3d_fwd": (_i, [_desc_p, _vp, _vp, _vp, _vp, _i, _vp]),
     "m1_convT3d_dgrad": (_i, [_desc_p, _vp, _vp, C.POINTER(_vp), C.POINTER(_i), _vp, _i, _vp]),
     "m1_convT3d_wgrad": (_i, [_desc_p, _vp, _vp, _vp, _vp, _i, _vp]),
diff --git a/prostatemr_3d-cad-cspca_amd/hip/ops.py b/prostatemr_3d-cad-cspca_amd/hip/ops.py
--- a/prostatemr_3d-cad-cspca_amd/hip/ops.py
+++ b/prostatemr_3d-cad-cspca_amd/hip/ops.py
@@ -10,7 +10,7 @@
 from . import lib as L
 from .streams import (_BRANCH, _FOLD, _WGP, _p, _req, _run_deferred_wgrads, _stream, branch, exchange_streams,
                       finish_queued_for_exchange, fold_async_default, fold_drop, fold_pending, join_side_streams,
-                      on_origin_stream, submit_wgrad)
+                      on_origin_stream, submit_wgrad, current_twin, wgrad_twin, match_wgrad_twins)
 from .gradslot import _GradSlot, _slot_of, _slot_target, _slot_written, batch_tail, fanout
 from .panels import _PANEL_EPOCH, _conv_ws, _pair_panel_ws, _panel_ws, invalidate_panels, repack_all
 
@@ -128,6 +128,7 @@
         ctx.w_param, ctx.b_param = w, b
         ctx.gslots = [_slot_of(t) for t in srcs]
         ctx.k, ctx.s, ctx.transposed, ctx.has_bias, ctx.cout = tuple(k), tuple(s), transposed, b is not None, cout
+        ctx.twin = None if transposed else current_twin()
         ctx.in_src = None
         for t in srcs:
             tk = getattr(t, "_m1_in_src", None)
@@ -155,7 +156,8 @@
         name = "convT3d" if ctx.transposed else "conv3d"
         dw = db = None
         if ctx.needs_input_grad[0] or (ctx.has_bias and ctx.needs_input_grad[1]):
-            dw, db = _wgrad_into_sinks(lib, d, dy, ctx.w_param, ctx.b_param if ctx.has_bias else None, ctx.transposed, st, srcs)
+            dw, db = _wgrad_into_sinks(lib, d, dy, ctx.w_param, ctx.b_param if ctx.has_bias else None, ctx.transposed, st, srcs,
+                                       twin=ctx.twin)
         dsrc, ptrs, accs = _dgrad_targets(ctx, srcs, 6)
         any_d = any(g is not None for g in dsrc)
         if any_d and ctx.in_src is not None and accs[0] == 0:
@@ -182,11 +184,11 @@
         return (dw, db, None, None, None, None, *dsrc)
 
 
-def _wgrad_into_sinks(lib, d, dy, w_param, b_param, transposed: bool, st, srcs=()):
+def _wgrad_into_sinks(lib, d, dy, w_param, b_param, transposed: bool, st, srcs=(), twin=None):
     (wbuf, bbuf), acc_w, (dw, db) = _sinks(w_param, b_param)
     fn = lib.m1_convT3d_wgrad if transposed else lib.m1_conv3d_wgrad
     ws = _conv_ws(d, transposed, 2, w_param.device)
-    submit_wgrad(fn, d, dy, wbuf, bbuf, ws, acc_w, transposed, srcs, st, flat=dw is None and db is None)
+    submit_wgrad(fn, d, dy, wbuf, bbuf, ws, acc_w, transposed, srcs, st, flat=dw is None and db is None, twin=twin)
     return dw, db
 
 
@@ -309,6 +311,29 @@
     with branch(dev, 0) as br:
         y4 = _WgradTap.apply(y4raw, w4, b4, tuple(k), tuple(s), *[t.detach() for t in srcs])
     return y1, s1, y4, s4, br
+
+
+def conv_pair_wgrad_supported(srcs, c1: int, c4: int, k, s) -> bool:
+    return bool(L.load().m1_conv3d_pair_wgrad_supported(C.byref(_desc(srcs, int(c1) + int(c4), k, s)), int(c1)))
+
+
+def conv_pair_wgrad(srcs, dy1, dy4, k, s, dw1, db1, dw4, db4, accumulate: bool = False) -> int:
+    _req(dy1, dy4, dw1, db1, dw4, db4, *srcs)
+    lib = L.load()
+    c1, c4 = int(dy1.shape[4]), int(dy4.shape[4])
+    d = _desc(srcs, c1 + c4, k, s)
+    ws = _conv_ws(d, False, 2, dy4.device)
+    lib.m1_wgrad_defer(1)
+    try:
+        rc = lib.m1_conv3d_pair_wgrad(C.byref(d), c1, _p(dy1), _p(dy4), _p(dw1), _p(db1), _p(dw4), _p(db4), _p(ws), int(bool(accumulate)),
+                                      _stream())
+    finally:
+        lib.m1_wgrad_defer(0)
+    if rc not in (0, -2):
+        L.check(rc, "m1_conv3d_pair_wgrad")
+    if rc == 0:
+        _FOLD["keep"].append((ws, torch.cuda.current_stream(ws.device)))
+    return rc
 
 
 def conv3d_same(srcs, w, b, k, s, stats: bool = False):
diff --git a/prostatemr_3d-cad-cspca_amd/hip/streams.py b/prostatemr_3d-cad-cspca_amd/hip/streams.py
--- a/prostatemr_3d-cad-cspca_amd/hip/streams.py
+++ b/prostatemr_3d-cad-cspca_amd/hip/streams.py
@@ -87,10 +87,89 @@
          "async_mb": int(_os.environ.get("M1_FOLD_ASYNC_MB", "0")), "bytes": 0}
 
 
-_WGP = {"maxvox": int(_os.environ.get("M1_WG_DEFER_VOX", str(1 << 40)) or 0), "jobs": [], "extra": []}
-
-
-def submit_wgrad(fn, d, dy, wbuf, bbuf, ws, acc_w, transposed: bool, srcs, st, flat: bool) -> None:
+_WGP = {"maxvox": int(_os.environ.get("M1_WG_DEFER_VOX", str(1 << 40)) or 0), "jobs": []}
+
+
+_TWIN = [None]
+_PAIR_MAX_C4 = int(_os.environ.get("M1_WG_PAIR_MAXC4", "32"))
+
+
+class wgrad_twin:
+
+    def __init__(self, key, role: int, c_other: int):
+        self.tag = (key, int(role), int(c_other))
+
+    def __enter__(self):
+        self.prev, _TWIN[0] = _TWIN[0], self.tag
+        return self
+
+    def __exit__(self, *exc):
+        _TWIN[0] = self.prev
+        return False
+
+
+def current_twin():
+    return _TWIN[0]
+
+
+class WgJob:
+    __slots__ = ("fn", "d", "dy", "wbuf", "bbuf", "ws", "acc_w", "srcs", "made_on", "twin", "role", "carried")
+
+    def __init__(self, fn, d, dy, wbuf, bbuf, ws, acc_w, srcs, made_on, twin=None, role=0):
+        self.fn, self.d, self.dy, self.wbuf, self.bbuf, self.ws, self.acc_w, self.srcs = fn, d, dy, wbuf, bbuf, ws, acc_w, srcs
+        self.made_on, self.twin, self.role, self.carried = made_on, twin, role, False
+
+
+def match_wgrad_twins(jobs, final: bool, compatible=lambda j1, j4: True):
+    out, waiting = [], {}
+    for j in jobs:
+        key = getattr(j, "twin", None)
+        if key is None or key not in waiting:
+            if key is not None:
+                waiting[key] = len(out)
+            out.append((j,))
+            continue
+        i = waiting.pop(key)
+        other = out[i][0]
+        j1, j4 = (other, j) if other.role == 1 else (j, other)
+        if {other.role, j.role} == {1, 4} and compatible(j1, j4):
+            out[i] = None
+            out.append((j1, j4))
+        else:
+            out.append((j,))
+    held = []
+    if not final:
+        for i in waiting.values():
+            held.append(out[i][0])
+            out[i] = None
+    return [x for x in out if x is not None], held
+
+
+def _pair_desc(d, cout: int):
+    d2 = type(d).from_buffer_copy(d)
+    d2.Cout = int(cout)
+    return d2
+
+
+def _twins_compatible(j1, j4) -> bool:
+    a, b = j1.d, j4.d
+    same = all(int(getattr(a, f)) == int(getattr(b, f)) for f in ("N", "D", "H", "W", "Cin", "kd", "kh", "kw", "sd", "sh", "sw", "dtype", "nsrc"))
+    return (same and j1.acc_w == j4.acc_w and
+            all(a.src[i].ptr == b.src[i].ptr and int(a.src[i].C) == int(b.src[i].C) for i in range(int(a.nsrc))))
+
+
+def _twin_of(tag, d, transposed: bool):
+    if tag is None or transposed:
+        return None, 0
+    key, role, c_other = tag
+    c1 = int(d.Cout) if role == 1 else c_other
+    if int(d.Cout) + c_other - c1 > _PAIR_MAX_C4:
+        return None, 0
+    ok = L.load().m1_conv3d_pair_wgrad_supported(C.byref(_pair_desc(d, int(d.Cout) + c_other)), c1)
+    return (key, role) if ok else (None, 0)
+
+
+def submit_wgrad(fn, d, dy, wbuf, bbuf, ws, acc_w, transposed: bool, srcs, st, flat: bool, twin=None) -> None:
     if not (flat and _FOLD["on"]):
         L.check(fn(C.byref(d), _p(dy), _p(wbuf), _p(bbuf), _p(ws), acc_w, st), "m1_conv3d_wgrad")
         return
@@ -98,8 +177,8 @@
     cur_ = torch.cuda.current_stream(ws.device)
     if (_WGP["maxvox"] > 0 and _BRANCH["on"] and _BRANCH.get("origin") is not None and
             int(d.N) * int(d.D) * int(d.H) * int(d.W) <= _WGP["maxvox"]):
-        _WGP["jobs"].append((fn, d, dy, wbuf, bbuf, ws, acc_w, tuple(srcs)))
-        _WGP["extra"].extend((t, cur_) for t in (dy, *srcs))
+        key, role = _twin_of(twin, d, transposed)
+        _WGP["jobs"].append(WgJob(fn, d, dy, wbuf, bbuf, ws, acc_w, tuple(srcs), cur_, key, role))
     else:
         lib.m1_wgrad_defer(1)
         try:
@@ -115,21 +194,38 @@
         _fold_async()
 
 
-def _run_deferred_wgrads(stream_handle, stream) -> None:
+def _run_deferred_wgrads(stream_handle, stream, final: bool = True) -> None:
     jobs, _WGP["jobs"] = _WGP["jobs"], []
     if not jobs:
         return
+    launches, held = match_wgrad_twins(jobs, final, _twins_compatible)
     lib = L.load()
     lib.m1_wgrad_defer(1)
     try:
-        for fn, d, dy, wbuf, bbuf, ws, acc_w, _srcs in jobs:
-            L.check(fn(C.byref(d), _p(dy), _p(wbuf), _p(bbuf), _p(ws), acc_w, stream_handle), "m1_conv3d_wgrad (deferred)")
+        for la in launches:
+            if len(la) == 2:
+                j1, j4 = la
+                c1 = int(j1.d.Cout)
+                d = _pair_desc(j4.d, c1 + int(j4.d.Cout))
+                ws = torch.empty(max(int(lib.m1_conv_ws_bytes(C.byref(d), 0, 2)), 256), dtype=torch.uint8, device=j4.ws.device)
+                L.check(lib.m1_conv3d_pair_wgrad(C.byref(d), c1, _p(j1.dy), _p(j4.dy), _p(j1.wbuf), _p(j1.bbuf), _p(j4.wbuf), _p(j4.bbuf),
+                                                 _p(ws), j4.acc_w, stream_handle), "m1_conv3d_pair_wgrad (deferred)")
+                _FOLD["keep"].append((ws, stream))
+            else:
+                j = la[0]
+                L.check(j.fn(C.byref(j.d), _p(j.dy), _p(j.wbuf), _p(j.bbuf), _p(j.ws), j.acc_w, stream_handle), "m1_conv3d_wgrad (deferred)")
+                if j.carried:
+                    _FOLD["keep"].append((j.ws, j.made_on))
     finally:
         lib.m1_wgrad_defer(0)
-    for t, made_on in _WGP["extra"]:
-        if made_on != stream:
-            t.record_stream(stream)
-    _WGP["extra"] = []
+    for la in launches:
+        for j in la:
+            for t in (j.dy, *j.srcs):
+                if j.made_on != stream:
+                    t.record_stream(stream)
+    for j in held:
+        j.carried = True
+    _WGP["jobs"] = held + _WGP["jobs"]
 
 
 def fold_async_default(n: int) -> None:
@@ -137,10 +233,10 @@
         _FOLD["async"] = int(n)
 
 
-def _fold_here() -> None:
+def _fold_here(final: bool = True) -> None:
     cur = torch.cuda.current_stream()
     try:
-        _run_deferred_wgrads(_stream(), cur)
+        _run_deferred_wgrads(_stream(), cur, final)
         L.check(L.load().m1_wgrad_fold_pending(_stream()), "m1_wgrad_fold_pending")
         for ws, made_on in _FOLD["keep"]:
             if made_on != cur:
@@ -163,16 +259,16 @@
             fs.wait_stream(s)
     _BRANCH["used"].add(fs)
     with torch.cuda.stream(fs):
+        _fold_here(final=False)
+
+
+def fold_pending() -> None:
+    if _FOLD["keep"] or _WGP["jobs"]:
         _fold_here()
 
 
-def fold_pending() -> None:
-    if _FOLD["keep"]:
-        _fold_here()
-
-
 def fold_drop() -> None:
-    _WGP["jobs"], _WGP["extra"] = [], []
+    _WGP["jobs"] = []
     if _FOLD["keep"]:
         L.load().m1_wgrad_fold_drop()
         _FOLD["keep"].clear(); _FOLD["bytes"] = 0
@@ -189,7 +285,7 @@
 
 
 def finish_queued_for_exchange() -> None:
-    if _FOLD["keep"]:
+    if _FOLD["keep"] or _WGP["jobs"]:
         cur = torch.cuda.current_stream()
         origin = _BRANCH.get("origin")
         if origin is not None and origin != cur:
diff --git a/prostatemr_3d-cad-cspca_amd/unets/network_blocks.py b/prostatemr_3d-cad-cspca_amd/unets/network_blocks.py
--- a/prostatemr_3d-cad-cspca_amd/unets/network_blocks.py
+++ b/prostatemr_3d-cad-cspca_amd/unets/network_blocks.py
@@ -147,9 +147,12 @@
         else:
             pairs = [ops.fanout(t, 2) for t in members]
             srcs, srcs4 = [a for a, _ in pairs], [b for _, b in pairs]
+            key, q = object(), self.filters // 4
             with ops.branch(srcs[0].device, 0) as br:
-                y4, s4 = self.conv4(srcs4, stats=True)
-            y1, s1 = self.conv1(srcs, stats=True)
+                with ops.wgrad_twin(key, 4, q):
+                    y4, s4 = self.conv4(srcs4, stats=True)
+            with ops.wgrad_twin(key, 1, self.filters):
+                y1, s1 = self.conv1(srcs, stats=True)
         a = self.norm1(y1, 0.1, s1)
         y2, s2 = self.conv2(a, stats=True)
         a = self.norm2(y2, 0.1, s2)
```

Result: no change. 91.36 volumes/s, median of 2 (+0.3%).
